# PraKesEy/EEGNetReplication

Hardware: AMD Instinct MI355X
Metric: train trials/sec (fwd+bwd) EEGNet-8,2 22ch x 256 (higher is better)
Workload: dtype fp32; 1 GPU; EEGNet-8,2 train step (fwd+CE+bwd+clamps+Adam), 22ch x 256, batch 4096/GPU, p=0.5, fp32 HIP kernels; model=EEGNet-8,2, global_batch=4096, seq_len=256, channels=22, parallelism=dp1

## Files before the change

eegnetreplication_amd/csrc/eegnet_common.h:

```cpp
#pragma once

#include <hip/hip_runtime.h>
#include <stdint.h>
#include <math.h>

namespace eeg {

constexpr int NTH = 1024;
constexpr int NWAVE = NTH / 64;
constexpr int K2 = 16;
constexpr int NCLS = 4;
constexpr int LP2 = 8;
constexpr int MAXPF = 16;
constexpr int F2MAX = 16;
constexpr int MAXT1Q = 4;

typedef float floatx4 __attribute__((ext_vector_type(4)));

__device__ __forceinline__ floatx4 lds_ld4(const float* p) {
    return *reinterpret_cast<const floatx4*>(__builtin_assume_aligned(p, 16));
}
__device__ __forceinline__ void lds_st4(float* p, floatx4 v) {
    *reinterpret_cast<floatx4*>(__builtin_assume_aligned(p, 16)) = v;
}
typedef float floatx2 __attribute__((ext_vector_type(2)));
__device__ __forceinline__ floatx2 lds_ld2(const float* p) {
    return *reinterpret_cast<const floatx2*>(__builtin_assume_aligned(p, 8));
}
__device__ __forceinline__ void lds_st_oct(float* p, int oc, floatx4 lo, floatx4 hi) {
    const bool sw = (oc >> 2) & 1;
    lds_st4(p + (sw ? 4 : 0), sw ? hi : lo);
    lds_st4(p + (sw ? 0 : 4), sw ? lo : hi);
}

struct Geo {
    int B, C, T, F1, D, F2, K1, P, R;
    int T1, T2, NF;
    int LP, RS;
    int TQ, NT16;
    int RS2;
    int RSW;
    int nwC, nwD;
    int CK, NCT, NKG;
    int nH, nTl, nedge;
    float p, scale, eps, mom;
    int drop;
    int noclamp;
    unsigned long long key;
    unsigned key0, key1;
    unsigned pthr;
    const int32_t* keystep;
    unsigned long long kseed, koff;
    int o_w1, o_g1, o_b1, o_ws, o_g2, o_b2, o_w2, o_W3, o_g3, o_b3, o_Wfc, o_bfc, nparam;
    int nA, nB, nC, nD, nE;
    int QR;
    int grid;
    int gridS;
    int gridA, gridE;
    int ldsA, ldsB, ldsC, ldsD, ldsE, ldsI;
    int ldsX;
    unsigned long long* trace;
    int wide, NOC, CPC, F2P, RB, gridB2;
    int gridW2;
    int splitC, splitD, splitE;
    int ldsWA, ldsWB, ldsWB2, ldsWC, ldsWD, ldsWE, ldsWI;
    int Bn;
    int defer;
    int XP;
};

#define EEG_SHAPE_W5(X)                                                                             \
    X(C, 64) X(T, 512) X(F1, 16) X(D, 4) X(F2, 64) X(K1, 32) X(P, 15) X(R, 16) X(T1, 128) X(T2, 16)  \
    X(NF, 1024) X(LP, 16) X(RS, 548) X(TQ, 128) X(NT16, 32) X(RS2, 144) X(RSW, 156) X(CK, 64)       \
    X(NCT, 4) X(NKG, 32) X(nH, 136) X(nTl, 120) X(nedge, 287) X(o_w1, 0) X(o_g1, 512) X(o_b1, 528)   \
    X(o_ws, 544) X(o_g2, 4640) X(o_b2, 4704) X(o_w2, 4768) X(o_W3, 5792) X(o_g3, 9888) X(o_b3, 9952) \
    X(o_Wfc, 10016) X(o_bfc, 14112) X(nparam, 14116) X(nA, 448) X(nB, 128) X(nC, 4229) X(nD, 5248)    \
    X(nE, 6272) X(QR, 64) X(wide, 1) X(NOC, 4) X(CPC, 16) X(F2P, 64) X(RB, 144) X(splitC, 1)         \
    X(splitD, 1) X(splitE, 1) X(ldsWA, 36656) X(ldsWB, 0) X(ldsWB2, 19712) X(ldsWC, 10528)           \
    X(ldsWD, 37952) X(ldsWE, 29504) X(ldsWI, 37760)
__host__ __device__ __forceinline__ void shape_w5(Geo& g) {
#define EEG_SET_(f, v) g.f = v;
    EEG_SHAPE_W5(EEG_SET_)
#undef EEG_SET_
}
template <bool SPEC>
__device__ __forceinline__ Geo geo_w(const Geo& gin) {
    Geo g = gin;
    if constexpr (SPEC) shape_w5(g);
    return g;
}

constexpr int TR_SLOTS = 16, TR_MAXWG = 2048;
enum TraceEv { TR_ENTRY = 0, TR_PRO, TR_LOOP, TR_PUB, TR_GRP, TR_TOP, TR_FIN, TR_PH0 = 8 };
#ifdef EEGNET_TRACE
#define TRACE_ON(g_) ((g_).trace != nullptr)
#else
#define TRACE_ON(g_) false
#endif
#define TRACE(g_, pass_, ev_)                                                                    \
    do {                                                                                         \
        if (TRACE_ON(g_) && threadIdx.x == 0)                                                      \
            (g_).trace[((size_t)(pass_) * TR_MAXWG + blockIdx.x) * TR_SLOTS + (ev_)] = wall_clock64(); \
    } while (0)
__device__ __forceinline__ void trial_range(const Geo& g, int& b0, int& b1) {
    const long long w = blockIdx.x, G = gridDim.x;
    b0 = (int)(w * g.B / G);
    b1 = (int)((w + 1) * g.B / G);
}

constexpr int TR_FINE = 6;
#define TRACE_FS(g_, pass_, k_)                                                                  \
    do {                                                                                         \
        if (TRACE_ON(g_) && threadIdx.x == 0)                                                      \
            (g_).trace[((size_t)TR_FINE * TR_MAXWG + (pass_)) * TR_SLOTS + (k_)] = wall_clock64(); \
    } while (0)
#define TRACE_PS(g_, k_)                                                                         \
    do {                                                                                         \
        if (TRACE_ON(g_) && threadIdx.x == 0)                                                      \
            (g_).trace[((size_t)(TR_FINE + 1) * TR_MAXWG + blockIdx.x) * TR_SLOTS + (k_)] = wall_clock64(); \
    } while (0)
#define TRACE_PH(g_, pass_, ph_, t0_)                                                            \
    do {                                                                                         \
        if (TRACE_ON(g_) && threadIdx.x == 0) {                                                  \
            const unsigned long long t1_ = clock64();                                            \
            tr_lds_[ph_] += t1_ - (t0_);                                                         \
            (t0_) = t1_;                                                                         \
        }                                                                                        \
    } while (0)
#define TRACE_LOOP(g_, pass_)                                                                    \
    do {                                                                                         \
        TRACE(g_, pass_, TR_LOOP);                                                               \
        if (TRACE_ON(g_) && threadIdx.x == 0)                                                    \
            for (int ph_ = 0; ph_ < 8; ++ph_)                                                    \
                (g_).trace[((size_t)(pass_) * TR_MAXWG + blockIdx.x) * TR_SLOTS + TR_PH0 + ph_] = tr_lds_[ph_]; \
    } while (0)
#ifdef EEGNET_TRACE
#define TRACE_DECL()                                                                             \
    __shared__ unsigned long long tr_lds_[8];                                                    \
    if (threadIdx.x == 0)                                                                        \
        for (int ph_ = 0; ph_ < 8; ++ph_) tr_lds_[ph_] = 0;                                      \
    unsigned long long tph_ = clock64();                                                         \
    (void)tph_
#else
#define TRACE_DECL() unsigned long long tph_ = 0; unsigned long long* tr_lds_ = nullptr; (void)tph_; (void)tr_lds_
#endif

enum CoefField {
    CF_A1 = 0, CF_C1, CF_INV1, CF_MU1, CF_AL2, CF_BE2, CF_INV2, CF_MU3, CF_INV3,
    CF_A3, CF_B3, CF_C3, CF_AO, CF_BO, CF_CO, CF_W, CF_LOSS, CF_ADAM, CF_COUNT
};
constexpr int CSTR = 64;

enum PassCMode { PC_LOGITS = 1, PC_BWD = 2, PC_CE = 4 };

constexpr int KSMAX = 16;
#ifndef EEGNET_NGRPMAX
#define EEGNET_NGRPMAX 16
#endif
constexpr int NGRPMAX = EEGNET_NGRPMAX;
constexpr int NCNT = 40;
#ifndef EEGNET_TKS
#define EEGNET_TKS 64
#endif
constexpr int TKS = EEGNET_TKS;
__host__ __device__ __forceinline__ unsigned* tkw(unsigned* cnt, int i) { return cnt + (size_t)i * TKS; }
constexpr int SPLIT_COLS = 2048;
constexpr int TK_PASSES = 5;
struct FinArgs {
    double* part2;
    unsigned* cnt;
    double* stats;
    float* coef;
    float* bn;
    float* grads;
    float* loss;
    int64_t* nbt;
    int update_running, ce;
    int tpass;
    float* params;
    float* adam_m;
    float* adam_v;
    int32_t* step;
    float lr, b1, b2, eps;
};

enum { TK_A = 0, TK_B, TK_C, TK_D, TK_E, TK_COUNT };

struct WsOff {
    unsigned long long cnt, partA, partB, partC, partD, partE, sums, stats, coef, d2, E1, E2, dp2, dl, s, v, q3, r3;
};
struct FoldCall {
    const eegnet_fold* folds;
    long long row0, slot;
    unsigned long long koff;
    float lr, b1, b2, eps;
    WsOff off;
};

#ifndef EEGNET_NT_MID
#define EEGNET_NT_MID 1
#endif
#ifndef EEGNET_NT_SV
#define EEGNET_NT_SV 1
#endif
template <int NT, typename V>
__device__ __forceinline__ void st_pol(V v, V* p) {
    if constexpr (NT != 0) __builtin_nontemporal_store(v, p);
    else *p = v;
}

#ifndef EEGNET_PRIO
#define EEGNET_PRIO 1
#endif
__device__ __forceinline__ void pace_prio(int done, int total) {
    if constexpr (EEGNET_PRIO != 0) {
        switch ((done * 4) / total) {
        case 0: __builtin_amdgcn_s_setprio(3); break;
        case 1: __builtin_amdgcn_s_setprio(2); break;
        case 2: __builtin_amdgcn_s_setprio(1); break;
        default: __builtin_amdgcn_s_setprio(0); break;
        }
    }
}
__device__ __forceinline__ void tail_prio() {
    if constexpr (EEGNET_PRIO != 0) __builtin_amdgcn_s_setprio(3);
}

__device__ __forceinline__ eegnet_fold fold_rec(const FoldCall& fc) {
#if defined(__HIP_DEVICE_COMPILE__)
    return ((const __attribute__((address_space(4))) eegnet_fold*)fc.folds)[blockIdx.y];
#else
    return fc.folds[blockIdx.y];
#endif
}

__device__ __forceinline__ long long fold_row(const int64_t* __restrict__ perm, long long row0, int bb) {
    return perm ? perm[row0 + bb] : row0 + bb;
}

__device__ __forceinline__ FinArgs fold_fin(const FoldCall& fc, const eegnet_fold& f, int tk, int update_running,
                                            int ce, bool nbt, bool adam, int nparam) {
    char* ws = (char*)f.ws;
    FinArgs a;
    a.part2 = (double*)(ws + fc.off.sums);
    a.cnt = tkw((unsigned*)(ws + fc.off.cnt), tk * NCNT);
    a.stats = (double*)(ws + fc.off.stats);
    a.coef = (float*)(ws + fc.off.coef);
    a.bn = f.bn_buffers;
    a.grads = f.grads;
    a.loss = f.losses ? f.losses + fc.slot : nullptr;
    a.nbt = nbt ? f.num_batches_tracked : nullptr;
    a.update_running = update_running;
    a.ce = ce;
    a.tpass = tk;
    a.params = adam ? f.params : nullptr;
    a.adam_m = adam ? f.adam_state : nullptr;
    a.adam_v = adam ? f.adam_state + nparam : nullptr;
    a.step = adam ? f.step : nullptr;
    a.lr = fc.lr; a.b1 = fc.b1; a.b2 = fc.b2; a.eps = fc.eps;
    return a;
}

__host__ __device__ constexpr int rup4(int a) { return (a + 3) & ~3; }
__host__ __device__ constexpr int imax(int a, int b) { return a > b ? a : b; }
__host__ __device__ constexpr int s_pitch(int T) { return (T + 3) & ~3; }

__host__ __device__ constexpr int row_stride(int K1, int T) {
    const int P = (K1 - 1) / 2, R = K1 - 1 - P, LP = (R + 3) & ~3, OFF = LP - P, OFFD = LP - R;
    const int NW = (OFF + K1 + 6) / 4, TQ = (T + 3) / 4, NT16 = (T + 15) / 16;
    const int NW8 = (imax(OFF, OFFD) + K1 + 10) / 4, NO = (T + 7) / 8;
    const int NWT = (15 + K1 - 1) / 16 + 1;
    const int rs = rup4(imax(imax(imax(imax(4 * (TQ - 1) + 4 * NW, 8 * (NO - 1) + 4 * NW8), LP + 16 * NT16), LP + T + R),
                             OFF + 16 * (NT16 + NWT - 1)));
    return ((rs / 4) & 1) ? rs : rs + 4;
}
__host__ __device__ constexpr int row_stride2(int T) { return rup4(LP2 + T / 4 + 8); }
__host__ __device__ constexpr int row_stride_b2(int T1) {
    const int r = rup4(T1 + 24);
    return ((r / 4) & 1) ? r : r + 4;
}

template <int K1>
struct KG {
    static constexpr int P = (K1 - 1) / 2;
    static constexpr int R = K1 - 1 - P;
    static constexpr int LP = (R + 3) & ~3;
    static constexpr int OFF = LP - P;
    static constexpr int OFFD = LP - R;
    static constexpr int NW = (OFF + K1 + 3 + 3) / 4;
    static constexpr int NW8 = ((OFF > OFFD ? OFF : OFFD) + K1 + 7 + 3) / 4;
    template <int NT>
    static constexpr int nei() { return ((R * (R + 1) / 2 + P * (P + 1) / 2 + R + P) + NT - 1) / NT; }
};

__device__ __forceinline__ float fast_exp(float z) { return __builtin_amdgcn_exp2f(z * 1.4426950408889634f); }
__device__ __forceinline__ float elu_f(float z) { return z > 0.f ? z : fast_exp(z) - 1.f; }
__device__ __forceinline__ float elu_d(float z) { return z > 0.f ? 1.f : fast_exp(z); }

__device__ __forceinline__ unsigned long long mix_key_dev(unsigned long long seed, unsigned long long off) {
    unsigned long long z = seed * 0xD1B54A32D192ED03ull + off * 0x9E3779B97F4A7C15ull + 0x632BE59BD9B4E019ull;
    z = (z ^ (z >> 30)) * 0xBF58476D1CE4E5B9ull;
    z = (z ^ (z >> 27)) * 0x94D049BB133111EBull;
    return z ^ (z >> 31);
}
__device__ __forceinline__ unsigned drop_key(const Geo& g, int layer) {
    if (!g.keystep) return layer ? g.key1 : g.key0;
    const unsigned long long k = mix_key_dev(g.kseed, g.koff + (unsigned long long)(*g.keystep));
    return layer ? (unsigned)(k >> 32) ^ 0x5BD1E995u : (unsigned)k;
}
__device__ __forceinline__ unsigned fold_drop_key(const FoldCall& fc, const eegnet_fold& f, int layer) {
    const unsigned long long k = mix_key_dev(f.seed, fc.koff + (unsigned long long)(*f.step));
    return layer ? (unsigned)(k >> 32) ^ 0x5BD1E995u : (unsigned)k;
}
__device__ __forceinline__ float keep_mul(const Geo& g, const uint8_t* __restrict__ mask, unsigned key,
                                          unsigned idx) {
    if (!g.drop) return 1.f;
    if (mask) return mask[idx] ? g.scale : 0.f;
    unsigned h = idx * 0x9E3779B1u + key;
    h ^= h >> 16;
    h *= 0x85EBCA6Bu;
    h ^= h >> 13;
    h *= 0xC2B2AE35u;
    h ^= h >> 16;
    return (h >> 8) >= g.pthr ? g.scale : 0.f;
}

__device__ __forceinline__ void drain_prologue_loads() { __builtin_amdgcn_s_waitcnt(0); }

template <int U, typename T>
struct Stage {
    T v[U];
    const T* src;
    __device__ __forceinline__ void load(const T* s, int n) {
        src = s;
        const int nth = blockDim.x, last = n > 0 ? n - 1 : 0;
#pragma unroll
        for (int j = 0; j < U; ++j) v[j] = s[min((int)threadIdx.x + j * nth, last)];
    }
    template <typename D>
    __device__ __forceinline__ void store(D* dst, int n) const {
        const int nth = blockDim.x;
#pragma unroll
        for (int j = 0; j < U; ++j) {
            const int i = threadIdx.x + j * nth;
            if (i < n) dst[i] = (D)v[j];
        }
        for (int i = threadIdx.x + U * nth; i < n; i += nth) dst[i] = (D)src[i];
    }
};

template <typename T>
__device__ __forceinline__ T ldc(const T* p) {
#if defined(__HIP_DEVICE_COMPILE__)
    return *(const __attribute__((address_space(4))) T*)p;
#else
    return *p;
#endif
}

__device__ __forceinline__ int opaque0() {
    int z = 0;
    asm volatile("" : "+s"(z));
    return z;
}
__device__ __forceinline__ int opaque0_after(float dep) {
    int z = 0;
    asm volatile("" : "+s"(z) : "v"(dep));
    return z;
}

__device__ __forceinline__ void swap32(float& a, float& b) {
    asm("s_nop 1\n\tv_permlane32_swap_b32 %0, %1" : "+v"(a), "+v"(b));
}
__device__ __forceinline__ void swap16(float& a, float& b) {
    asm("s_nop 1\n\tv_permlane16_swap_b32 %0, %1" : "+v"(a), "+v"(b));
}
template <int CTRL>
__device__ __forceinline__ float dpp(float v) {
    return __builtin_bit_cast(float, __builtin_amdgcn_update_dpp(0, __builtin_bit_cast(int, v), CTRL, 0xF, 0xF, false));
}
__device__ __forceinline__ float row_sum16(float v) {
    v += dpp<0xB1>(v);
    v += dpp<0x4E>(v);
    v += dpp<0x124>(v);
    v += dpp<0x128>(v);
    return v;
}

template <int N>
__device__ __forceinline__ void half_reduce(float (&v)[N]) {
    static_assert(N % 2 == 0, "half_reduce: N must be even");
#pragma unroll
    for (int j = 0; j < N / 2; ++j) {
        swap16(v[j], v[j + N / 2]);
        v[j] += v[j + N / 2];
    }
#pragma unroll
    for (int j = 0; j < N / 2; ++j) v[j] = row_sum16(v[j]);
}

__device__ __forceinline__ float wave_sum(float v) {
    float a = v, b = v;
    swap32(a, b);
    v = a + b;
    a = v; b = v;
    swap16(a, b);
    return row_sum16(a + b);
}

template <int N>
__device__ __forceinline__ void wave_reduce(float (&v)[N]) {
    static_assert(N % 4 == 0, "wave_reduce: N must be a multiple of 4");
#pragma unroll
    for (int i = 0; i < N / 2; ++i) {
        swap32(v[i], v[i + N / 2]);
        v[i] += v[i + N / 2];
    }
#pragma unroll
    for (int j = 0; j < N / 4; ++j) {
        swap16(v[j], v[j + N / 4]);
        v[j] += v[j + N / 4];
    }
#pragma unroll
    for (int j = 0; j < N / 4; ++j) v[j] = row_sum16(v[j]);
}

template <int NWMAX>
__device__ __forceinline__ float wave_rows_sum(const float* red, int nw, int stride, int c) {
    float v[NWMAX];
#pragma unroll
    for (int w = 0; w < NWMAX; ++w) v[w] = red[min(w, nw - 1) * stride + c];
    float a = 0.f;
#pragma unroll
    for (int w = 0; w < NWMAX; ++w) a += w < nw ? v[w] : 0.f;
    return a;
}

__device__ __forceinline__ void wave_lds_fence() {
    __builtin_amdgcn_fence(__ATOMIC_RELEASE, "wavefront");
    __builtin_amdgcn_s_waitcnt(0xC07F);
    __builtin_amdgcn_fence(__ATOMIC_ACQUIRE, "wavefront");
}

template <int NW>
__device__ __forceinline__ void lds_window(const float* __restrict__ p, float (&w)[4 * NW]) {
#pragma unroll
    for (int i = 0; i < NW; ++i) {
        const floatx4 f = lds_ld4(p + 4 * i);
        w[4 * i + 0] = f[0]; w[4 * i + 1] = f[1]; w[4 * i + 2] = f[2]; w[4 * i + 3] = f[3];
    }
}

template <int K, int OFF, int NWF>
__device__ __forceinline__ void fir4(const float (&w)[NWF], const float (&tap)[K], float (&out)[4]) {
#pragma unroll
    for (int i = 0; i < 4; ++i) {
        float a = 0.f;
#pragma unroll
        for (int k = 0; k < K; ++k) a = fmaf(tap[k], w[OFF + i + k], a);
        out[i] = a;
    }
}

template <int K, int OFF, int NWF>
__device__ __forceinline__ void fir8(const float (&w)[NWF], const float (&tap)[K], float (&out)[8]) {
#pragma unroll
    for (int i = 0; i < 8; ++i) out[i] = 0.f;
#pragma unroll
    for (int k = 0; k < K; ++k)
#pragma unroll
        for (int i = 0; i < 8; ++i) out[i] = fmaf(tap[k], w[OFF + i + k], out[i]);
}

template <int PF, int NT = NTH>
__device__ __forceinline__ void x_prefetch(const float* __restrict__ xb, int C, int T, float (&pf)[PF], int tid) {
    const int n = C * T;
    if ((T & 3) == 0) {
        const float4* src = reinterpret_cast<const float4*>(xb);
#pragma unroll
        for (int j = 0; j < PF / 4; ++j) {
            const int i = tid + NT * j;
            float4 v = make_float4(0.f, 0.f, 0.f, 0.f);
            if (4 * i < n) v = src[i];
            pf[4 * j] = v.x; pf[4 * j + 1] = v.y; pf[4 * j + 2] = v.z; pf[4 * j + 3] = v.w;
        }
    } else {
#pragma unroll
        for (int j = 0; j < PF; ++j) {
            const int i = tid + NT * j;
            pf[j] = i < n ? xb[i] : 0.f;
        }
    }
}

template <int PF, int NT = NTH>
__device__ __forceinline__ void x_store(const float (&pf)[PF], int C, int T, int RS, int LP, float* Xs, int tid) {
    const int n = C * T;
    if ((T & 3) == 0) {
        const int TQ = T >> 2;
#pragma unroll
        for (int j = 0; j < PF / 4; ++j) {
            const int i = tid + NT * j;
            if (4 * i < n) {
                const int c = i / TQ, q = i - c * TQ;
                lds_st4(Xs + c * RS + LP + 4 * q, (floatx4){pf[4 * j], pf[4 * j + 1], pf[4 * j + 2], pf[4 * j + 3]});
            }
        }
    } else {
#pragma unroll
        for (int j = 0; j < PF; ++j) {
            const int i = tid + NT * j;
            if (i < n) {
                const int c = i / T, t = i - c * T;
                Xs[c * RS + LP + t] = pf[j];
            }
        }
    }
}

#ifndef EEGNET_LDSX_A
#define EEGNET_LDSX_A 0
#endif
#ifndef EEGNET_SPATIAL_PLAIN
#define EEGNET_SPATIAL_PLAIN 0
#endif
template <int KS>
__device__ __forceinline__ int spatial_ch(int s, int lk) {
    if constexpr (KS % 2 == 0 && !EEGNET_SPATIAL_PLAIN) {
        return (8 * (s >> 1) + 2 * (s & 1)) + ((lk >> 1) + 4 * (lk & 1));
    } else {
        return 4 * s + lk;
    }
}

template <int KS>
__device__ __forceinline__ void load_ws_frag(const float* __restrict__ ws, int C, int F2, float (&aw)[KS],
                                             int lane) {
    const int o = lane & 15, lk = lane >> 4;
#pragma unroll
    for (int s = 0; s < KS; ++s) {
        const int c = spatial_ch<KS>(s, lk);
        aw[s] = (o < F2 && c < C) ? ws[o * C + c] : 0.f;
    }
}

template <int KS, int NW = NWAVE>
__device__ __forceinline__ void spatial_mfma(const float* Xs, const float (&aw)[KS], float* Ss, int C, int F2,
                                             int NT16, int RS, int LP, int wave, int lane) {
    const int li = lane & 15, lk = lane >> 4;
    int ks = (C + 3) >> 2;
    if constexpr (KS % 2 == 0 && !EEGNET_SPATIAL_PLAIN) ks = (ks + 1) & ~1;
    const int cl = spatial_ch<KS>(0, lk);
    const float* xcol = Xs + LP + li + cl * RS;
    for (int n = wave; n < NT16; n += NW) {
        floatx4 acc = {0.f, 0.f, 0.f, 0.f};
#pragma unroll
        for (int s = 0; s < KS; ++s) {
            if (s < ks) {
                const int c = spatial_ch<KS>(s, lk), cs = c - cl;
#if EEGNET_LDSX_A == 1
                const float b = 0.01f * (c + n);
#else
                const float b = (c < C) ? xcol[cs * RS + 16 * n] : 0.f;
#endif
                acc = __builtin_amdgcn_mfma_f32_16x16x4f32(aw[s], b, acc, 0, 0, 0);
            }
        }
#pragma unroll
        for (int r = 0; r < 4; ++r) {
            const int o = 4 * lk + r;
            if (o < F2) Ss[o * RS + LP + 16 * n + li] = acc[r];
        }
    }
}

#define EEG_DIMS(g) EEG_DIMS_NT(g, NTH)
#define EEG_DIMS_NT(g, NT_)                                                                 \
    const int C = CC ? CC : (g).C;                                                          \
    const int T = TT ? TT : (g).T;                                                          \
    const int F2 = FF ? FF : (g).F2;                                                        \
    const int TQ = (T + 3) >> 2, T1 = T >> 2, T2 = T1 >> 3, NF = F2 * T2;                   \
    const int RS = TT ? row_stride(K1, TT) : (g).RS;                                        \
    const int RS2 = TT ? row_stride2(TT) : (g).RS2;                                         \
    const int NT16 = (T + 15) >> 4, NCT = (C + 15) >> 4;                                    \
    constexpr int LP = KG<K1>::LP;                                                          \
    constexpr int PF = (CC && TT) ? ((CC * TT + (NT_) - 1) / (NT_) + 3) / 4 * 4 : MAXPF * NTH / (NT_); \
    constexpr int KS = CC ? (CC + 3) / 4 : 16;                                              \
    (void)TQ; (void)T1; (void)T2; (void)NF; (void)RS2; (void)NT16; (void)NCT; (void)LP

}
```

eegnetreplication_amd/csrc/eegnet_host.hip:

```cpp
using namespace eeg;

static thread_local std::string g_err;

static int fail(int code, const char* fmt, ...) {
    char buf[512];
    va_list ap;
    va_start(ap, fmt);
    vsnprintf(buf, sizeof(buf), fmt, ap);
    va_end(ap);
    g_err = buf;
    return code;
}

constexpr int LDS_MAX = 160 * 1024 - 256;

static inline int rup(int a, int m) { return (a + m - 1) / m * m; }
static inline size_t rupz(size_t a, size_t m) { return (a + m - 1) / m * m; }

constexpr size_t CNT_BYTES = (size_t)TK_COUNT * NCNT * TKS * 4;

struct WsLayout {
    size_t cnt, partA, partB, partC, partD, partE, sums, stats, coef, d2, E1, E2, dp2, dl, s, v, q3, r3;
    size_t total;
};

static int device_cus() {
    static int cus = 0;
    if (cus == 0) {
        int dev = 0;
        if (hipGetDevice(&dev) != hipSuccess ||
            hipDeviceGetAttribute(&cus, hipDeviceAttributeMultiprocessorCount, dev) != hipSuccess || cus <= 0)
            cus = 256;
    }
    return cus;
}

static unsigned long long* g_trace_buf = nullptr;

static int make_geo_wide(Geo* g, bool launch);

static void b2_lds(Geo* g, int nw) {
    auto tailw = [](int ncols, int fin) { return 2 * (tail_s_doubles(ncols) + fin); };
    const int nf4 = (g->NF + 3) / 4 * 4;
    const int b2 = 2 * g->F2P * g->RB + g->F2P * K2 + g->F2P * (g->F2P + 1);
    const int TQ1 = (g->T1 + 3) / 4;
    g->ldsWB2 = std::max(b2 + nw * 2 * 16, tailw(g->nB, 0));
    g->ldsWC = std::max(nf4 + nw * 4 + nw * 2 * 16 + g->F2P * g->RB, tailw(g->nC, 0));
    g->ldsWD = std::max(b2 + g->F2P * g->RB + nf4 + 2 * g->F2 * TQ1, tailw(g->nD, 0));
}

#ifndef EEGNET_B2
#define EEGNET_B2 0
#endif
static bool use_b2_narrow(const Geo&) { return EEGNET_B2 == 1; }

#ifndef EEGNET_D1
#define EEGNET_D1 0
#endif

#ifndef EEGNET_GRIDS_MULT
#define EEGNET_GRIDS_MULT 1
#endif
#ifndef EEGNET_GRIDC_MULT
#define EEGNET_GRIDC_MULT 1
#endif
static_assert(EEGNET_GRIDS_MULT >= 1 && EEGNET_GRIDS_MULT <= 8 && EEGNET_GRIDC_MULT >= 1 && EEGNET_GRIDC_MULT <= 8,
              "grid multipliers are 1..8");
static constexpr int grid_mult() { return EEGNET_GRIDS_MULT; }
static constexpr int grid_mult_cd() { return EEGNET_GRIDC_MULT; }

static bool x_pitch_shape(const eegnet_dims& d) {
    return d.K1 == 32 && d.C == 22 && d.T == 257 && d.F1 == 8 && d.D == 2;
}

static int make_geo(const eegnet_dims* d, Geo* g, bool launch = true) {
    if (!d) return fail(EEGNET_EINVAL, "dims is NULL");
    memset(g, 0, sizeof(*g));
    g->trace = g_trace_buf;
    g->B = d->B; g->C = d->C; g->T = d->T; g->F1 = d->F1; g->D = d->D; g->K1 = d->K1;
    g->Bn = d->B;
    g->F2 = d->F1 * d->D;
    if (g->B < 1) return fail(EEGNET_EINVAL, "B must be >= 1 (got %d)", g->B);
    if (g->K1 != 32 && g->K1 != 64) return fail(EEGNET_EINVAL, "K1 must be 32 or 64 (got %d)", g->K1);
    if (g->C < 1 || g->C > 64) return fail(EEGNET_EINVAL, "C must be in [1,64] (got %d)", g->C);
    if (g->F1 < 1 || g->D < 1 || g->F2 > 64 || (g->F2 & 3))
        return fail(EEGNET_EINVAL, "F1*D must be a multiple of 4 in [4,64] (got F1=%d D=%d)", g->F1, g->D);
    if (g->T < 32 || g->T < g->K1 || g->T > 1024)
        return fail(EEGNET_EINVAL, "T must be in [max(32,K1), 1024] (got %d)", g->T);
    g->XP = d->x_pitch ? d->x_pitch : g->T;
    if (g->XP != g->T && !(x_pitch_shape(*d) && (g->XP & 3) == 0 && g->XP > g->T))
        return fail(EEGNET_EINVAL, "x_pitch %d: only the 22 x 257 EEGNet-8,2 (K1 = 32) training kernels take "
                    "a row pitch, a multiple of 4 above T (eegnet_x_pitch)", g->XP);
    g->P = (g->K1 - 1) / 2; g->R = g->K1 - 1 - g->P;
    g->T1 = g->T / 4; g->T2 = g->T1 / 8; g->NF = g->F2 * g->T2;
    g->LP = (g->R + 3) & ~3;
    g->TQ = (g->T + 3) / 4; g->NT16 = (g->T + 15) / 16; g->NKG = g->NT16;
    g->RS = row_stride(g->K1, g->T);
    g->RS2 = rup(LP2 + g->T1 + 8, 4);
    g->CK = rup(g->C, 4); g->NCT = (g->C + 15) / 16;
    g->nH = g->R * (g->R + 1) / 2;
    g->nTl = g->P * (g->P + 1) / 2;
    g->nedge = g->nH + g->nTl + g->R + g->P;
    g->p = d->p_drop; g->eps = d->bn_eps; g->mom = d->bn_momentum;
    if (!(g->p >= 0.f && g->p <= 1.f)) return fail(EEGNET_EINVAL, "p_drop must be in [0,1]");
    g->scale = g->p < 1.f ? 1.f / (1.f - g->p) : 0.f;
    int o = 0;
    g->o_w1 = o; o += g->F1 * g->K1;
    g->o_g1 = o; o += g->F1;
    g->o_b1 = o; o += g->F1;
    g->o_ws = o; o += g->F2 * g->C;
    g->o_g2 = o; o += g->F2;
    g->o_b2 = o; o += g->F2;
    g->o_w2 = o; o += g->F2 * 16;
    g->o_W3 = o; o += g->F2 * g->F2;
    g->o_g3 = o; o += g->F2;
    g->o_b3 = o; o += g->F2;
    g->o_Wfc = o; o += NCLS * g->NF;
    g->o_bfc = o; o += NCLS;
    g->nparam = o;
    if (g->NF < 1) return fail(EEGNET_EINVAL, "T//32 must be >= 1");
    g->nA = g->K1 + 1 + g->nedge + 2 * g->F2;
    g->nB = 2 * g->F2;
    g->nC = NCLS * g->NF + NCLS + 2 * g->F2 + 1;
    g->nD = g->F2 * g->F2 + 18 * g->F2;
    g->QR = (g->F2 <= F2MAX && g->D == 2) ? g->F1 : g->F2;
    g->nE = g->QR * g->K1 + g->F2 * g->C + 2 * g->F2;
    g->grid = std::min(g->B, device_cus() * grid_mult_cd());
    g->gridS = std::min(g->B, device_cus() * WGPC * grid_mult());
    g->gridA = g->gridE = g->gridS;
    const int rows1 = g->C * g->RS;
    const int nf4 = rup(g->NF, 4);
    const bool spec = g->C == 22 && (g->T == 256 || g->T == 257) && g->F1 == 8 && g->D == 2 && g->K1 == 32;
    g->ldsA = (spec ? 2 : 1) * rows1 + g->F2 * g->RS + NWB * (g->K1 + 1) + (spec ? 2 * rup(g->K1 + 1 + g->nedge, 4) : 0);
    g->ldsB = 3 * g->F2 * g->RS2 + F2MAX * (K2 + F2MAX);
    g->RSW = row_stride_b2(g->T1);
    const int pwC = nf4, pwD = 3 * g->F2 * g->RSW + nf4;
    g->nwC = std::max(1, std::min(spec ? NWAVE : NTHS / 64, (LDS_MAX / 4 - 4 * F2MAX) / pwC));
    g->nwD = std::max(1, std::min(NTHS / 64, (LDS_MAX / 4) / pwD));
    g->ldsC = std::max(g->nwC * pwC + 4 * F2MAX, g->nwC * g->nC);
    g->ldsD = EEGNET_D1 ? std::max(g->nwD * pwD, g->nwD * g->nD)
                        : std::max(dr_lds_floats(spec ? 1 : MAXT1Q), dr_tail_floats(spec));
    g->ldsE = std::max((2 * g->F2 + g->C) * g->RS + rup(g->F2 * g->T1, 4) + 8 * g->F2,
                       NWB * 256 * (1 + (15 + g->K1 - 1) / 16 + 1));
    g->ldsI = rows1 + g->F2 * g->RS + 2 * g->F2 * g->RS2 + nf4;
    g->ldsX = rows1 + 2 * g->F2 * g->RS + 2 * g->F2 * g->RS2 + nf4 + 4;
    auto tail = [](int ncols, int fin) { return 2 * (tail_s_doubles(ncols) + std::max(tail_scratch_doubles(ncols), fin)); };
    g->ldsA = std::max(g->ldsA, tail(g->nA, fin1_scratch_doubles(g->K1, g->F1, g->F2, g->C)));
    g->ldsB = std::max(g->ldsB, tail(g->nB, 0));
    g->ldsC = std::max(g->ldsC, tail(g->nC, 0));
    g->ldsD = std::max(g->ldsD, tail(g->nD, 0));
    g->ldsE = std::max(g->ldsE, tail(g->nE, fin5_scratch_doubles(g->K1, g->F1, g->o_g2)));
    g->wide = g->F2 > F2MAX ? 1 : 0;
    if (g->wide) return make_geo_wide(g, launch);
    g->F2P = 16;
    g->RB = rb_stride(g->T1);
    b2_lds(g, 4);
    g->gridB2 = std::min(g->B, 4 * device_cus());
    if (launch) {
        if (g->C * g->T > NTH * MAXPF)
            return fail(EEGNET_EINVAL, "C*T = %d exceeds the %d-float prefetch of one trial", g->C * g->T,
                        NTH * MAXPF);
        if (g->T1 > 64 * MAXT1Q) return fail(EEGNET_EINVAL, "T/4 > %d", 64 * MAXT1Q);
        if (g->F2 * g->T1 > 4 * NTH) return fail(EEGNET_EINVAL, "F2*(T/4) > %d", 4 * NTH);
        if ((double)g->B * g->F2 * g->T1 >= 4294967296.0)
            return fail(EEGNET_EINVAL, "B*F2*(T/4) must stay below 2^32 (dropout / mask indices)");
        if (g->NF > 64 * MAXNFQ) return fail(EEGNET_EINVAL, "F2*(T/32) = %d > %d", g->NF, 64 * MAXNFQ);
        if (g->nparam > APT * NTB) return fail(EEGNET_EINVAL, "%d parameters > %d", g->nparam, APT * NTB);
        const int lmax = std::max(std::max(std::max(g->ldsA, g->ldsB), std::max(g->ldsC, g->ldsD)),
                                  std::max(g->ldsE, g->ldsI));
        if (lmax * 4 > LDS_MAX) return fail(EEGNET_EINVAL, "dims need %d B of LDS (> %d)", lmax * 4, LDS_MAX);
    }
    return 0;
}

static int make_geo_wide(Geo* g, bool launch) {
    const int cus = device_cus();
    g->NOC = (g->F2 + 15) / 16;
    g->CPC = (g->C + g->NOC - 1) / g->NOC;
    g->F2P = g->F2 <= 32 ? 32 : 64;
    g->RB = rb_stride(g->T1);
    int G = std::min(g->B * g->NOC, cus);
    G = std::max(g->NOC, G / g->NOC * g->NOC);
    if (G >= 8 * g->NOC) G = G / (8 * g->NOC) * (8 * g->NOC);
    g->gridS = G;
    g->gridA = g->gridE = G;
    g->grid = std::min(g->B, cus);
    g->splitC = g->nC > SPLIT_COLS; g->splitD = g->nD > SPLIT_COLS; g->splitE = g->nE > SPLIT_COLS;
    const int nf4 = rup(g->NF, 4);
    auto tailw = [](int ncols, int fin) { return 2 * (tail_s_doubles(ncols) + fin); };
    const int awl = KSW * 64;
    const int cgw = NWW * 256 * ((15 + g->K1 - 1) / 16 + 1);
    const bool w5 = g->C == 64 && g->T == 512 && g->F1 == 16 && g->D == 4 && g->K1 == 32;
    const int baseA = (w5 ? 2 : 1) * (g->CPC + 16) * g->RS + NWW * (g->K1 + 1) + 2 * NWW + awl;
    g->ldsWA = std::max(baseA + ((g->CPC + 16) * g->RS >= cgw ? 0 : cgw),
                        tailw(g->nA, std::max(NTH, fin1_scratch_doubles(g->K1, g->F1, g->F2, g->C))));
    g->ldsWB = 0;
    const int b2 = 2 * g->F2P * g->RB + g->F2P * K2 + g->F2P * (g->F2P + 1);
    b2_lds(g, NWB2);
    g->gridB2 = g->grid;
    g->gridW2 = w5 ? std::min(g->B, 2 * cus) : g->grid;
    if (w5) g->ldsWB2 = std::max(g->ldsWB2 - g->F2P * (g->F2P + 1), tailw(g->nB, 0));
    g->ldsWE = std::max(std::max(3 * 16 * g->RS + rup(16 * g->T1, 4) + 8 * 16 + awl, NWW * 256 + 32 + NWW * 256 * ((15 + g->K1 - 1) / 16 + 1)),
                        tailw(g->nE, fin5_scratch_doubles(g->K1, g->F1, g->o_g2)));
    g->ldsWI = 16 * g->RS + b2 + nf4 + 4 * g->F2P + g->NOC * awl;
    (void)nf4;
    if (!launch) return 0;
    if (g->C > 4 * KSW) return fail(EEGNET_EINVAL, "C = %d > %d", g->C, 4 * KSW);
    if (g->T1 > 16 * NTTW * (NWB2 / 4)) return fail(EEGNET_EINVAL, "T/4 = %d > %d", g->T1, 16 * NTTW * (NWB2 / 4));
    if (g->NF > MAXNFW * NTB2) return fail(EEGNET_EINVAL, "F2*(T/32) = %d > %d", g->NF, MAXNFW * NTB2);
    if ((double)g->B * g->F2 * g->T1 >= 4294967296.0)
        return fail(EEGNET_EINVAL, "B*F2*(T/4) must stay below 2^32 (dropout / mask indices)");
    const int lmax = std::max(std::max(std::max(g->ldsWA, g->ldsWB), std::max(g->ldsWB2, g->ldsWC)),
                              std::max(std::max(g->ldsWD, g->ldsWE), g->ldsWI));
    if (lmax * 4 > LDS_MAX) return fail(EEGNET_EINVAL, "dims need %d B of LDS (> %d)", lmax * 4, LDS_MAX);
    return 0;
}

static WsLayout make_layout(const Geo& g) {
    WsLayout L;
    size_t o = 0;
    auto take = [&](size_t bytes) { size_t r = o; o = rupz(o + bytes, 256); return r; };
    L.cnt = take(CNT_BYTES);
    L.partA = take((size_t)std::max(g.gridS, g.gridA) * g.nA * 4);
    L.partB = take((size_t)std::max(std::max(g.gridS, g.grid), g.gridW2) * g.nB * 4);
    L.partC = take((size_t)std::max(std::max(g.grid, g.gridB2), g.gridW2) * g.nC * 4);
    L.partD = take((size_t)std::max(std::max(g.grid, g.gridB2), g.gridS) * g.nD * 4);
    L.partE = take((size_t)std::max(g.gridS, g.gridE) * g.nE * 4);
    const int nmax = std::max(std::max(std::max(g.nA, g.nB), std::max(g.nC, g.nD)), g.nE);
    L.sums = take((size_t)nmax * 8 * NGRPMAX);
    L.stats = take((size_t)(g.F1 * g.K1 + g.K1) * 8);
    L.coef = take((size_t)CF_COUNT * CSTR * 4);
    const size_t per = (size_t)g.B * g.F2 * g.T1 * 4;
    L.d2 = take(per); L.E1 = take(per); L.E2 = take(per); L.dp2 = take(per);
    L.dl = take((size_t)g.B * NCLS * 4);
    L.s = take((size_t)g.B * g.F2 * s_pitch(g.T) * 4);
    L.v = take((size_t)g.B * g.F2 * ((g.T + 7) / 8 * 8) * 4);
    L.q3 = take(per);
    L.r3 = take(per);
    L.total = o;
    return L;
}

static uint64_t mix_key(uint64_t seed, uint64_t offset) {
    uint64_t z = seed * 0xD1B54A32D192ED03ull + offset * 0x9E3779B97F4A7C15ull + 0x632BE59BD9B4E019ull;
    z = (z ^ (z >> 30)) * 0xBF58476D1CE4E5B9ull;
    z = (z ^ (z >> 27)) * 0x94D049BB133111EBull;
    return z ^ (z >> 31);
}

static void set_key(Geo* g, uint64_t seed, uint64_t offset) {
    g->key = mix_key(seed, offset);
    g->key0 = (unsigned)g->key;
    g->key1 = (unsigned)(g->key >> 32) ^ 0x5BD1E995u;
    g->pthr = (unsigned)std::min(16777216.0, std::max(0.0, (double)g->p * 16777216.0));
}

enum KernelId { KID_A = 0, KID_B, KID_C, KID_D, KID_E, KID_ADAM, KID_INFER, KID_MEMSET, KID_INFER_BF16,
                KID_WA, KID_WB, KID_WB2, KID_WC, KID_WD, KID_WE, KID_WINFER, KID_CTAIL, KID_XSTATS, KID_INFER_DX,
                KID_COUNT };
static const char* kKernelNames[KID_COUNT] = {"k_pass_a", "k_pass_b", "k_pass_c", "k_pass_d", "k_pass_e",
                                              "k_adam", "k_infer", "memset_tickets", "k_infer_bf16",
                                              "k_wpass_a", "k_wpass_b", "k_wpass_b2", "k_wpass_c", "k_wpass_d",
                                              "k_wpass_e", "k_winfer", "k_coltail", "k_xstats", "k_infer_dx"};
#ifndef EEGNET_PROF_EVENT_FLAGS
#define EEGNET_PROF_EVENT_FLAGS hipEventDisableSystemFence
#endif
struct ProfRec { int kid; hipEvent_t a, b; };
struct ProfState { unsigned mask = 0; std::vector<ProfRec> recs; std::vector<hipEvent_t> pool; };
static thread_local ProfState g_prof;

static hipEvent_t prof_event() {
    if (!g_prof.pool.empty()) { hipEvent_t e = g_prof.pool.back(); g_prof.pool.pop_back(); return e; }
    hipEvent_t e;
    hipEventCreateWithFlags(&e, EEGNET_PROF_EVENT_FLAGS);
    return e;
}
struct ProfScope {
    int kid; hipStream_t s; hipEvent_t a = nullptr;
    ProfScope(int k, hipStream_t st) : kid(k), s(st) {
        if ((g_prof.mask >> k) & 1u) { a = prof_event(); hipEventRecord(a, s); }
    }
    ~ProfScope() {
        if (a) { hipEvent_t b = prof_event(); hipEventRecord(b, s); g_prof.recs.push_back({kid, a, b}); }
    }
};
#define PROF(kid) ProfScope prof_scope_##kid(kid, s)

#define LAUNCH_CHECK(what)                                                            \
    do {                                                                              \
        hipError_t e_ = hipGetLastError();                                            \
        if (e_ != hipSuccess) return fail(EEGNET_ELAUNCH, "%s: %s", what, hipGetErrorString(e_)); \
    } while (0)

static bool g_attr_done = false;

template <int K1, int CC, int TT, int FF>
static void set_attrs_shape() {
    const int lds = LDS_MAX;
    for (const void* f : {(const void*)k_pass_a<K1, CC, TT, FF>, (const void*)k_pass_b<K1, CC, TT, FF>,
                          (const void*)k_pass_c<K1, CC, TT, FF>,
                          (const void*)k_pass_e<K1, CC, TT, FF>, (const void*)k_pass_a<K1, CC, TT, FF, true>,
                          (const void*)k_pass_b<K1, CC, TT, FF, true>, (const void*)k_pass_c<K1, CC, TT, FF, true>,
                          (const void*)k_pass_e<K1, CC, TT, FF, true>,
#if EEGNET_D1
                          (const void*)k_pass_d<K1, CC, TT, FF>, (const void*)k_pass_d<K1, CC, TT, FF, false, false>,
                          (const void*)k_pass_d<K1, CC, TT, FF, true, false>,
#endif
                          (const void*)k_pass_dr<K1, CC, TT, FF>, (const void*)k_pass_dr<K1, CC, TT, FF, false, false>,
                          (const void*)k_pass_dr<K1, CC, TT, FF, true, false>})
        hipFuncSetAttribute(f, hipFuncAttributeMaxDynamicSharedMemorySize, lds);
    hipFuncSetAttribute((const void*)k_infer<K1, CC, TT, FF>, hipFuncAttributeMaxDynamicSharedMemorySize, lds);
    hipFuncSetAttribute((const void*)k_infer_dx<K1, CC, TT, FF>, hipFuncAttributeMaxDynamicSharedMemorySize, lds);
    hipFuncSetAttribute((const void*)k_frozen<K1, CC, TT, FF, true>, hipFuncAttributeMaxDynamicSharedMemorySize, lds);
    hipFuncSetAttribute((const void*)k_frozen<K1, CC, TT, FF, false>, hipFuncAttributeMaxDynamicSharedMemorySize, lds);
    hipFuncSetAttribute((const void*)k_eval_folds<K1, CC, TT, FF>, hipFuncAttributeMaxDynamicSharedMemorySize, lds);
}

template <int K1>
static void set_attrs_wide() {
    for (const void* f : {(const void*)k_wpass_a<K1>, (const void*)k_wpass_b<K1>, (const void*)k_wpass_e<K1>,
                          (const void*)k_winfer<K1>})
        hipFuncSetAttribute(f, hipFuncAttributeMaxDynamicSharedMemorySize, LDS_MAX);
}

static void ensure_attrs() {
    if (g_attr_done) return;
    set_attrs_wide<32>();
    set_attrs_wide<64>();
    for (const void* f : {(const void*)k_wpass_a<32, true>, (const void*)k_wpass_b<32, true>, (const void*)k_wpass_e<32, true>,
                          (const void*)k_winfer<32, true>, (const void*)k_wpass_b2<NTB2, true>,
                          (const void*)k_wpass_c<NTB2, false, true>, (const void*)k_wpass_d<NTB2, false, true>,
                          (const void*)k_coltail<3, true>, (const void*)k_coltail<4, true>, (const void*)k_coltail<5, true>})
        hipFuncSetAttribute(f, hipFuncAttributeMaxDynamicSharedMemorySize, LDS_MAX);
    for (const void* f : {(const void*)k_wpass_b2<NTB2>, (const void*)k_wpass_c<NTB2>, (const void*)k_wpass_d<NTB2>,
                          (const void*)k_wpass_c<256>, (const void*)k_wpass_d<256>,
                          (const void*)k_wpass_c<256, true>, (const void*)k_wpass_d<256, true>,
                          (const void*)k_coltail<3>, (const void*)k_coltail<4>, (const void*)k_coltail<5>,
                          (const void*)k_fin})
        hipFuncSetAttribute(f, hipFuncAttributeMaxDynamicSharedMemorySize, LDS_MAX);
    for (const void* f : {(const void*)k_infer_bf16<0>, (const void*)k_infer_bf16<1>, (const void*)k_infer_bf16<2>,
                          (const void*)k_infer_bf16<4>, (const void*)k_infer_bf16<8>, (const void*)k_infer_bf16<16>,
                          (const void*)k_infer_bf16<8, true>, (const void*)k_infer_bf16_cfg5})
        hipFuncSetAttribute(f, hipFuncAttributeMaxDynamicSharedMemorySize, LDS_MAX);
    set_attrs_shape<32, 0, 0, 0>();
    set_attrs_shape<64, 0, 0, 0>();
    hipFuncSetAttribute((const void*)k_xstats<32>, hipFuncAttributeMaxDynamicSharedMemorySize, LDS_MAX);
    hipFuncSetAttribute((const void*)k_xstats<64>, hipFuncAttributeMaxDynamicSharedMemorySize, LDS_MAX);
    set_attrs_shape<32, 22, 256, 16>();
    set_attrs_shape<32, 22, 257, 16>();
    g_attr_done = true;
}

#define EEG_DISPATCH(K1_, g_, LAUNCH)                                                            \
    do {                                                                                         \
        if ((K1_) == 32 && (g_).C == 22 && (g_).T == 256 && (g_).F1 == 8 && (g_).D == 2) { LAUNCH(32, 22, 256, 16); } \
        else if ((K1_) == 32 && (g_).C == 22 && (g_).T == 257 && (g_).F1 == 8 && (g_).D == 2) { LAUNCH(32, 22, 257, 16); } \
        else { LAUNCH(K1_, 0, 0, 0); }                                                           \
    } while (0)

static FinArgs fin_args(const WsLayout& L, char* ws, int tk, float* bn, float* grads, float* loss,
                        int update_running, int ce, int64_t* nbt = nullptr) {
    FinArgs f;
    memset(&f, 0, sizeof(f));
    f.part2 = (double*)(ws + L.sums);
    f.cnt = tkw((unsigned*)(ws + L.cnt), tk * NCNT);
    f.stats = (double*)(ws + L.stats);
    f.coef = (float*)(ws + L.coef);
    f.bn = bn; f.grads = grads; f.loss = loss;
    f.update_running = update_running; f.ce = ce;
    f.nbt = nbt;
    f.tpass = tk;
    return f;
}


static bool same_shape_w5(const Geo& g) {
#define EEG_EQ_(f, v) && g.f == v
    return true EEG_SHAPE_W5(EEG_EQ_);
#undef EEG_EQ_
}
#define WLAUNCH(sp, KG, KS, grid_, blk_, lds_, ...)                                               \
    do {                                                                                          \
        if (sp) hipLaunchKernelGGL(KS, grid_, blk_, lds_, __VA_ARGS__);                           \
        else hipLaunchKernelGGL(KG, grid_, blk_, lds_, __VA_ARGS__);                              \
    } while (0)

static int grid_wpass_b(const Geo& g, bool sp) { return sp ? std::min(2 * g.gridS, g.B * g.NOC) : g.gridS; }
static int grid_pass_c(const Geo& g) { return g.wide ? g.gridW2 : use_b2_narrow(g) ? g.gridB2 : g.grid; }
static int grid_pass_d(const Geo& g) {
    return g.wide ? g.grid : use_b2_narrow(g) ? g.gridB2 : EEGNET_D1 ? g.grid : g.gridS;
}
static int streams_pass_c(const Geo& g) {
    return grid_pass_c(g) * ((g.wide || use_b2_narrow(g)) ? 1 : g.nwC);
}
static int streams_pass_d(const Geo& g) {
    return grid_pass_d(g) * ((g.wide || use_b2_narrow(g) || !EEGNET_D1) ? 1 : g.nwD);
}

template <int K1>
static int run_forward_wide(const Geo& g, const WsLayout& L, char* ws, const float* params, float* bn,
                            const float* x, const uint8_t* m2, int update_running, int64_t* nbt, hipStream_t s) {
    const FinArgs fa = fin_args(L, ws, TK_A, bn, nullptr, nullptr, update_running, 0);
    const FinArgs fb = fin_args(L, ws, TK_B, bn, nullptr, nullptr, update_running, 0, nbt);
    const bool sp = K1 == 32 && same_shape_w5(g);
    { PROF(KID_WA); WLAUNCH(sp, (k_wpass_a<K1>), (k_wpass_a<K1, K1 == 32>), dim3(g.gridS), dim3(NTW), g.ldsWA * 4, s, g,
                            params, x, (float*)(ws + L.s), (float*)(ws + L.v), (float*)(ws + L.partA), fa); }
    LAUNCH_CHECK("k_wpass_a");
    { PROF(KID_WB); WLAUNCH(sp, (k_wpass_b<K1>), (k_wpass_b<K1, K1 == 32>), dim3(sp ? std::min(2 * g.gridS, g.B * g.NOC) : g.gridS), dim3(NTW), g.ldsWB * 4, s, g,
                            params, (const float*)(ws + L.coef), (const float*)(ws + L.v), m2, (float*)(ws + L.d2),
                            (float*)(ws + L.E1), (float*)(ws + L.E2)); } LAUNCH_CHECK("k_wpass_b");
    { PROF(KID_WB2); WLAUNCH(sp, k_wpass_b2<NTB2>, (k_wpass_b2<NTB2, true>), dim3(g.gridW2), dim3(NTB2), g.ldsWB2 * 4, s,
                             g, params, (const float*)(ws + L.d2), (float*)(ws + L.q3), (float*)(ws + L.r3),
                             (float*)(ws + L.partB), fb); } LAUNCH_CHECK("k_wpass_b2");
    return 0;
}

template <int K1>
static int run_backward_wide(const Geo& g, const WsLayout& L, char* ws, float* params, const float* x,
                             const uint8_t* m2, const uint8_t* m3, const float* dlogits, const int64_t* labels,
                             float* logits, float* grads, float* loss, int c_mode, const FinArgs* adam,
                             hipStream_t s) {
    const float* coef = (const float*)(ws + L.coef);
    const float* dl = dlogits ? dlogits : (const float*)(ws + L.dl);
    const FinArgs fc = fin_args(L, ws, TK_C, nullptr, grads, loss, 0, (c_mode & PC_CE) ? 1 : 0);
    const FinArgs fd = fin_args(L, ws, TK_D, nullptr, grads, nullptr, 0, 0);
    FinArgs fe = fin_args(L, ws, TK_E, nullptr, grads, nullptr, 0, 0);
    if (adam) {
        fe.params = params; fe.adam_m = adam->adam_m; fe.adam_v = adam->adam_v; fe.step = adam->step;
        fe.lr = adam->lr; fe.b1 = adam->b1; fe.b2 = adam->b2; fe.eps = adam->eps;
    }
    const bool sp = K1 == 32 && same_shape_w5(g);
    auto coltail = [&](int fin, const float* part, int nrows, int ncols, const FinArgs& fa, int scr) {
        const int nb = (ncols + 63) / 64;
        const size_t lds = 8 * (size_t)std::max(2 + (NTCT / 64) * 64, tail_s_doubles(ncols) + scr);
        PROF(KID_CTAIL);
        if (fin == 3) WLAUNCH(sp, k_coltail<3>, (k_coltail<3, true>), dim3(nb), dim3(NTCT), lds, s, g, (const float*)params, part, nrows, ncols, fa);
        else if (fin == 4) WLAUNCH(sp, k_coltail<4>, (k_coltail<4, true>), dim3(nb), dim3(NTCT), lds, s, g, (const float*)params, part, nrows, ncols, fa);
        else WLAUNCH(sp, k_coltail<5>, (k_coltail<5, true>), dim3(nb), dim3(NTCT), lds, s, g, (const float*)params, part, nrows, ncols, fa);
    };
    { PROF(KID_WC); WLAUNCH(sp, k_wpass_c<NTB2>, (k_wpass_c<NTB2, false, true>), dim3(g.gridW2), dim3(NTB2), g.ldsWC * 4, s,
                            g, params, coef, (const float*)(ws + L.r3), m3, dlogits, labels, logits, (float*)(ws + L.dl),
                            (float*)(ws + L.partC), c_mode, fc, FoldCall{}); } LAUNCH_CHECK("k_wpass_c(bwd)");
    if (g.splitC) { coltail(3, (const float*)(ws + L.partC), g.gridW2, g.nC, fc, 0); LAUNCH_CHECK("k_coltail(C)"); }
    { PROF(KID_WD); WLAUNCH(sp, k_wpass_d<NTB2>, (k_wpass_d<NTB2, false, true>), dim3(g.grid), dim3(NTB2), g.ldsWD * 4, s,
                            g, params, coef, (const float*)(ws + L.d2), (const float*)(ws + L.E1), (const float*)(ws + L.E2),
                            (const float*)(ws + L.q3), (const float*)(ws + L.r3), m2, m3, dl,
                            (float*)(ws + L.dp2), (float*)(ws + L.partD), fd, FoldCall{}); }
    LAUNCH_CHECK("k_wpass_d");
    if (g.splitD) { coltail(4, (const float*)(ws + L.partD), g.grid, g.nD, fd, 0); LAUNCH_CHECK("k_coltail(D)"); }
    { PROF(KID_WE); WLAUNCH(sp, (k_wpass_e<K1>), (k_wpass_e<K1, K1 == 32>), dim3(g.gridS), dim3(NTW), g.ldsWE * 4, s, g,
                            (const float*)params, coef, x, (const float*)(ws + L.s), (const float*)(ws + L.v),
                            (const float*)(ws + L.dp2), (float*)(ws + L.partE), fe); } LAUNCH_CHECK("k_wpass_e");
    if (g.splitE) {
        coltail(5, (const float*)(ws + L.partE), g.gridS / g.NOC, g.nE, fe, fin5_scratch_doubles(g.K1, g.F1, g.o_g2));
        LAUNCH_CHECK("k_coltail(E)");
    }
    return 0;
}

template <int K1>
static int run_forward(const Geo& g, const WsLayout& L, char* ws, const float* params, float* bn,
                       const float* x, const uint8_t* m2, int update_running, int64_t* nbt, hipStream_t s,
                       const FoldCall& fc = FoldCall{}, int nf = 1, int only = -1) {
    if (g.wide) return run_forward_wide<K1>(g, L, ws, params, bn, x, m2, update_running, nbt, s);
    const FinArgs fa = fin_args(L, ws, TK_A, bn, nullptr, nullptr, update_running, 0);
    const FinArgs fb = fin_args(L, ws, TK_B, bn, nullptr, nullptr, update_running, 0, nbt);
#define LAUNCH_A(K, CC, TT, FF) if (fc.folds) hipLaunchKernelGGL((k_pass_a<K, CC, TT, FF, true>), dim3(g.gridA, nf), dim3(NTB), g.ldsA * 4, s, \
                                                   g, params, x, (float*)(ws + L.s), (float*)(ws + L.v), (float*)(ws + L.partA), fa, fc); \
    else hipLaunchKernelGGL((k_pass_a<K, CC, TT, FF>), dim3(g.gridA, nf), dim3(NTB), g.ldsA * 4, s, \
                                                   g, params, x, (float*)(ws + L.s), (float*)(ws + L.v), (float*)(ws + L.partA), fa, fc)
    if (only < 0 || only == 0) { { PROF(KID_A); EEG_DISPATCH(K1, g, LAUNCH_A);
    } LAUNCH_CHECK("k_pass_a"); }
#define LAUNCH_B(K, CC, TT, FF) if (fc.folds) hipLaunchKernelGGL((k_pass_b<K, CC, TT, FF, true>), dim3(g.gridS, nf), dim3(NTB), g.ldsB * 4, s, \
                       g, params, (const float*)(ws + L.coef), (const float*)(ws + L.v), m2, (float*)(ws + L.d2), \
                       (float*)(ws + L.E1), (float*)(ws + L.E2), (float*)(ws + L.q3), (float*)(ws + L.r3), \
                       (float*)(ws + L.partB), fb, fc); \
    else hipLaunchKernelGGL((k_pass_b<K, CC, TT, FF>), dim3(g.gridS, nf), dim3(NTB), g.ldsB * 4, s, \
                       g, params, (const float*)(ws + L.coef), (const float*)(ws + L.v), m2, (float*)(ws + L.d2), \
                       (float*)(ws + L.E1), (float*)(ws + L.E2), (float*)(ws + L.q3), (float*)(ws + L.r3), \
                       (float*)(ws + L.partB), fb, fc)
    if (only < 0 || only == 1) { { PROF(KID_B); EEG_DISPATCH(K1, g, LAUNCH_B);
    } LAUNCH_CHECK("k_pass_b"); }
    return 0;
}

template <int K1>
static int run_backward(const Geo& g, const WsLayout& L, char* ws, float* params,
                        const float* x, const uint8_t* m2, const uint8_t* m3, const float* dlogits,
                        const int64_t* labels, float* logits, float* grads, float* loss, int c_mode,
                        const FinArgs* adam, hipStream_t s, const FoldCall& fc = FoldCall{}, int nf = 1,
                        int only = -1) {
    if (g.wide)
        return run_backward_wide<K1>(g, L, ws, params, x, m2, m3, dlogits, labels, logits, grads, loss, c_mode,
                                     adam, s);
    const float* coef = (const float*)(ws + L.coef);
    const float* dl = dlogits ? dlogits : (const float*)(ws + L.dl);
    const FinArgs fcC = fin_args(L, ws, TK_C, nullptr, grads, loss, 0, (c_mode & PC_CE) ? 1 : 0);
    const FinArgs fd = fin_args(L, ws, TK_D, nullptr, grads, nullptr, 0, 0);
    FinArgs fe = fin_args(L, ws, TK_E, nullptr, grads, nullptr, 0, 0);
    if (adam) {
        fe.params = params; fe.adam_m = adam->adam_m; fe.adam_v = adam->adam_v; fe.step = adam->step;
        fe.lr = adam->lr; fe.b1 = adam->b1; fe.b2 = adam->b2; fe.eps = adam->eps;
    }
#define LAUNCH_CB(K, CC, TT, FF) if (fc.folds) hipLaunchKernelGGL((k_pass_c<K, CC, TT, FF, true>), dim3(grid_pass_c(g), nf), dim3(64 * g.nwC), g.ldsC * 4, s, \
                       g, params, coef, (const float*)(ws + L.r3), m3, dlogits, labels, logits, \
                       (float*)(ws + L.dl), (float*)(ws + L.partC), c_mode, fcC, fc); \
    else hipLaunchKernelGGL((k_pass_c<K, CC, TT, FF>), dim3(grid_pass_c(g), nf), dim3(64 * g.nwC), g.ldsC * 4, s, \
                       g, params, coef, (const float*)(ws + L.r3), m3, dlogits, labels, logits, \
                       (float*)(ws + L.dl), (float*)(ws + L.partC), c_mode, fcC, fc)
    if (use_b2_narrow(g)) {
        if (only >= 0) return fail(EEGNET_EINVAL, "staged steps do not support EEGNET_B2=1");
        { PROF(KID_C);
          if (fc.folds) hipLaunchKernelGGL((k_wpass_c<256, true>), dim3(grid_pass_c(g), nf), dim3(256), g.ldsWC * 4, s, g,
                                           params, coef, (const float*)(ws + L.r3), m3, dlogits, labels, logits,
                                           (float*)(ws + L.dl), (float*)(ws + L.partC), c_mode, fcC, fc);
          else hipLaunchKernelGGL((k_wpass_c<256>), dim3(grid_pass_c(g)), dim3(256), g.ldsWC * 4, s, g, params, coef,
                                  (const float*)(ws + L.r3), m3, dlogits, labels, logits, (float*)(ws + L.dl),
                                  (float*)(ws + L.partC), c_mode, fcC, fc);
        } LAUNCH_CHECK("k_wpass_c<256>");
        { PROF(KID_D);
          if (fc.folds) hipLaunchKernelGGL((k_wpass_d<256, true>), dim3(grid_pass_d(g), nf), dim3(256), g.ldsWD * 4, s, g,
                                           params, coef, (const float*)(ws + L.d2), (const float*)(ws + L.E1),
                                           (const float*)(ws + L.E2), (const float*)(ws + L.q3),
                                           (const float*)(ws + L.r3), m2, m3, dl, (float*)(ws + L.dp2),
                                           (float*)(ws + L.partD), fd, fc);
          else hipLaunchKernelGGL((k_wpass_d<256>), dim3(grid_pass_d(g)), dim3(256), g.ldsWD * 4, s, g, params, coef,
                                  (const float*)(ws + L.d2), (const float*)(ws + L.E1), (const float*)(ws + L.E2),
                                  (const float*)(ws + L.q3), (const float*)(ws + L.r3), m2, m3, dl,
                                  (float*)(ws + L.dp2), (float*)(ws + L.partD), fd, fc);
        } LAUNCH_CHECK("k_wpass_d<256>");
    } else {
    if (only < 0 || only == 2) { { PROF(KID_C); EEG_DISPATCH(K1, g, LAUNCH_CB);
    } LAUNCH_CHECK("k_pass_c(bwd)"); }
#define LAUNCH_DR(K, CC, TT, FF) if (fc.folds) hipLaunchKernelGGL((k_pass_dr<K, CC, TT, FF, true, false>), dim3(grid_pass_d(g), nf), dim3(NTB), g.ldsD * 4, s, \
                       g, params, coef, (const float*)(ws + L.d2), (const float*)(ws + L.E1), \
                       (const float*)(ws + L.E2), (const float*)(ws + L.q3), (const float*)(ws + L.r3), \
                       m2, m3, dl, (float*)(ws + L.dp2), \
                       (float*)(ws + L.partD), fd, fc); \
    else if (m2 || m3) hipLaunchKernelGGL((k_pass_dr<K, CC, TT, FF>), dim3(grid_pass_d(g), nf), dim3(NTB), g.ldsD * 4, s, \
                       g, params, coef, (const float*)(ws + L.d2), (const float*)(ws + L.E1), \
                       (const float*)(ws + L.E2), (const float*)(ws + L.q3), (const float*)(ws + L.r3), \
                       m2, m3, dl, (float*)(ws + L.dp2), \
                       (float*)(ws + L.partD), fd, fc); \
    else hipLaunchKernelGGL((k_pass_dr<K, CC, TT, FF, false, false>), dim3(grid_pass_d(g), nf), dim3(NTB), g.ldsD * 4, s, \
                       g, params, coef, (const float*)(ws + L.d2), (const float*)(ws + L.E1), \
                       (const float*)(ws + L.E2), (const float*)(ws + L.q3), (const float*)(ws + L.r3), \
                       m2, m3, dl, (float*)(ws + L.dp2), \
                       (float*)(ws + L.partD), fd, fc)
#define LAUNCH_D(K, CC, TT, FF) if (fc.folds) hipLaunchKernelGGL((k_pass_d<K, CC, TT, FF, true, false>), dim3(grid_pass_d(g), nf), dim3(64 * g.nwD), g.ldsD * 4, s, \
                       g, params, coef, (const float*)(ws + L.d2), (const float*)(ws + L.E1), \
                       (const float*)(ws + L.E2), (const float*)(ws + L.q3), (const float*)(ws + L.r3), \
                       m2, m3, dl, (float*)(ws + L.dp2), \
                       (float*)(ws + L.partD), fd, fc); \
    else if (m2 || m3) hipLaunchKernelGGL((k_pass_d<K, CC, TT, FF>), dim3(grid_pass_d(g), nf), dim3(64 * g.nwD), g.ldsD * 4, s, \
                       g, params, coef, (const float*)(ws + L.d2), (const float*)(ws + L.E1), \
                       (const float*)(ws + L.E2), (const float*)(ws + L.q3), (const float*)(ws + L.r3), \
                       m2, m3, dl, (float*)(ws + L.dp2), \
                       (float*)(ws + L.partD), fd, fc); \
    else hipLaunchKernelGGL((k_pass_d<K, CC, TT, FF, false, false>), dim3(grid_pass_d(g), nf), dim3(64 * g.nwD), g.ldsD * 4, s, \
                       g, params, coef, (const float*)(ws + L.d2), (const float*)(ws + L.E1), \
                       (const float*)(ws + L.E2), (const float*)(ws + L.q3), (const float*)(ws + L.r3), \
                       m2, m3, dl, (float*)(ws + L.dp2), \
                       (float*)(ws + L.partD), fd, fc)
#if EEGNET_D1
#define LAUNCH_PASS_D LAUNCH_D
#else
#define LAUNCH_PASS_D LAUNCH_DR
#endif
    if (only < 0 || only == 3) { { PROF(KID_D); EEG_DISPATCH(K1, g, LAUNCH_PASS_D);
    } LAUNCH_CHECK("k_pass_d"); }
    }
#define LAUNCH_E(K, CC, TT, FF) if (fc.folds) hipLaunchKernelGGL((k_pass_e<K, CC, TT, FF, true>), dim3(g.gridE, nf), dim3(NTB), g.ldsE * 4, s, \
                       g, (const float*)params, coef, x, (const float*)(ws + L.s), (const float*)(ws + L.v), \
                       (const float*)(ws + L.dp2), (float*)(ws + L.partE), fe, fc); \
    else hipLaunchKernelGGL((k_pass_e<K, CC, TT, FF>), dim3(g.gridE, nf), dim3(NTB), g.ldsE * 4, s, \
                       g, (const float*)params, coef, x, (const float*)(ws + L.s), (const float*)(ws + L.v), \
                       (const float*)(ws + L.dp2), (float*)(ws + L.partE), fe, fc)
    if (only < 0 || only == 4) { { PROF(KID_E); EEG_DISPATCH(K1, g, LAUNCH_E);
    } LAUNCH_CHECK("k_pass_e"); }
    return 0;
}

#ifndef EEGNET_BF16_V1
#define EEGNET_BF16_V1 0
#endif
static float* g_bf16_dbg = nullptr;

static int make_geo_bf16(const eegnet_dims* d, GeoI* g) {
    Geo q;
    if (int r = make_geo(d, &q, false)) return r;
    memset(g, 0, sizeof(*g));
    g->B = q.B; g->C = q.C; g->T = q.T; g->F1 = q.F1; g->D = q.D; g->F2 = q.F2; g->K1 = q.K1; g->P = q.P;
    g->eps = q.eps;
    g->o_w1 = q.o_w1; g->o_g1 = q.o_g1; g->o_b1 = q.o_b1; g->o_ws = q.o_ws; g->o_g2 = q.o_g2;
    g->o_b2 = q.o_b2; g->o_w2 = q.o_w2; g->o_W3 = q.o_W3; g->o_g3 = q.o_g3; g->o_b3 = q.o_b3;
    g->o_Wfc = q.o_Wfc; g->o_bfc = q.o_bfc;
    g->CP = rup(g->C, 32); g->KC = g->CP / 32;
    g->F2P = g->F2 <= 16 ? 16 : g->F2 <= 32 ? 32 : 64;
    g->NOT = g->F2P / 16;
    g->F2K = std::max(32, g->F2P); g->KCW = g->F2K / 32;
    g->TX = rup(g->T, 128);
    g->NT = (g->T + 15) / 16; g->NBLK = (g->NT + 15) / 16;
    g->LPs = g->P + 1;
    g->KSF = (g->K1 + 16 + 31) / 32;
    g->SXs = 256 * g->NBLK + 32 * g->KSF - 8;
    g->T1 = g->T / 4; g->T2 = g->T1 / 8; g->NF = g->F2 * g->T2;
    const int nq = (g->T1 + 3) / 4;
    g->RA = 4 * nq + 16;
    g->NT1 = (8 * g->T2 + 15) / 16;
    g->TZ = rup(std::max(4 * nq, 16 * g->NT1), 128);
    if (g->T % 8 == 0) {
        const int units = g->CP * g->TX / 8;
        int u = (units + NTI - 1) / NTI, p = 1;
        while (p < u) p *= 2;
        g->PFU = p;
    } else {
        g->PFU = 0;
    }
    if (g->PFU > 16) return fail(EEGNET_EINVAL, "bf16 eval: C*T too large for one trial in registers");
    const int r1 = std::max(g->CP * g->TX * 2, rup(g->F2P * g->RA * 4, 16) + g->F2K * g->TZ * 2);
    g->offZ = rup(g->F2P * g->RA * 4, 16);
    g->offS = rup(r1, 16);
    g->offW1 = rup(g->offS + g->F2P * g->SXs * 2, 16);
    g->offW2 = rup(g->offW1 + g->F1 * g->K1 * 4, 16);
    g->offCo = rup(g->offW2 + g->F2P * K2 * 4, 16);
    g->offL = rup(g->offCo + 4 * g->F2P * 4, 16);
    g->lds = g->offL + NWI * NCLS * 4;
    const int offF = rup(g->lds, 16);
    if (offF + NCLS * g->NF * 4 <= LDS_MAX) {
        g->offF = offF;
        g->lds = offF + NCLS * g->NF * 4;
    }
    g->dbg = g_bf16_dbg;
    if (g->lds > LDS_MAX)
        return fail(EEGNET_EINVAL, "bf16 eval: dims need %d B of LDS (> %d): C=%d T=%d F2=%d", g->lds, LDS_MAX,
                    g->C, g->T, g->F2);
    return 0;
}

static bool same_geo_bf16(GeoI a, GeoI b) {
    a.B = b.B = 0;
    a.eps = b.eps = 0.f;
    a.dbg = b.dbg = nullptr;
    return memcmp(&a, &b, sizeof(GeoI)) == 0;
}

static int check_wide_train(const Geo& g, const char* what) {
    if (g.wide && g.K1 == 64)
        return fail(EEGNET_EINVAL, "%s: training with F1*D = %d > 16 and K1 = 64 is not supported "
                    "(K1 = 32, or F1*D <= 16; the eval forward takes these dims)", what, g.F2);
    return 0;
}

static int check_ptrs(const void* a, const char* na, const void* b = (const void*)1, const char* nb = "") {
    if (!a) return fail(EEGNET_EINVAL, "%s is NULL", na);
    if (!b) return fail(EEGNET_EINVAL, "%s is NULL", nb);
    return 0;
}

extern "C" {

int eegnet_param_count(const eegnet_dims* dims, int64_t* out) {
    Geo g;
    if (int r = make_geo(dims, &g, false)) return r;
    if (!out) return fail(EEGNET_EINVAL, "out is NULL");
    *out = g.nparam;
    return 0;
}

int eegnet_x_pitch(const eegnet_dims* dims) {
    if (!dims) return fail(EEGNET_EINVAL, "dims is NULL");
    return x_pitch_shape(*dims) && (dims->T & 3) ? (dims->T + 3) & ~3 : dims->T;
}

int eegnet_wide_spec(const eegnet_dims* dims) {
    Geo g;
    memset(&g, 0, sizeof(g));
    if (int r = make_geo(dims, &g, false)) return r;
    if (!g.wide || g.K1 != 32) return 0;
    if (same_shape_w5(g)) return 1;
    std::string msg = "geometry differs from EEG_SHAPE_W5:";
    char b[96];
#define EEG_DIFF_(f, v) if (g.f != v) { snprintf(b, sizeof(b), " %s = %d (compiled %d)", #f, (int)g.f, v); msg += b; }
    EEG_SHAPE_W5(EEG_DIFF_)
#undef EEG_DIFF_
    g_err = msg;
    return 0;
}

int eegnet_workspace_bytes(const eegnet_dims* dims, size_t* out) {
    Geo g;
    if (int r = make_geo(dims, &g)) return r;
    if (!out) return fail(EEGNET_EINVAL, "out is NULL");
    *out = make_layout(g).total;
    return 0;
}

int eegnet_forward_train(const eegnet_dims* dims, const float* params, float* bn_buffers,
                         const float* x, const uint8_t* mask2, const uint8_t* mask3,
                         uint64_t seed, uint64_t offset, float* logits, void* ws, void* stream,
                         int64_t* num_batches_tracked) {
    Geo g;
    if (int r = make_geo(dims, &g)) return r;
    if (int r = check_wide_train(g, "eegnet_forward_train")) return r;
    if (int r = check_ptrs(params, "params", bn_buffers, "bn_buffers")) return r;
    if (int r = check_ptrs(x, "x", logits, "logits")) return r;
    if (int r = check_ptrs(ws, "ws")) return r;
    g.drop = g.p > 0.f ? 1 : 0;
    set_key(&g, seed, offset);
    ensure_attrs();
    const WsLayout L = make_layout(g);
    hipStream_t s = (hipStream_t)stream;
    char* w = (char*)ws;
    int r = g.K1 == 32 ? run_forward<32>(g, L, w, params, bn_buffers, x, mask2, 1, num_batches_tracked, s)
                       : run_forward<64>(g, L, w, params, bn_buffers, x, mask2, 1, num_batches_tracked, s);
    if (r) return r;
    FinArgs none;
    memset(&none, 0, sizeof(none));
    if (g.wide) {
        const bool sp = g.K1 == 32 && same_shape_w5(g);
        { PROF(KID_WC); WLAUNCH(sp, k_wpass_c<NTB2>, (k_wpass_c<NTB2, false, true>), dim3(g.gridW2), dim3(NTB2),
                                g.ldsWC * 4, s, g, params, (const float*)(w + L.coef), (const float*)(w + L.r3), mask3,
                                (const float*)nullptr, (const int64_t*)nullptr, logits, (float*)nullptr,
                                (float*)nullptr, (int)PC_LOGITS, none, FoldCall{}); }
        LAUNCH_CHECK("k_wpass_c(fwd)");
        return 0;
    }
#define LAUNCH_CF(K, CC, TT, FF) hipLaunchKernelGGL((k_pass_c<K, CC, TT, FF>), dim3(g.grid), dim3(64 * g.nwC), g.ldsC * 4, s, \
                       g, params, (const float*)(w + L.coef), (const float*)(w + L.r3), mask3, (const float*)nullptr, \
                       (const int64_t*)nullptr, logits, (float*)nullptr, (float*)nullptr, (int)PC_LOGITS, none, \
                       FoldCall{})
    { PROF(KID_C);
      if (g.K1 == 32) EEG_DISPATCH(32, g, LAUNCH_CF); else EEG_DISPATCH(64, g, LAUNCH_CF);
    } LAUNCH_CHECK("k_pass_c(fwd)");
    return 0;
}

int eegnet_backward(const eegnet_dims* dims, const float* params, const float* x,
                    const float* dlogits, const int64_t* labels, const uint8_t* mask2,
                    const uint8_t* mask3, uint64_t seed, uint64_t offset, float* grads, float* loss,
                    void* ws, void* stream, int flags) {
    Geo g;
    if (int r = make_geo(dims, &g)) return r;
    if (int r = check_wide_train(g, "eegnet_backward")) return r;
    g.noclamp = (flags & EEGNET_NO_CLAMP) ? 1 : 0;
    if (int r = check_ptrs(params, "params", x, "x")) return r;
    if (int r = check_ptrs(grads, "grads", ws, "ws")) return r;
    if (!dlogits && !labels) return fail(EEGNET_EINVAL, "need dlogits or labels");
    g.drop = g.p > 0.f ? 1 : 0;
    set_key(&g, seed, offset);
    ensure_attrs();
    const WsLayout L = make_layout(g);
    const int mode = PC_BWD | (dlogits ? 0 : PC_CE);
    hipStream_t s = (hipStream_t)stream;
    float* p = const_cast<float*>(params);
    return g.K1 == 32
        ? run_backward<32>(g, L, (char*)ws, p, x, mask2, mask3, dlogits, labels, nullptr, grads, loss, mode, nullptr, s)
        : run_backward<64>(g, L, (char*)ws, p, x, mask2, mask3, dlogits, labels, nullptr, grads, loss, mode, nullptr, s);
}

int eegnet_forward_eval(const eegnet_dims* dims, const float* params, const float* bn_buffers,
                        const float* x, float* logits, void* stream) {
    Geo g;
    if (int r = make_geo(dims, &g)) return r;
    if (g.XP != g.T) return fail(EEGNET_EINVAL, "the eval forward takes x as [B][C][T] (x_pitch 0 or T)");
    if (int r = check_ptrs(params, "params", bn_buffers, "bn_buffers")) return r;
    if (int r = check_ptrs(x, "x", logits, "logits")) return r;
    ensure_attrs();
    hipStream_t s = (hipStream_t)stream;
    if (g.wide) {
        PROF(KID_WINFER);
        if (g.K1 == 32) WLAUNCH(same_shape_w5(g), k_winfer<32>, (k_winfer<32, true>), dim3(g.grid), dim3(NTW), g.ldsWI * 4, s,
                                g, params, bn_buffers, x, logits);
        else hipLaunchKernelGGL(k_winfer<64>, dim3(g.grid), dim3(NTW), g.ldsWI * 4, s, g, params, bn_buffers, x, logits);
        LAUNCH_CHECK("k_winfer");
        return 0;
    }
    PROF(KID_INFER);
#define LAUNCH_I(K, CC, TT, FF) hipLaunchKernelGGL((k_infer<K, CC, TT, FF>), dim3(g.grid), dim3(NTH), g.ldsI * 4, s, \
                                                   g, params, bn_buffers, x, logits)
    if (g.K1 == 32) EEG_DISPATCH(32, g, LAUNCH_I); else EEG_DISPATCH(64, g, LAUNCH_I);
    LAUNCH_CHECK("k_infer");
    return 0;
}

int eegnet_input_grad_eval(const eegnet_dims* dims, const float* params, const float* bn_buffers,
                           const float* x, int seed_kind, const float* dlogits, const int64_t* targets,
                           float* dx, float* logits, void* stream) {
    Geo g;
    if (int r = make_geo(dims, &g, false)) return r;
    if (g.wide) return fail(EEGNET_EINVAL, "input gradients: F1*D = %d > 16 is not supported", g.F2);
    if (int r = make_geo(dims, &g)) return r;
    if (g.XP != g.T) return fail(EEGNET_EINVAL, "input gradients take x as [B][C][T] (x_pitch 0 or T)");
    if (seed_kind < EEGNET_SEED_DLOGITS || seed_kind > EEGNET_SEED_CE)
        return fail(EEGNET_EINVAL, "seed_kind must be 0 (dlogits), 1 (logit) or 2 (cross-entropy) (got %d)", seed_kind);
    if (int r = check_ptrs(params, "params", bn_buffers, "bn_buffers")) return r;
    if (int r = check_ptrs(x, "x", dx, "dx")) return r;
    if (seed_kind == EEGNET_SEED_DLOGITS && !dlogits) return fail(EEGNET_EINVAL, "EEGNET_SEED_DLOGITS needs dlogits");
    if (seed_kind == EEGNET_SEED_CE && !targets) return fail(EEGNET_EINVAL, "EEGNET_SEED_CE needs targets");
    if (g.ldsX * 4 > LDS_MAX)
        return fail(EEGNET_EINVAL, "input gradients: dims need %d B of LDS (> %d)", g.ldsX * 4, LDS_MAX);
    if ((g.T & 3) == 0 && ((uintptr_t)x & 15)) return fail(EEGNET_EINVAL, "input gradients: x must be 16-byte aligned");
    const int vec = (g.T & 3) == 0 && ((uintptr_t)dx & 15) == 0;
    ensure_attrs();
    hipStream_t s = (hipStream_t)stream;
    PROF(KID_INFER_DX);
#define LAUNCH_X(K, CC, TT, FF) hipLaunchKernelGGL((k_infer_dx<K, CC, TT, FF>), dim3(g.grid), dim3(NTH), g.ldsX * 4, s, \
                                                   g, params, bn_buffers, x, seed_kind, dlogits, targets, dx, logits, vec)
    if (g.K1 == 32) EEG_DISPATCH(32, g, LAUNCH_X); else EEG_DISPATCH(64, g, LAUNCH_X);
    LAUNCH_CHECK("k_infer_dx");
    return 0;
}

int eegnet_forward_eval_bf16(const eegnet_dims* dims, const float* params, const float* bn_buffers,
                             const uint16_t* x, float* logits, void* stream) {
    GeoI g;
    if (int r = make_geo_bf16(dims, &g)) return r;
    if (dims->x_pitch && dims->x_pitch != dims->T)
        return fail(EEGNET_EINVAL, "the eval forward takes x as [B][C][T] (x_pitch 0 or T)");
    if (int r = check_ptrs(params, "params", bn_buffers, "bn_buffers")) return r;
    if (int r = check_ptrs(x, "x", logits, "logits")) return r;
    if (g.PFU > 0 && ((uintptr_t)x & 15))
        return fail(EEGNET_EINVAL, "bf16 eval: x must be 16-byte aligned");
    ensure_attrs();
    hipStream_t s = (hipStream_t)stream;
    const dim3 grid(std::min(g.B, device_cus())), blk(NTI);
    PROF(KID_INFER_BF16);
    if (same_geo_bf16(g, kGeoCfg5)) {
        if (EEGNET_BF16_V1 == 1) hipLaunchKernelGGL((k_infer_bf16<8, true>), grid, blk, g.lds, s, g, params, bn_buffers, x, logits);
        else hipLaunchKernelGGL(k_infer_bf16_cfg5, dim3(std::min(g.B, 2 * device_cus())), dim3(c5::NT), c5::LDS, s,
                                g, params, bn_buffers, x, logits);
        LAUNCH_CHECK("k_infer_bf16(cfg5)");
        return 0;
    }
    switch (g.PFU) {
        case 0: hipLaunchKernelGGL(k_infer_bf16<0>, grid, blk, g.lds, s, g, params, bn_buffers, x, logits); break;
        case 1: hipLaunchKernelGGL(k_infer_bf16<1>, grid, blk, g.lds, s, g, params, bn_buffers, x, logits); break;
        case 2: hipLaunchKernelGGL(k_infer_bf16<2>, grid, blk, g.lds, s, g, params, bn_buffers, x, logits); break;
        case 4: hipLaunchKernelGGL(k_infer_bf16<4>, grid, blk, g.lds, s, g, params, bn_buffers, x, logits); break;
        case 8: hipLaunchKernelGGL(k_infer_bf16<8>, grid, blk, g.lds, s, g, params, bn_buffers, x, logits); break;
        default: hipLaunchKernelGGL(k_infer_bf16<16>, grid, blk, g.lds, s, g, params, bn_buffers, x, logits); break;
    }
    LAUNCH_CHECK("k_infer_bf16");
    return 0;
}

int eegnet_adam_step(int64_t n, float* params, const float* grads, float* exp_avg,
                     float* exp_avg_sq, int32_t* step, float lr, float beta1, float beta2,
                     float eps, void* stream) {
    if (n <= 0) return fail(EEGNET_EINVAL, "n must be > 0");
    if (!params || !grads || !exp_avg || !exp_avg_sq || !step) return fail(EEGNET_EINVAL, "null pointer");
    hipStream_t s = (hipStream_t)stream;
    { PROF(KID_ADAM); hipLaunchKernelGGL(k_adam, dim3((unsigned)((n + 255) / 256)), dim3(256), 0, s, n, params, grads,
                       exp_avg, exp_avg_sq, step, lr, beta1, beta2, eps);
    } LAUNCH_CHECK("k_adam");
    hipLaunchKernelGGL(k_step_inc, dim3(1), dim3(64), 0, s, step);
    LAUNCH_CHECK("k_step_inc");
    return 0;
}

int eegnet_train_step(const eegnet_dims* dims, float* params, float* bn_buffers, const float* x,
                      const int64_t* labels, uint64_t seed, uint64_t offset, float* grads,
                      float* adam_state, int32_t* step, float lr, float beta1, float beta2,
                      float eps, float* loss, float* logits, void* ws, void* stream, int flags,
                      int64_t* num_batches_tracked) {
    Geo g;
    if (int r = make_geo(dims, &g)) return r;
    if (int r = check_wide_train(g, "eegnet_train_step")) return r;
    if (int r = check_ptrs(params, "params", bn_buffers, "bn_buffers")) return r;
    if (int r = check_ptrs(x, "x", labels, "labels")) return r;
    if (int r = check_ptrs(grads, "grads", ws, "ws")) return r;
    if (adam_state && !step) return fail(EEGNET_EINVAL, "step is NULL");
// ... 416 lines not shown
```

eegnetreplication_amd/csrc/eegnet_passes.hip:

```cpp

namespace eeg {


__device__ __forceinline__ void block2_rows(int F2, int T1, int RS2, const float* D2s, float* Qs,
                                            const float (&w2)[K2], const float (&w3)[F2MAX], bool row_on,
                                            int o, int lane, float (&r)[MAXT1Q]) {
    if (row_on) {
        const float* dr = D2s + o * RS2 + 1;
#pragma unroll
        for (int m = 0; m < MAXT1Q; ++m) {
            const int t = lane + 64 * m;
            if (t < T1) {
                float a = 0.f;
#pragma unroll
                for (int k = 0; k < K2; ++k) a = fmaf(w2[k], dr[t + k], a);
                Qs[o * RS2 + t] = a;
            }
        }
    }
    __syncthreads();
#pragma unroll
    for (int m = 0; m < MAXT1Q; ++m) {
        const int t = lane + 64 * m;
        float a = 0.f;
// ... 33 lines not shown
        const float carry = m > 0 ? readlane_f(x[m > 0 ? m - 1 : 0], 63) : 0.f;
        const float v = __builtin_bit_cast(float, __builtin_amdgcn_update_dpp(0, __builtin_bit_cast(int, x[m]), 0x138, 0xF, 0xF, true));
        x[m] = (m > 0 && lane == 0) ? carry : v;
    }
}
template <int MQ>
__device__ __forceinline__ void shl1(float (&x)[MQ], int lane) {
#pragma unroll
    for (int m = 0; m < MQ; ++m) {
        const float carry = m < MQ - 1 ? readlane_f(x[m < MQ - 1 ? m + 1 : m], 0) : 0.f;
        const float v = __builtin_bit_cast(float, __builtin_amdgcn_update_dpp(0, __builtin_bit_cast(int, x[m]), 0x130, 0xF, 0xF, true));
        x[m] = (m < MQ - 1 && lane == 63) ? carry : v;
    }
}

template <int MQ>
__device__ __forceinline__ void conv16_same_t(const float (&x)[MQ], const float* __restrict__ w, float (&y)[MQ],
                                              int lane) {
    float s[MQ];
#pragma unroll
    for (int m = 0; m < MQ; ++m) { y[m] = w[7] * x[m]; s[m] = x[m]; }
#pragma unroll
    for (int k = 6; k >= 0; --k) {
        shl1<MQ>(s, lane);
#pragma unroll
        for (int m = 0; m < MQ; ++m) y[m] = fmaf(w[k], s[m], y[m]);
    }
#pragma unroll
    for (int m = 0; m < MQ; ++m) s[m] = x[m];
#pragma unroll
    for (int k = 8; k < K2; ++k) {
        shr1<MQ>(s, lane);
#pragma unroll
        for (int m = 0; m < MQ; ++m) y[m] = fmaf(w[k], s[m], y[m]);
    }
}

template <int MQ>
__device__ __forceinline__ void conv16_same_t2(const float (&x)[MQ], const float* __restrict__ w, float (&y)[MQ],
                                               int lane) {
    float s[MQ], u[MQ], y1[MQ];
#pragma unroll
    for (int m = 0; m < MQ; ++m) { y[m] = w[7] * x[m]; s[m] = x[m]; u[m] = x[m]; y1[m] = 0.f; }
#pragma unroll
    for (int k = 6; k >= 0; --k) {
        shl1<MQ>(s, lane);
        shr1<MQ>(u, lane);
#pragma unroll
        for (int m = 0; m < MQ; ++m) { y[m] = fmaf(w[k], s[m], y[m]); y1[m] = fmaf(w[14 - k], u[m], y1[m]); }
    }
    shr1<MQ>(u, lane);
#pragma unroll
    for (int m = 0; m < MQ; ++m) y[m] += fmaf(w[15], u[m], y1[m]);
}

template <int MQ>
__device__ __forceinline__ void load_rows(const float* __restrict__ src, int b, int F2, int T1, int lane,
                                          float (&d)[F2MAX][MQ]) {
    const float* base = src + (size_t)b * F2 * T1;
#pragma unroll
    for (int o = 0; o < F2MAX; ++o)
#pragma unroll
        for (int m = 0; m < MQ; ++m) {
            const int t = lane + 64 * m;
            d[o][m] = (o < F2 && t < T1) ? base[o * T1 + t] : 0.f;
        }
}

template <int MQ>
__device__ __forceinline__ void bn3_rows(const float* coef, int F2, const float (&r)[F2MAX][MQ],
                                         float (&xh)[F2MAX][MQ]) {
#pragma unroll
    for (int j = 0; j < F2MAX; ++j) {
        const float mu3 = j < F2 ? coef[CF_MU3 * CSTR + j] : 0.f, inv3 = j < F2 ? coef[CF_INV3 * CSTR + j] : 0.f;
#pragma unroll
        for (int m = 0; m < MQ; ++m) xh[j][m] = (r[j][m] - mu3) * inv3;
    }
}

template <int K1, int CC, int TT, int FF, bool FOLD>
__device__ __forceinline__ void pass_c_body(const Geo& g, const float* __restrict__ prm,
                                            const float* coef,
                                            const float* __restrict__ r3g,
                                            const uint8_t* __restrict__ mask3,
                                            const float* __restrict__ dlin,
                                            const int64_t* __restrict__ labels,
                                            float* __restrict__ logits, float* __restrict__ dlout,
                                            float* __restrict__ part, int mode, FinArgs fa, const FoldCall& fc,
                                            float* sm) {
    EEG_DIMS(g);
    TRACE(g, 2, TR_ENTRY);
    unsigned dk1;
    const int64_t* perm = nullptr;
    long long row0 = 0;
    if (FOLD) {
        const eegnet_fold f = fold_rec(fc);
        char* ws = (char*)f.ws;
        prm = f.params;
        coef = (const float*)(ws + fc.off.coef);
        r3g = (const float*)(ws + fc.off.r3);
        mask3 = nullptr; dlin = nullptr; logits = nullptr;
        labels = f.labels;
        perm = f.perm; row0 = fc.row0;
        dlout = (float*)(ws + fc.off.dl);
        part = (float*)(ws + fc.off.partC);
        fa = fold_fin(fc, f, TK_C, 0, 1, false, false, g.nparam);
        dk1 = fold_drop_key(fc, f, 1);
    } else {
        dk1 = drop_key(g, 1);
    }
    constexpr int MQ = TT ? (TT / 4 + 63) / 64 : MAXT1Q;
    constexpr int NFQ = (TT && FF) ? (FF * (TT / 32) + 63) / 64 : MAXNFQ;
    const int NFP = rup4(NF);
    const int nw = blockDim.x >> 6;
    const int tid = threadIdx.x, lane = tid & 63;
    const int wave = __builtin_amdgcn_readfirstlane(tid >> 6);
    float* Hs = sm + wave * NFP;
    float* const Ct = sm + nw * NFP;
    if (tid < F2MAX) {
        const int j = tid < F2 ? tid : 0;
        const bool on = tid < F2;
        Ct[4 * tid + 0] = on ? coef[CF_MU3 * CSTR + j] : 0.f;
        Ct[4 * tid + 1] = on ? coef[CF_INV3 * CSTR + j] : 0.f;
        Ct[4 * tid + 2] = on ? prm[g.o_g3 + j] : 0.f;
        Ct[4 * tid + 3] = on ? prm[g.o_b3 + j] : 0.f;
    }

    float wf[NCLS][NFQ], wacc[NCLS][NFQ];
#pragma unroll
    for (int n = 0; n < NCLS; ++n)
#pragma unroll
        for (int u = 0; u < NFQ; ++u) {
            const int i = lane + 64 * u;
            wf[n][u] = i < NF ? prm[g.o_Wfc + n * NF + i] : 0.f;
            wacc[n][u] = 0.f;
        }
    float sdz[2 * F2MAX];
#pragma unroll
    for (int j = 0; j < 2 * F2MAX; ++j) sdz[j] = 0.f;
    float bacc[NCLS] = {0.f, 0.f, 0.f, 0.f}, lossacc = 0.f;
    const float invB = 1.0f / (float)g.Bn;
    const int bfirst = blockIdx.x * nw + wave, bstop = g.B, bstep = gridDim.x * nw;

    __syncthreads();
    TRACE(g, 2, TR_PRO);
    TRACE_DECL();
    drain_prologue_loads();
    for (int b = bfirst; b < bstop; b += bstep) {
        float xh[F2MAX][MQ];
        {
            float r[F2MAX][MQ];
            load_rows<MQ>(r3g, b, F2, T1, lane, r);
            TRACE_PH(g, 2, 0, tph_);
#pragma unroll
            for (int j = 0; j < F2MAX; ++j) {
                const floatx4 c = lds_ld4(Ct + 4 * j);
                const float mu = sgpr_f(c[0]), inv = sgpr_f(c[1]);
#pragma unroll
                for (int m = 0; m < MQ; ++m) xh[j][m] = (r[j][m] - mu) * inv;
            }
            TRACE_PH(g, 2, 1, tph_);
        }
#pragma unroll
        for (int j = 0; j < F2MAX; ++j) {
            if (j >= F2) continue;
            const floatx4 c = lds_ld4(Ct + 4 * j);
            const float g3 = sgpr_f(c[2]), b3 = sgpr_f(c[3]);
#pragma unroll
            for (int m = 0; m < MQ; ++m) {
                const int t = lane + 64 * m;
                float e = t < 8 * T2 ? elu_f(fmaf(g3, xh[j][m], b3)) : 0.f;
                e = sum8_hi(e);
                if ((lane & 7) == 7 && t < 8 * T2) Hs[j * T2 + (t >> 3)] = e * 0.125f;
            }
        }
        wave_lds_fence();
        TRACE_PH(g, 2, 2, tph_);
        float hv[NFQ], kp[NFQ];
#pragma unroll
        for (int u = 0; u < NFQ; ++u) {
            const int i = lane + 64 * u;
            kp[u] = i < NF ? keep_mul(g, mask3, dk1, (unsigned)(b * NF + i)) : 0.f;
            hv[u] = i < NF ? Hs[i] * kp[u] : 0.f;
        }
        float lg[NCLS];
#pragma unroll
        for (int n = 0; n < NCLS; ++n) {
            float a = 0.f;
#pragma unroll
            for (int u = 0; u < NFQ; ++u) a = fmaf(wf[n][u], hv[u], a);
            lg[n] = a;
        }
        wave_reduce<NCLS>(lg);
        float L[NCLS];
#pragma unroll
        for (int n = 0; n < NCLS; ++n) L[n] = readlane_f(lg[0], 16 * n) + prm[g.o_bfc + n];
        if ((mode & PC_LOGITS) && lane < NCLS)
            logits[(size_t)b * NCLS + lane] = lane == 0 ? L[0] : lane == 1 ? L[1] : lane == 2 ? L[2] : L[3];
        if (mode & PC_BWD) {
            float dl[NCLS];
            if (mode & PC_CE) {
                const float mx = fmaxf(fmaxf(L[0], L[1]), fmaxf(L[2], L[3]));
                float se = 0.f;
#pragma unroll
                for (int n = 0; n < NCLS; ++n) se += expf(L[n] - mx);
                const float lse = mx + logf(se);
                const int y = (int)labels[fold_row(perm, row0, b)];
                const float Ly = y == 0 ? L[0] : y == 1 ? L[1] : y == 2 ? L[2] : L[3];
                lossacc += lse - Ly;
#pragma unroll
                for (int n = 0; n < NCLS; ++n) dl[n] = (expf(L[n] - lse) - (n == y ? 1.f : 0.f)) * invB;
                if (lane < NCLS)
                    dlout[(size_t)b * NCLS + lane] = lane == 0 ? dl[0] : lane == 1 ? dl[1] : lane == 2 ? dl[2] : dl[3];
            } else {
#pragma unroll
                for (int n = 0; n < NCLS; ++n) dl[n] = dlin[(size_t)b * NCLS + n];
            }
#pragma unroll
            for (int n = 0; n < NCLS; ++n) {
                bacc[n] += dl[n];
#pragma unroll
                for (int u = 0; u < NFQ; ++u) wacc[n][u] = fmaf(dl[n], hv[u], wacc[n][u]);
            }
#pragma unroll
            for (int u = 0; u < NFQ; ++u) {
                const int i = lane + 64 * u;
                float d = 0.f;
#pragma unroll
                for (int n = 0; n < NCLS; ++n) d = fmaf(dl[n], wf[n][u], d);
                if (i < NF) Hs[i] = d * kp[u];
            }
            wave_lds_fence();
            TRACE_PH(g, 2, 3, tph_);
#pragma unroll
            for (int j = 0; j < F2MAX; ++j) {
                if (j >= F2) continue;
                const floatx4 c = lds_ld4(Ct + 4 * j);
                const float g3 = sgpr_f(c[2]), b3 = sgpr_f(c[3]);
#pragma unroll
                for (int m = 0; m < MQ; ++m) {
                    const int t = lane + 64 * m;
                    if (t < 8 * T2) {
                        const float dz = Hs[j * T2 + (t >> 3)] * 0.125f * elu_d(fmaf(g3, xh[j][m], b3));
                        sdz[j] += dz;
                        sdz[F2MAX + j] = fmaf(dz, xh[j][m], sdz[F2MAX + j]);
                    }
                }
            }
        }
        wave_lds_fence();
        TRACE_PH(g, 2, 4, tph_);
    }
    TRACE_LOOP(g, 2);
    if (!(mode & PC_BWD)) return;
    __syncthreads();
    TRACE_PS(g, 8);
    float* red = sm;
    float* rw = red + wave * g.nC;
#pragma unroll
    for (int n = 0; n < NCLS; ++n)
#pragma unroll
        for (int u = 0; u < NFQ; ++u) {
            const int i = lane + 64 * u;
            if (i < NF) rw[n * NF + i] = wacc[n][u];
        }
    wave_reduce<2 * F2MAX>(sdz);
    TRACE_PS(g, 9);
    if ((lane & 15) == 0) {
        const int r0 = (lane >> 4) * (F2MAX / 2);
#pragma unroll
        for (int j = 0; j < F2MAX / 2; ++j) {
            const int idx = j + r0;
            if (idx < F2MAX) { if (idx < F2) rw[NCLS * NF + NCLS + idx] = sdz[j]; }
            else if (idx - F2MAX < F2) rw[NCLS * NF + NCLS + F2 + idx - F2MAX] = sdz[j];
        }
    }
    if (lane == 0) {
#pragma unroll
        for (int n = 0; n < NCLS; ++n) rw[NCLS * NF + n] = bacc[n];
        rw[NCLS * NF + NCLS + 2 * F2] = lossacc;
    }
    __syncthreads();
    TRACE_PS(g, 10);
    float* row = part + (size_t)blockIdx.x * g.nC;
    for (int c = tid; c < g.nC; c += blockDim.x) pub(row + c, wave_rows_sum<NTH / 64>(red, nw, g.nC, c));
    TRACE_PS(g, 11);
    double* dsm = (double*)sm;
    if (grid_reduce(g, part, g.nC, fa, dsm)) { fin3(g, prm, dsm + 2, fa); TRACE(g, 2, TR_FIN); }
}

template <int K1, int CC, int TT, int FF, bool FOLD = false>
__global__ __launch_bounds__(TT ? NTH : NTHS) void k_pass_c(Geo g, const float* __restrict__ prm,
                                                const float* coef,
                                                const float* __restrict__ r3g,
                                                const uint8_t* __restrict__ mask3,
                                                const float* __restrict__ dlin,
                                                const int64_t* __restrict__ labels,
                                                float* __restrict__ logits, float* __restrict__ dlout,
                                                float* __restrict__ part, int mode, FinArgs fa, FoldCall fc) {
    extern __shared__ __attribute__((aligned(16))) float sm[];
    pass_c_body<K1, CC, TT, FF, FOLD>(g, prm, coef, r3g, mask3, dlin, labels, logits, dlout, part, mode, fa, fc, sm);
}

#if EEGNET_D1
template <int K1, int CC, int TT, int FF, bool FOLD = false, bool MASK = true>
__global__ __launch_bounds__(NTHS) void k_pass_d(Geo g, const float* __restrict__ prm,
                                                 const float* coef,
                                                 const float* __restrict__ d2g,
                                                 const float* __restrict__ E1g,
                                                 const float* __restrict__ E2g,
                                                 const float* __restrict__ q3g,
                                                 const float* __restrict__ r3g,
                                                 const uint8_t* __restrict__ mask2,
                                                 const uint8_t* __restrict__ mask3,
                                                 const float* __restrict__ dl,
                                                 float* __restrict__ dp2g, float* __restrict__ part,
                                                 FinArgs fa, FoldCall fc) {
    EEG_DIMS(g);
    TRACE(g, 3, TR_ENTRY);
    unsigned dk0, dk1;
    if (FOLD) {
        const eegnet_fold f = fold_rec(fc);
        char* ws = (char*)f.ws;
        prm = f.params;
        coef = (const float*)(ws + fc.off.coef);
        d2g = (const float*)(ws + fc.off.d2);
        E1g = (const float*)(ws + fc.off.E1); E2g = (const float*)(ws + fc.off.E2);
        q3g = (const float*)(ws + fc.off.q3); r3g = (const float*)(ws + fc.off.r3);
        mask2 = nullptr; mask3 = nullptr;
        dl = (const float*)(ws + fc.off.dl);
        dp2g = (float*)(ws + fc.off.dp2);
        part = (float*)(ws + fc.off.partD);
        fa = fold_fin(fc, f, TK_D, 0, 0, false, false, g.nparam);
        dk0 = fold_drop_key(fc, f, 0);
        dk1 = fold_drop_key(fc, f, 1);
    } else {
        dk0 = drop_key(g, 0);
        dk1 = drop_key(g, 1);
    }
    if constexpr (!MASK) { mask2 = nullptr; mask3 = nullptr; }
    constexpr int MQ = TT ? (TT / 4 + 63) / 64 : MAXT1Q;
    constexpr int NFQ = (TT && FF) ? (FF * (TT / 32) + 63) / 64 : MAXNFQ;
    const int RSW = TT ? row_stride_b2(TT / 4) : g.RSW;
    const int NFP = rup4(NF);
    const int nw = blockDim.x >> 6;
    extern __shared__ __attribute__((aligned(16))) float sm[];
    const int tid = threadIdx.x, lane = tid & 63;
    const int li = lane & 15, lk = lane >> 4;
    const int wave = __builtin_amdgcn_readfirstlane(tid >> 6);
    float* P0 = sm + wave * (3 * F2 * RSW + NFP);
    float* P1 = P0 + F2 * RSW;
    float* P2 = P1 + F2 * RSW;
    float* Hs = P2 + F2 * RSW;

    for (int i = lane; i < 3 * F2 * RSW; i += 64) P0[i] = 0.f;
    float wf[NCLS][NFQ];
#pragma unroll
    for (int n = 0; n < NCLS; ++n)
#pragma unroll
        for (int u = 0; u < NFQ; ++u) {
            const int i = lane + 64 * u;
            wf[n][u] = i < NF ? prm[g.o_Wfc + n * NF + i] : 0.f;
        }
    floatx4 acc3 = {0.f, 0.f, 0.f, 0.f};
    const int o2 = lane >> 2, kq = lane & 3;
    float acc2[4] = {0.f, 0.f, 0.f, 0.f};
    float sz[2 * F2MAX];
#pragma unroll
    for (int j = 0; j < 2 * F2MAX; ++j) sz[j] = 0.f;
    const int nkg = (T1 + 15) >> 4, ntq = (T1 + 3) >> 2;
    wave_lds_fence();

    TRACE(g, 3, TR_PRO);
    TRACE_DECL();
    drain_prologue_loads();
    float dlv[NCLS];
    float d[F2MAX][MQ], q[F2MAX][MQ], r[F2MAX][MQ];
    auto load_trial = [&](int bb) {
#pragma unroll
        for (int n = 0; n < NCLS; ++n) dlv[n] = dl[(size_t)bb * NCLS + n];
        load_rows<MQ>(d2g, bb, F2, T1, lane, d);
        load_rows<MQ>(q3g, bb, F2, T1, lane, q);
        load_rows<MQ>(r3g, bb, F2, T1, lane, r);
    };
    const int bstep = gridDim.x * nw;
    if (blockIdx.x * nw + wave < g.B) load_trial(blockIdx.x * nw + wave);
    for (int b = blockIdx.x * nw + wave; b < g.B; b += bstep) {
#pragma unroll
        for (int o = 0; o < F2MAX; ++o)
#pragma unroll
            for (int m = 0; m < MQ; ++m) {
                const int t = lane + 64 * m;
                if (o < F2 && t < T1) P0[o * RSW + LPD + t] = d[o][m];
            }
#pragma unroll
        for (int u = 0; u < NFQ; ++u) {
            const int i = lane + 64 * u;
            float dd = 0.f;
#pragma unroll
            for (int n = 0; n < NCLS; ++n) dd = fmaf(dlv[n], wf[n][u], dd);
            if (i < NF) Hs[i] = dd * keep_mul(g, mask3, dk1, (unsigned)(b * NF + i));
        }
        TRACE_PH(g, 3, 0, tph_);
#pragma unroll
        for (int o = 0; o < F2MAX; ++o)
#pragma unroll
            for (int m = 0; m < MQ; ++m) {
                const int t = lane + 64 * m;
                if (o < F2 && t < T1) P1[o * RSW + LPQ + t] = q[o][m];
            }
        wave_lds_fence();
        TRACE_PH(g, 3, 1, tph_);
        float dr[F2MAX][MQ];
        {
            float xh[F2MAX][MQ];
            bn3_rows<MQ>(coef, F2, r, xh);
#pragma unroll
            for (int j = 0; j < F2MAX; ++j) {
                if (j < F2) {
                    const int oz = opaque0();
                    const float g3 = prm[g.o_g3 + j + oz], b3 = prm[g.o_b3 + j + oz];
                    const float A3 = coef[CF_A3 * CSTR + j + oz], B3 = coef[CF_B3 * CSTR + j + oz];
                    const float C3 = coef[CF_C3 * CSTR + j + oz];
#pragma unroll
                    for (int m = 0; m < MQ; ++m) {
                        const int t = lane + 64 * m;
                        const float dz = t < 8 * T2 ? Hs[j * T2 + (t >> 3)] * 0.125f * elu_d(fmaf(g3, xh[j][m], b3)) : 0.f;
                        dr[j][m] = t < T1 ? fmaf(A3, dz, fmaf(C3, xh[j][m], B3)) : 0.f;
                        if (t < T1) P2[j * RSW + LPQ + t] = dr[j][m];
                    }
                } else {
#pragma unroll
                    for (int m = 0; m < MQ; ++m) dr[j][m] = 0.f;
                }
            }
        }
        wave_lds_fence();
        TRACE_PH(g, 3, 2, tph_);
        float e1v[F2MAX][MQ], e2v[F2MAX][MQ];
        load_rows<MQ>(E1g, b, F2, T1, lane, e1v);
        load_rows<MQ>(E2g, b, F2, T1, lane, e2v);
        if (b + bstep < g.B) load_trial(b + bstep);
        {
            const bool on = li < F2;
            const float* ar = P2 + (on ? li : 0) * RSW + LPQ + 2 * lk;
            const float* br = P1 + (on ? li : 0) * RSW + LPQ + 2 * lk;
            for (int kg = 0; kg < nkg; ++kg) {
                floatx2 a0 = lds_ld2(ar + 16 * kg), a1 = lds_ld2(ar + 16 * kg + 8);
                floatx2 b0 = lds_ld2(br + 16 * kg), b1 = lds_ld2(br + 16 * kg + 8);
                if (!on) { a0 = (floatx2){0.f, 0.f}; a1 = a0; b0 = a0; b1 = a0; }
                acc3 = __builtin_amdgcn_mfma_f32_16x16x4f32(a0[0], b0[0], acc3, 0, 0, 0);
                acc3 = __builtin_amdgcn_mfma_f32_16x16x4f32(a0[1], b0[1], acc3, 0, 0, 0);
                acc3 = __builtin_amdgcn_mfma_f32_16x16x4f32(a1[0], b1[0], acc3, 0, 0, 0);
                acc3 = __builtin_amdgcn_mfma_f32_16x16x4f32(a1[1], b1[1], acc3, 0, 0, 0);
            }
        }
        wave_lds_fence();
        TRACE_PH(g, 3, 3, tph_);
        float dq[F2MAX][MQ];
#pragma unroll
        for (int i = 0; i < F2MAX; ++i) {
            if (i < F2) {
                const int oz = i >= 2 ? opaque0_after(dq[i >= 2 ? i - 2 : 0][0]) : opaque0();
                const float* w3c = prm + (g.o_W3 + i + oz);
#pragma unroll
                for (int m = 0; m < MQ; ++m) {
                    const int t = lane + 64 * m;
                    float a = 0.f;
#pragma unroll
                    for (int j = 0; j < F2MAX; ++j)
                        if (j < F2) a = fmaf(w3c[j * F2], dr[j][m], a);
                    dq[i][m] = a;
                    if (t < T1) P1[i * RSW + LPQ + t] = a;
                }
            } else {
#pragma unroll
                for (int m = 0; m < MQ; ++m) dq[i][m] = 0.f;
            }
        }
        wave_lds_fence();
        TRACE_PH(g, 3, 4, tph_);
        if (o2 < F2) {
            const float* dqr = P1 + o2 * RSW + LPQ;
            const float* d2r = P0 + o2 * RSW + 4 * kq;
            for (int tq = 0; tq < ntq; ++tq) {
                const floatx4 a4 = lds_ld4(dqr + 4 * tq);
                const floatx4 w0 = lds_ld4(d2r + 4 * tq), w1 = lds_ld4(d2r + 4 * tq + 4);
                const float w[8] = {w0[0], w0[1], w0[2], w0[3], w1[0], w1[1], w1[2], w1[3]};
#pragma unroll
                for (int kk = 0; kk < 4; ++kk)
#pragma unroll
                    for (int i = 0; i < 4; ++i) acc2[kk] = fmaf(a4[i], w[i + kk], acc2[kk]);
            }
        }
        TRACE_PH(g, 3, 5, tph_);
        const size_t rb = (size_t)b * F2 * T1;
#pragma unroll
        for (int o = 0; o < F2MAX; ++o) {
            if (o >= F2) continue;
            float a[MQ];
            const int oz = o >= 2 ? opaque0_after(sz[o >= 2 ? o - 2 : 0]) : opaque0();
            conv16_same_t<MQ>(dq[o], prm + (g.o_w2 + o * K2 + oz), a, lane);
#pragma unroll
            for (int m = 0; m < MQ; ++m) {
                const int t = lane + 64 * m;
                if (t < T1) {
                    const int gi = o * T1 + t;
                    const float dp = a[m] * keep_mul(g, mask2, dk0, (unsigned)(rb + gi));
                    st_pol<EEGNET_NT_MID>(dp, dp2g + rb + gi);
                    sz[o] = fmaf(dp * 0.25f, e1v[o][m], sz[o]);
                    sz[F2MAX + o] = fmaf(dp * 0.25f, e2v[o][m], sz[F2MAX + o]);
                }
            }
        }
        wave_lds_fence();
        TRACE_PH(g, 3, 6, tph_);
    }
    TRACE_LOOP(g, 3);
    __syncthreads();
    float* red = sm;
    float* rw = red + wave * g.nD;
#pragma unroll
    for (int r = 0; r < 4; ++r) {
        const int j = 4 * lk + r;
        if (j < F2 && li < F2) rw[j * F2 + li] = acc3[r];
    }
    if (o2 < F2) {
#pragma unroll
        for (int kk = 0; kk < 4; ++kk) rw[F2 * F2 + o2 * K2 + 4 * kq + kk] = acc2[kk];
    }
    wave_reduce<2 * F2MAX>(sz);
    if ((lane & 15) == 0) {
        const int r0 = (lane >> 4) * (F2MAX / 2);
#pragma unroll
        for (int j = 0; j < F2MAX / 2; ++j) {
            const int idx = j + r0;
            if (idx < F2MAX) { if (idx < F2) rw[F2 * F2 + 16 * F2 + idx] = sz[j]; }
            else if (idx - F2MAX < F2) rw[F2 * F2 + 17 * F2 + idx - F2MAX] = sz[j];
        }
    }
    __syncthreads();
    float* row = part + (size_t)blockIdx.x * g.nD;
    for (int c = tid; c < g.nD; c += blockDim.x) pub(row + c, wave_rows_sum<NTHS / 64>(red, nw, g.nD, c));
    double* dsm = (double*)sm;
    if (grid_reduce(g, part, g.nD, fa, dsm)) { fin4(g, prm, dsm + 2, fa); TRACE(g, 3, TR_FIN); }
}
#endif

__host__ __device__ constexpr int dr_stride(int MQ) { return 64 * MQ + 2; }
__host__ __device__ constexpr int dr_lds_floats(int MQ) { return 4 * F2MAX * dr_stride(MQ) + F2MAX * (F2MAX + K2); }
__host__ __device__ constexpr int dr_tail_floats(bool hankel) { return NWB * 256 + 18 * F2MAX + (hankel ? NWB * RPW * 2 * 256 : 0); }

template <int K1, int CC, int TT, int FF, bool FOLD = false, bool MASK = true>
__global__ __launch_bounds__(NTB, TT ? WPEB : 2) void k_pass_dr(Geo g, const float* __restrict__ prm,
                                                  const float* coef,
                                                  const float* __restrict__ d2g,
                                                  const float* __restrict__ E1g,
                                                  const float* __restrict__ E2g,
                                                  const float* __restrict__ q3g,
                                                  const float* __restrict__ r3g,
                                                  const uint8_t* __restrict__ mask2,
                                                  const uint8_t* __restrict__ mask3,
                                                  const float* __restrict__ dl,
                                                  float* __restrict__ dp2g, float* __restrict__ part,
                                                  FinArgs fa, FoldCall fc) {
    EEG_DIMS_NT(g, NTB);
    TRACE(g, 3, TR_ENTRY);
    unsigned dk0, dk1;
    if (FOLD) {
        const eegnet_fold f = fold_rec(fc);
        char* ws = (char*)f.ws;
        prm = f.params;
        coef = (const float*)(ws + fc.off.coef);
        d2g = (const float*)(ws + fc.off.d2);
        E1g = (const float*)(ws + fc.off.E1); E2g = (const float*)(ws + fc.off.E2);
        q3g = (const float*)(ws + fc.off.q3); r3g = (const float*)(ws + fc.off.r3);
        mask2 = nullptr; mask3 = nullptr;
        dl = (const float*)(ws + fc.off.dl);
        dp2g = (float*)(ws + fc.off.dp2);
        part = (float*)(ws + fc.off.partD);
        fa = fold_fin(fc, f, TK_D, 0, 0, false, false, g.nparam);
        dk0 = fold_drop_key(fc, f, 0);
        dk1 = fold_drop_key(fc, f, 1);
    } else {
        dk0 = drop_key(g, 0);
        dk1 = drop_key(g, 1);
    }
    if constexpr (!MASK) { mask2 = nullptr; mask3 = nullptr; }
    constexpr int MQ = TT ? (TT / 4 + 63) / 64 : MAXT1Q;
    constexpr int RSD = dr_stride(MQ);
    constexpr int NKS = TT ? (TT / 4 + 3) / 4 : 16 * MAXT1Q;
    extern __shared__ __attribute__((aligned(16))) float sm[];
    float* const DR0 = sm;
    float* const Q0 = DR0 + 2 * F2MAX * RSD;
    float* const W3t = Q0 + 2 * F2MAX * RSD;
    float* const W2t = W3t + F2MAX * F2MAX;
    const int tid = threadIdx.x, lane = tid & 63;
    const int li = lane & 15, lk = lane >> 4;
    const int wave = __builtin_amdgcn_readfirstlane(tid >> 6);
    int b0, b1;
    trial_range(g, b0, b1);
    const int nks = TT ? NKS : (T1 + 3) >> 2;
    constexpr bool FULL = TT && FF == F2MAX && TT / 4 == 64 * MQ;

    float sr[2][RPW][MQ], sq[2][RPW][MQ], sd[2][RPW][MQ], se1[2][RPW][MQ], se2[2][RPW][MQ];
    floatx4 sdl[2];
    auto row_base = [&](int bb, int r) {
        const int o = RPW * wave + r;
        return (size_t)bb * F2 * T1 + (size_t)((FULL || o < F2) ? o * T1 : 0);
    };
    auto lane_off = [&](int r, int m, bool& ok) {
        const int o = RPW * wave + r, t = lane + 64 * m;
        ok = FULL || (o < F2 && t < T1);
        return ok ? t : 0;
    };
    auto load_rq = [&](int bb, float (&xr)[RPW][MQ], float (&xq)[RPW][MQ], floatx4& xdl) {
#pragma unroll
        for (int r = 0; r < RPW; ++r)
#pragma unroll
            for (int m = 0; m < MQ; ++m) {
                bool ok;
                const int i = lane_off(r, m, ok);
                const size_t rb_ = row_base(bb, r);
                const float vr = (r3g + rb_)[i], vq = (q3g + rb_)[i];
                xr[r][m] = ok ? vr : 0.f;
                xq[r][m] = ok ? vq : 0.f;
            }
        xdl = ldc(reinterpret_cast<const floatx4*>(dl) + bb);
    };
    auto load_de = [&](int bb, float (&xd)[RPW][MQ], float (&x1)[RPW][MQ], float (&x2)[RPW][MQ]) {
#pragma unroll
        for (int r = 0; r < RPW; ++r)
#pragma unroll
            for (int m = 0; m < MQ; ++m) {
                bool ok;
                const int i = lane_off(r, m, ok);
                const size_t rb_ = row_base(bb, r);
                const float vd = (d2g + rb_)[i], v1 = (E1g + rb_)[i], v2 = (E2g + rb_)[i];
                xd[r][m] = ok ? vd : 0.f;
                x1[r][m] = ok ? v1 : 0.f;
                x2[r][m] = ok ? v2 : 0.f;
            }
    };

    for (int i = tid; i < F2MAX * (F2MAX + K2); i += NTB) {
        float v = 0.f;
        if (i < F2MAX * F2MAX) {
            const int ii = i / F2MAX, j = i - ii * F2MAX;
            if (ii < F2 && j < F2) v = prm[g.o_W3 + j * F2 + ii];
        } else {
            const int k = i - F2MAX * F2MAX, o = k / K2;
            if (o < F2) v = prm[g.o_w2 + k];
        }
        W3t[i] = v;
    }
    if (F2 < F2MAX)
        for (int i = tid; i < 4 * (F2MAX - F2) * RSD; i += NTB) {
            const int buf = i / ((F2MAX - F2) * RSD), k = i - buf * ((F2MAX - F2) * RSD);
            DR0[buf * F2MAX * RSD + F2 * RSD + k] = 0.f;
        }
    float g3[RPW], b3[RPW], mu3[RPW], inv3[RPW], A3[RPW], B3[RPW], C3[RPW];
    float wfl[RPW][MQ][NCLS];
#pragma unroll
    for (int r = 0; r < RPW; ++r) {
        const int o = RPW * wave + r, oo = (FULL || o < F2) ? o : 0;
        const bool on = FULL || o < F2;
        g3[r] = on ? ldc(prm + g.o_g3 + oo) : 0.f;
        b3[r] = on ? ldc(prm + g.o_b3 + oo) : 0.f;
        mu3[r] = on ? ldc(coef + CF_MU3 * CSTR + oo) : 0.f;
        inv3[r] = on ? ldc(coef + CF_INV3 * CSTR + oo) : 0.f;
        A3[r] = on ? ldc(coef + CF_A3 * CSTR + oo) : 0.f;
        B3[r] = on ? ldc(coef + CF_B3 * CSTR + oo) : 0.f;
        C3[r] = on ? ldc(coef + CF_C3 * CSTR + oo) : 0.f;
#pragma unroll
        for (int m = 0; m < MQ; ++m) {
            const int t = lane + 64 * m;
            const bool ft = on && t < 8 * T2;
#pragma unroll
            for (int n = 0; n < NCLS; ++n) wfl[r][m][n] = ft ? prm[g.o_Wfc + n * NF + oo * T2 + (t >> 3)] : 0.f;
        }
    }
    floatx4 acc3 = {0.f, 0.f, 0.f, 0.f};
    floatx4 hq[RPW][2];
    float acc2[RPW][K2];
    float sz1[RPW], sz2[RPW];
#pragma unroll
    for (int r = 0; r < RPW; ++r) {
        sz1[r] = 0.f; sz2[r] = 0.f;
        hq[r][0] = acc3; hq[r][1] = acc3;
#pragma unroll
        for (int k = 0; k < K2; ++k) acc2[r][k] = 0.f;
    }
    const int blast = b1 > b0 ? b1 - 1 : b0;
#pragma unroll
    for (int k = 0; k < 2; ++k) {
        load_rq(min(b0 + k, blast), sr[k], sq[k], sdl[k]);
        load_de(min(b0 + k, blast), sd[k], se1[k], se2[k]);
    }
    barrier_lds();

    TRACE(g, 3, TR_PRO);
    TRACE_DECL();
    auto trial = [&](const int bt, const bool live, const int buf, float (&xr)[RPW][MQ], float (&xq)[RPW][MQ],
                     float (&xd)[RPW][MQ], float (&x1)[RPW][MQ], float (&x2)[RPW][MQ], floatx4& xdl) {
        const int b = min(bt, blast), bn = min(bt + 2, blast);
        float* DR = DR0 + buf * F2MAX * RSD;
        float* Qb = Q0 + buf * F2MAX * RSD;
        TRACE_PH(g, 3, 0, tph_);
        const floatx4 dlv = xdl;
#pragma unroll
        for (int r = 0; r < RPW; ++r) {
            const int o = RPW * wave + r;
            if (FULL || o < F2) {
#pragma unroll
                for (int m = 0; m < MQ; ++m) {
                    const int t = lane + 64 * m;
                    const float xh = (xr[r][m] - mu3[r]) * inv3[r];
                    float dd = 0.f;
#pragma unroll
                    for (int n = 0; n < NCLS; ++n) dd = fmaf(dlv[n], wfl[r][m][n], dd);
                    const bool ft = t < 8 * T2;
                    const float kp = keep_mul(g, mask3, dk1, (unsigned)(b * NF + (ft ? o * T2 + (t >> 3) : 0)));
                    const float dz = ft ? dd * kp * 0.125f * elu_d(fmaf(g3[r], xh, b3[r])) : 0.f;
                    DR[o * RSD + t] = (FULL || t < T1) ? fmaf(A3[r], dz, fmaf(C3[r], xh, B3[r])) : 0.f;
                    Qb[o * RSD + t] = xq[r][m];
                }
            }
        }
        load_rq(bn, xr, xq, xdl);
        TRACE_PH(g, 3, 1, tph_);
        barrier_lds();
        TRACE_PH(g, 3, 2, tph_);
        for (int ks = wave; ks < nks; ks += NWB) {
            const float a = DR[li * RSD + 4 * ks + lk], bq = Qb[li * RSD + 4 * ks + lk];
            acc3 = __builtin_amdgcn_mfma_f32_16x16x4f32(live ? a : 0.f, bq, acc3, 0, 0, 0);
        }
        float dq[RPW][MQ];
        {
            float dv[F2MAX][MQ];
#pragma unroll
            for (int j = 0; j < F2MAX; ++j)
#pragma unroll
                for (int m = 0; m < MQ; ++m) dv[j][m] = j < F2 ? DR[j * RSD + lane + 64 * m] : 0.f;
#pragma unroll
            for (int r = 0; r < RPW; ++r) {
                const int o = RPW * wave + r, oo = (FULL || o < F2) ? o : 0;
                float w3r[F2MAX];
#pragma unroll
                for (int q4 = 0; q4 < F2MAX / 4; ++q4) {
                    const floatx4 w = lds_ld4(W3t + oo * F2MAX + 4 * q4);
                    w3r[4 * q4] = sgpr_f(w[0]); w3r[4 * q4 + 1] = sgpr_f(w[1]);
                    w3r[4 * q4 + 2] = sgpr_f(w[2]); w3r[4 * q4 + 3] = sgpr_f(w[3]);
                }
#pragma unroll
                for (int m = 0; m < MQ; ++m) {
                    float a = 0.f;
#pragma unroll
                    for (int j = 0; j < F2MAX; ++j)
                        if (j < F2) a = fmaf(w3r[j], dv[j][m], a);
                    dq[r][m] = a;
                }
            }
        }
        TRACE_PH(g, 3, 3, tph_);
        const size_t rb = (size_t)b * F2 * T1;
#pragma unroll
        for (int r = 0; r < RPW; ++r) {
            const int o = RPW * wave + r;
            if (!FULL && o >= F2) continue;
            if constexpr (FULL) {
                const float dqg = live ? dq[r][0] : 0.f;
                const int i0 = lane - 7, i1 = lane + 9;
                const float d0 = __builtin_bit_cast(float, __builtin_amdgcn_ds_bpermute(max(i0, 0) * 4, __builtin_bit_cast(int, xd[r][0])));
                const float d1 = __builtin_bit_cast(float, __builtin_amdgcn_ds_bpermute(min(i1, 63) * 4, __builtin_bit_cast(int, xd[r][0])));
                hq[r][0] = __builtin_amdgcn_mfma_f32_16x16x4f32(dqg, i0 >= 0 ? d0 : 0.f, hq[r][0], 0, 0, 0);
                hq[r][1] = __builtin_amdgcn_mfma_f32_16x16x4f32(dqg, i1 < 64 ? d1 : 0.f, hq[r][1], 0, 0, 0);
            } else {
                float s[MQ], dqg[MQ];
#pragma unroll
                for (int m = 0; m < MQ; ++m) {
                    dqg[m] = live ? dq[r][m] : 0.f;
                    s[m] = xd[r][m];
                    acc2[r][7] = fmaf(dqg[m], s[m], acc2[r][7]);
                }
#pragma unroll
                for (int k = 8; k < K2; ++k) {
                    shl1<MQ>(s, lane);
#pragma unroll
                    for (int m = 0; m < MQ; ++m) acc2[r][k] = fmaf(dqg[m], s[m], acc2[r][k]);
                }
#pragma unroll
                for (int m = 0; m < MQ; ++m) s[m] = xd[r][m];
#pragma unroll
                for (int k = 6; k >= 0; --k) {
                    shr1<MQ>(s, lane);
#pragma unroll
                    for (int m = 0; m < MQ; ++m) acc2[r][k] = fmaf(dqg[m], s[m], acc2[r][k]);
                }
            }
            float w2r[K2];
#pragma unroll
            for (int q4 = 0; q4 < K2 / 4; ++q4) {
                const floatx4 w = lds_ld4(W2t + o * K2 + 4 * q4);
                w2r[4 * q4] = sgpr_f(w[0]); w2r[4 * q4 + 1] = sgpr_f(w[1]);
                w2r[4 * q4 + 2] = sgpr_f(w[2]); w2r[4 * q4 + 3] = sgpr_f(w[3]);
            }
            float y[MQ];
            conv16_same_t2<MQ>(dq[r], w2r, y, lane);
#pragma unroll
            for (int m = 0; m < MQ; ++m) {
                const int t = lane + 64 * m;
                if (FULL || t < T1) {
                    const int gi = o * T1 + t;
                    const float dp = y[m] * keep_mul(g, mask2, dk0, (unsigned)(rb + gi));
                    st_pol<EEGNET_NT_MID>(dp, dp2g + rb + gi);
                    const float dpg = live ? dp * 0.25f : 0.f;
                    sz1[r] = fmaf(dpg, x1[r][m], sz1[r]);
                    sz2[r] = fmaf(dpg, x2[r][m], sz2[r]);
                }
            }
        }
        load_de(bn, xd, x1, x2);
        TRACE_PH(g, 3, 4, tph_);
    };
    for (int b = b0; b < b1; b += 2) {
        pace_prio(b - b0, b1 - b0);
        trial(b, true, 0, sr[0], sq[0], sd[0], se1[0], se2[0], sdl[0]);
        trial(b + 1, b + 1 < b1, 1, sr[1], sq[1], sd[1], se1[1], se2[1], sdl[1]);
    }
    TRACE_LOOP(g, 3);
    tail_prio();
    __syncthreads();
    float* red = sm;
    float* own = red + NWB * 256;
#pragma unroll
    for (int r = 0; r < 4; ++r) red[wave * 256 + (4 * lk + r) * 16 + li] = acc3[r];
    if constexpr (FULL) {
        float* hs = own + 18 * F2MAX + wave * (RPW * 2 * 256);
#pragma unroll
        for (int r = 0; r < RPW; ++r)
#pragma unroll
            for (int h = 0; h < 2; ++h)
#pragma unroll
                for (int i = 0; i < 4; ++i) hs[((r * 2 + h) * 16 + 4 * lk + i) * 16 + li] = hq[r][h][i];
        wave_lds_fence();
        if (lane < RPW * K2) {
            const int r = lane / K2, k = lane % K2;
            float a = 0.f;
#pragma unroll
            for (int u = 0; u < 16; ++u) {
                const int w = u + k;
                a += hs[((r * 2 + (w >> 4)) * 16 + u) * 16 + (w & 15)];
            }
            own[(RPW * wave + r) * K2 + k] = a;
        }
        float v[4] = {sz1[0], sz1[1], sz2[0], sz2[1]};
        wave_reduce<4>(v);
        if ((lane & 15) == 0) {
            const int q = lane >> 4;
            own[F2 * K2 + (q >> 1) * F2 + RPW * wave + (q & 1)] = v[0];
        }
    } else {
        constexpr int NV = RPW * K2 + 2 * RPW;
        float v[NV];
#pragma unroll
        for (int r = 0; r < RPW; ++r) {
#pragma unroll
            for (int k = 0; k < K2; ++k) v[r * K2 + k] = acc2[r][k];
            v[RPW * K2 + r] = sz1[r];
            v[RPW * K2 + RPW + r] = sz2[r];
        }
        wave_reduce<NV>(v);
        if ((lane & 15) == 0) {
            const int q = lane >> 4;
#pragma unroll
            for (int j = 0; j < NV / 4; ++j) {
                const int item = j + (NV / 4) * q;
                if (item < RPW * K2) {
                    const int o = RPW * wave + item / K2;
                    if (o < F2) own[o * K2 + item % K2] = v[j];
                } else {
                    const int e = item - RPW * K2, o = RPW * wave + (e % RPW);
                    if (o < F2) own[F2 * K2 + (e / RPW) * F2 + o] = v[j];
                }
            }
        }
    }
    __syncthreads();
    float* row = part + (size_t)blockIdx.x * g.nD;
    for (int c = tid; c < g.nD; c += NTB) {
        float val;
        if (c < F2 * F2) {
            const int j = c / F2, i = c - j * F2;
            val = wave_rows_sum<NWB>(red, NWB, 256, j * 16 + i);
        } else {
            val = own[c - F2 * F2];
        }
        pub(row + c, val);
    }
    double* dsm = (double*)sm;
    if (grid_reduce(g, part, g.nD, fa, dsm)) { fin4(g, prm, dsm + 2, fa); TRACE(g, 3, TR_FIN); }
}

template <int K1, int KS_>
struct InferOps {
    float aw[KS_];
    float tap[K1];
    float w2[K2], w3[F2MAX];
    float al, be, s3, b3;
};

template <bool SC>
__device__ __forceinline__ float ld_w(const float* p) {
    if constexpr (SC) return ldc(p);
    else return *p;
}

template <int K1, int CC, int TT, int FF, bool SC, int KS_>
__device__ __forceinline__ void infer_ops_load(const Geo& g, const float* __restrict__ prm,
                                               const float* __restrict__ bn, int wave, int lane,
                                               InferOps<K1, KS_>& w) {
    EEG_DIMS(g);
    static_assert(KS_ == KS, "InferOps: k-steps of the spatial fragment");
    const float* rm1 = bn;                 const float* rv1 = bn + g.F1;
    const float* rm2 = bn + 2 * g.F1;      const float* rv2 = rm2 + F2;
    const float* rm3 = rm2 + 2 * F2;     const float* rv3 = rm3 + F2;
    load_ws_frag<KS>(prm + g.o_ws, C, F2, w.aw, lane);
    const int o = wave;
    const int oo = o < F2 ? o : 0, gg = oo / g.D;
#pragma unroll
    for (int k = 0; k < K1; ++k) w.tap[k] = ld_w<SC>(prm + (g.o_w1 + gg * K1 + k));
#pragma unroll
    for (int k = 0; k < K2; ++k) w.w2[k] = ld_w<SC>(prm + (g.o_w2 + oo * K2 + k));
#pragma unroll
    for (int i = 0; i < F2MAX; ++i) w.w3[i] = i < F2 ? ld_w<SC>(prm + (g.o_W3 + oo * F2 + i)) : 0.f;
    {
        const float a1 = ld_w<SC>(prm + (g.o_g1 + gg)) / sqrtf(ld_w<SC>(rv1 + gg) + g.eps);
        const float c1 = ld_w<SC>(prm + (g.o_b1 + gg)) - a1 * ld_w<SC>(rm1 + gg);
        float W = 0.f;
        for (int c = 0; c < C; ++c) W += ld_w<SC>(prm + (g.o_ws + oo * C + c));
        const float s2 = ld_w<SC>(prm + (g.o_g2 + oo)) / sqrtf(ld_w<SC>(rv2 + oo) + g.eps);
        w.al = a1 * s2;
        w.be = (c1 * W - ld_w<SC>(rm2 + oo)) * s2 + ld_w<SC>(prm + (g.o_b2 + oo));
        w.s3 = ld_w<SC>(prm + (g.o_g3 + oo)) / sqrtf(ld_w<SC>(rv3 + oo) + g.eps);
        w.b3 = ld_w<SC>(prm + (g.o_b3 + oo)) - ld_w<SC>(rm3 + oo) * w.s3;
    }
}

template <int K1, int CC, int TT, int FF, int KS_, int PF_, typename Out>
__device__ __forceinline__ void infer_trial(const Geo& g, const float* __restrict__ prm,
                                            const InferOps<K1, KS_>& w, float* sm,
                                            const float* __restrict__ xn, float (&pf)[PF_], int tid, int wave,
                                            int lane, Out&& out) {
    using G_ = KG<K1>;
    EEG_DIMS(g);
    static_assert(KS_ == KS && PF_ == PF, "infer_trial: fragment / prefetch sizes of this shape");
    float* const Xb0 = sm;
    float* Ss = sm + C * RS;
    float* D2s = Ss + F2 * RS;
    float* Qs = D2s + F2 * RS2;
    float* Hs = Qs + F2 * RS2;
    const int o = wave;
    const bool row_on = o < F2;
    if (xn) x_prefetch<PF>(xn, C, T, pf, tid);
    spatial_mfma<KS>(Xb0, w.aw, Ss, C, F2, NT16, RS, LP, wave, lane);
    __syncthreads();
    if (row_on) {
        const float* row = Ss + o * RS;
        float* drow = D2s + o * RS2 + LP2;
        for (int q = lane; q < T1; q += 64) {
            float win[4 * G_::NW];
            lds_window<G_::NW>(row + 4 * q, win);
            float v[4];
            fir4<K1, G_::OFF>(win, w.tap, v);
            float pe = 0.f;
#pragma unroll
            for (int i = 0; i < 4; ++i) pe += elu_f(fmaf(w.al, v[i], w.be));
            drow[q] = pe * 0.25f;
        }
    }
    if (xn) x_store<PF>(pf, C, T, RS, LP, Xb0, tid);
    __syncthreads();
    float r[MAXT1Q];
    block2_rows(F2, T1, RS2, D2s, Qs, w.w2, w.w3, row_on, o, lane, r);
#pragma unroll
    for (int m = 0; m < MAXT1Q; ++m) {
        const int t = lane + 64 * m;
        float e = (row_on && t < 8 * T2) ? elu_f(fmaf(w.s3, r[m], w.b3)) : 0.f;
        e += dpp<0xB1>(e);
        e += dpp<0x4E>(e);
        e += dpp<0x141>(e);
        if (row_on && (t & 7) == 0 && t < 8 * T2) Hs[o * T2 + (t >> 3)] = e * 0.125f;
    }
    __syncthreads();
    if (wave < NCLS) {
        const int n = wave;
        float a = 0.f;
        for (int i = lane; i < NF; i += 64) a = fmaf(prm[g.o_Wfc + n * NF + i], Hs[i], a);
        a = wave_sum(a);
        if (lane == 0) out(n, a + prm[g.o_bfc + n]);
    }
    __syncthreads();
}

template <int K1, int CC, int TT, int FF>
__global__ __launch_bounds__(NTH) void k_infer(Geo g, const float* __restrict__ prm,
                                               const float* __restrict__ bn,
                                               const float* __restrict__ x, float* __restrict__ logits) {
    EEG_DIMS(g);
    TRACE(g, 5, TR_ENTRY);
    extern __shared__ __attribute__((aligned(16))) float sm[];
    float* const Xb0 = sm;
    const int tid = threadIdx.x, lane = tid & 63;
    const int wave = __builtin_amdgcn_readfirstlane(tid >> 6);

    for (int i = tid; i < (C + F2) * RS + 2 * F2 * RS2; i += NTH) sm[i] = 0.f;
    InferOps<K1, KS> w;
    infer_ops_load<K1, CC, TT, FF, false>(g, prm, bn, wave, lane, w);
    float pf[PF];
    if ((int)blockIdx.x < g.B) x_prefetch<PF>(x + (size_t)blockIdx.x * C * T, C, T, pf, tid);
    __syncthreads();
    x_store<PF>(pf, C, T, RS, LP, Xb0, tid);
    __syncthreads();

    TRACE(g, 5, TR_PRO);
    drain_prologue_loads();
    for (int b = blockIdx.x; b < g.B; b += gridDim.x) {
        const int bnx = b + gridDim.x;
        const float* xn = bnx < g.B ? x + (size_t)bnx * C * T : nullptr;
        infer_trial<K1, CC, TT, FF>(g, prm, w, sm, xn, pf, tid, wave, lane,
                                    [&](int n, float l) { logits[(size_t)b * NCLS + n] = l; });
    }
}

}
```

eegnetreplication_amd/csrc/eegnet_stream.hip:

```cpp

namespace eeg {

constexpr int NTB = 512;
constexpr int NWB = NTB / 64;
constexpr int RPW = F2MAX / NWB;
constexpr int WGPC = 2;
constexpr int WPEB = NWB * WGPC / 4;

__device__ __forceinline__ int fir_row(int lane) { return (lane >> 3) & 1; }
__device__ __forceinline__ int fir_oct(int lane) { return (lane & 7) | ((lane >> 4) << 3); }
#define EEG_XP(TT, g) (((TT) && ((TT) & 3) == 0) ? (TT) : (g).XP)
#define EEG_NO(TT) ((TT) ? ((TT) + 7) / 8 : ((T + 7) >> 3))
#define EEG_MO(TT) ((TT) ? (((TT) + 7) / 8 + 31) / 32 : 4)

typedef __attribute__((address_space(1))) void gvoid_t;
typedef __attribute__((address_space(3))) void lvoid_t;
__device__ __forceinline__ void x_dma(const float* __restrict__ xb, int C, int T, int RS, int LP, float* Xs,
                                      int wave, int lane) {
    if ((T & 255) == 0) {
        const int np = T >> 8;
        for (int i = wave; i < C * np; i += NWB) {
            const int c = i / np, p = i - c * np;
            __builtin_amdgcn_global_load_lds((gvoid_t*)(xb + (size_t)c * T + 256 * p + 4 * lane),
                                             (lvoid_t*)(Xs + c * RS + LP + 256 * p), 16, 0, 0);
// ... 329 lines not shown
#pragma unroll
            for (int i = 0; i < 4; ++i) a[i] = (4 * q + i < T) ? w[G_::OFF + i] : 0.f;
            s0 += (a[0] + a[1]) + (a[2] + a[3]);
#pragma unroll
            for (int d = 0; d < K1; ++d) {
                float acc = G0[d];
#pragma unroll
                for (int i = 0; i < 4; ++i) acc = fmaf(a[i], w[G_::OFF + i + d], acc);
                G0[d] = acc;
            }
        }
#pragma unroll
        for (int i = 0; i < NEIX; ++i) {
            if (ea[i] >= 0) {
                const float* xa = Xb + LP + ea[i];
                float acc0 = 0.f, acc1 = 0.f;
                if (eb[i] >= 0) {
                    const float* xb2 = Xb + LP + eb[i];
                    int c = 0;
                    for (; c + 1 < C; c += 2) {
                        acc0 = fmaf(xa[c * RS], xb2[c * RS], acc0);
                        acc1 = fmaf(xa[(c + 1) * RS], xb2[(c + 1) * RS], acc1);
                    }
                    if (c < C) acc0 = fmaf(xa[c * RS], xb2[c * RS], acc0);
                } else {
                    int c = 0;
                    for (; c + 1 < C; c += 2) { acc0 += xa[c * RS]; acc1 += xa[(c + 1) * RS]; }
                    if (c < C) acc0 += xa[c * RS];
                }
                eacc[i] += acc0 + acc1;
            }
        }
        }
        TRACE_PH(g, 0, 0, tph_);
        barrier_lds();
        if constexpr (!XDMA)
            if (bn < b1) x_prefetch<PF, NTB>(x + fold_row(perm, row0, bn) * (C * XP), C, T, pf, tid);
        TRACE_PH(g, 0, 1, tph_);
        if (EEGNET_LDSX_A != 5) s_rows_store<NTB>(Ss, sg + (size_t)b * F2 * s_pitch(T), F2, T, RS, LP, tid);
        const int hr = fir_row(lane), o = RPW * wave + hr;
        float* const vrow = vg + ((size_t)b * F2 + (o < F2 ? o : 0)) * (8 * NO);
        constexpr bool DEFER = XDMA;
        constexpr int MOA = DEFER ? EEG_MO(TT) : 1;
        float vs[MOA][8];
        {
            float tl[K1];
            half_taps<K1, NTS>(tap, hr, tl);
            if (o < F2) {
                const float* row = Ss + o * RS;
                if constexpr (DEFER) {
                    constexpr bool TAIL1 = TT && (TT % 8 == 1) && (EEG_NO(TT) % 32 == 1);
#pragma unroll
                    for (int m = 0; m < MOA; ++m) {
                        const int oc = fir_oct(lane) + 32 * m;
                        if (oc < NO) {
                            float w[4 * G_::NW8];
                            if (EEGNET_LDSX_A == 6) {
#pragma unroll
                                for (int i = 0; i < 4 * G_::NW8; ++i) w[i] = 0.001f * (oc + i);
                            } else
                                lds_window<G_::NW8>(row + 8 * oc, w);
                            if (TAIL1 && m == MOA - 1) {
                                float a = 0.f;
#pragma unroll
                                for (int k = 0; k < K1; ++k) a = fmaf(tl[k], w[G_::OFF + k], a);
                                vs[m][0] = a;
#pragma unroll
                                for (int i = 1; i < 8; ++i) vs[m][i] = 0.f;
                                svl += a;
                                sv2l = fmaf(a, a, sv2l);
                            } else {
                                fir8<K1, G_::OFF>(w, tl, vs[m]);
#pragma unroll
                                for (int i = 0; i < 8; ++i)
                                    if (8 * oc + i < T) { svl += vs[m][i]; sv2l = fmaf(vs[m][i], vs[m][i], sv2l); }
                            }
                        }
                    }
                } else {
                    for (int oc = fir_oct(lane); oc < NO; oc += 32) {
                        float w[4 * G_::NW8];
                        lds_window<G_::NW8>(row + 8 * oc, w);
                        float v[8];
                        fir8<K1, G_::OFF>(w, tl, v);
#pragma unroll
                        for (int i = 0; i < 8; ++i)
                            if (8 * oc + i < T) { svl += v[i]; sv2l = fmaf(v[i], v[i], sv2l); }
                        st_pol<EEGNET_NT_SV>((floatx4){v[0], v[1], v[2], v[3]}, reinterpret_cast<floatx4*>(vrow + 8 * oc));
                        st_pol<EEGNET_NT_SV>((floatx4){v[4], v[5], v[6], v[7]}, reinterpret_cast<floatx4*>(vrow + 8 * oc + 4));
                    }
                }
            }
        }
        TRACE_PH(g, 0, 2, tph_);
        if constexpr (!XDMA)
            if (bn < b1) x_store<PF, NTB>(pf, C, T, RS, LP, Xb, tid);
        TRACE_PH(g, 0, 3, tph_);
        constexpr int NSST = (TT && FF) ? imax(0, (FF * (s_pitch(TT) / 4)) / NTB) : 0;
        static_assert(NSST <= 16, "vmcnt window");
        if constexpr (XDMA) barrier_vm<NSST>();
        else __syncthreads();
        if constexpr (DEFER) {
            if (o < F2) {
#pragma unroll
                for (int m = 0; m < MOA; ++m) {
                    const int oc = fir_oct(lane) + 32 * m;
                    if (oc < NO) {
                        st_pol<EEGNET_NT_SV>((floatx4){vs[m][0], vs[m][1], vs[m][2], vs[m][3]}, reinterpret_cast<floatx4*>(vrow + 8 * oc));
                        st_pol<EEGNET_NT_SV>((floatx4){vs[m][4], vs[m][5], vs[m][6], vs[m][7]}, reinterpret_cast<floatx4*>(vrow + 8 * oc + 4));
                    }
                }
            }
        }
        TRACE_PH(g, 0, 4, tph_);
    }
    TRACE_LOOP(g, 0);
    tail_prio();

    float* row = part + (size_t)blockIdx.x * g.nA;
    {
        constexpr int NR = K1 + 8, NQ = NR / 4;
        float rv[NR];
#pragma unroll
        for (int d = 0; d < K1; ++d) rv[d] = G0[d];
        rv[K1] = s0;
#pragma unroll
        for (int r = 0; r < RPW; ++r) {
            rv[K1 + 1 + r] = fir_row(lane) == r ? svl : 0.f;
            rv[K1 + 1 + RPW + r] = fir_row(lane) == r ? sv2l : 0.f;
        }
#pragma unroll
        for (int i = K1 + 1 + 2 * RPW; i < NR; ++i) rv[i] = 0.f;
        wave_reduce<NR>(rv);
        if ((lane & 15) == 0) {
            const int r0 = (lane >> 4) * NQ;
#pragma unroll
            for (int j = 0; j < NQ; ++j) {
                const int idx = j + r0;
                if (idx <= K1) {
                    red[wave * (K1 + 1) + idx] = rv[j];
                } else if (idx < K1 + 1 + 2 * RPW) {
                    const int k = idx - K1 - 1, r = k % RPW, o = RPW * wave + r;
                    if (o < F2) pub(row + (K1 + 1 + g.nedge + (k < RPW ? 0 : F2) + o), rv[j]);
                }
            }
        }
    }
    __syncthreads();
    if (FOLD && xst) {
#pragma unroll
        for (int k = 0; k < NXI; ++k) {
            const int c = tid + NTB * k;
            if (c < NV) pub(row + c, xacc[k]);
        }
    } else {
    if (tid <= K1) {
        float t = 0.f;
        for (int w = 0; w < NWB; ++w) t += red[w * (K1 + 1) + tid];
        pub(row + (tid), t);
    }
    if constexpr (LAGM) {
        constexpr int R_ = G_::R, P_ = G_::P, nH_ = R_ * (R_ + 1) / 2, nTl_ = P_ * (P_ + 1) / 2;
        if (wave == EW_H || wave == EW_T) {
            const int n = lane & 15, E = wave == EW_H ? R_ : P_;
            const int base = K1 + 1 + (wave == EW_H ? 0 : nH_);
#pragma unroll
            for (int r = 0; r < 4; ++r) {
                const int m = 4 * (lane >> 4) + r;
                if (m <= n && n < E) pub(row + (base + m * E - m * (m - 1) / 2 + (n - m)), egram[r]);
            }
        } else if (wave == EW_S && lane < R_ + P_) {
            pub(row + (K1 + 1 + nH_ + nTl_ + lane), esum);
        }
    } else {
#pragma unroll
    for (int i = 0; i < NEIX; ++i)
        if (ea[i] != -2 && tid + NTB * i < g.nedge) pub(row + (K1 + 1 + tid + NTB * i), eacc[i]);
    }
    }
    {
        double* dsm = (double*)sm;
        Fin1Stage f1;
        if (!g.defer) fin1_load(g, prm, fa, f1);
        if (grid_reduce(g, part, g.nA, fa, dsm)) {
            fin1_body<K1, true>(g, prm, dsm + 2, dsm + tail_s_doubles(g.nA), fa, f1);
            TRACE(g, 0, TR_FIN);
        }
    }
}

template <int K1, int CC, int TT, int FF, bool FOLD = false>
__global__ __launch_bounds__(NTB, WPEB) void k_pass_a(Geo g, const float* __restrict__ prm,
                                                      const float* __restrict__ x, float* __restrict__ sg,
                                                      float* __restrict__ vg, float* __restrict__ part,
                                                      FinArgs fa, FoldCall fc) {
    extern __shared__ __attribute__((aligned(16))) float sm[];
    pass_a_body<K1, CC, TT, FF, FOLD>(g, prm, x, sg, vg, part, fa, fc, sm);
}

template <int K1>
__global__ __launch_bounds__(NTB) void k_xstats(Geo g, long long n, const float* __restrict__ x,
                                                float* __restrict__ out) {
    using G_ = KG<K1>;
    constexpr int NEI = G_::template nei<NTB>();
    const int C = g.C, T = g.T, RS = g.RS, XP = g.XP, TQ = (T + 3) >> 2;
    constexpr int LP = G_::LP;
    const int NV = K1 + 1 + g.nedge;
    extern __shared__ __attribute__((aligned(16))) float sm[];
    float* const Xb = sm;
    float* const red = sm + C * RS;
    const int tid = threadIdx.x, lane = tid & 63;
    const int wave = __builtin_amdgcn_readfirstlane(tid >> 6);
    for (int i = tid; i < C * RS; i += NTB) Xb[i] = 0.f;
    int ea[NEI], eb[NEI];
#pragma unroll
    for (int i = 0; i < NEI; ++i) {
        int e = tid + NTB * i;
        ea[i] = -2; eb[i] = -1;
        if (e < g.nH) {
            int a = 0;
            while (e >= g.R - a) { e -= g.R - a; ++a; }
            ea[i] = a; eb[i] = a + e;
        } else if ((e -= g.nH) < g.nTl) {
            int u = 0;
            while (e >= g.P - u) { e -= g.P - u; ++u; }
            ea[i] = T - g.P + u; eb[i] = T - g.P + u + e;
        } else if ((e -= g.nTl) < g.R) {
            ea[i] = e;
        } else if ((e -= g.R) < g.P) {
            ea[i] = T - g.P + e;
        }
    }
    for (long long b = blockIdx.x; b < n; b += gridDim.x) {
        __syncthreads();
        const float* xb = x + (size_t)b * C * XP;
        for (int i = tid; i < C * T; i += NTB) {
            const int c = i / T, t = i - c * T;
            Xb[c * RS + LP + t] = xb[(size_t)c * XP + t];
        }
        __syncthreads();
        float G0[K1];
#pragma unroll
        for (int d = 0; d < K1; ++d) G0[d] = 0.f;
        float s0 = 0.f;
        for (int j = tid; j < C * TQ; j += NTB) {
            const int c = j / TQ, q = j - c * TQ;
            float w[4 * G_::NW];
            lds_window<G_::NW>(Xb + c * RS + 4 * q, w);
            float a[4];
#pragma unroll
            for (int i = 0; i < 4; ++i) a[i] = (4 * q + i < T) ? w[G_::OFF + i] : 0.f;
            s0 += (a[0] + a[1]) + (a[2] + a[3]);
#pragma unroll
            for (int d = 0; d < K1; ++d) {
                float acc = G0[d];
#pragma unroll
                for (int i = 0; i < 4; ++i) acc = fmaf(a[i], w[G_::OFF + i + d], acc);
                G0[d] = acc;
            }
        }
        float* orow = out + (size_t)b * NV;
#pragma unroll
        for (int i = 0; i < NEI; ++i) {
            if (ea[i] >= 0) {
                const float* xa = Xb + LP + ea[i];
                float acc = 0.f;
                if (eb[i] >= 0) {
                    const float* xb2 = Xb + LP + eb[i];
                    for (int c = 0; c < C; ++c) acc = fmaf(xa[c * RS], xb2[c * RS], acc);
                } else {
                    for (int c = 0; c < C; ++c) acc += xa[c * RS];
                }
                orow[K1 + 1 + tid + NTB * i] = acc;
            }
        }
        constexpr int NR = (K1 + 1 + 3) & ~3, NQ = NR / 4;
        float rv[NR];
#pragma unroll
        for (int d = 0; d < K1; ++d) rv[d] = G0[d];
        rv[K1] = s0;
#pragma unroll
        for (int i = K1 + 1; i < NR; ++i) rv[i] = 0.f;
        wave_reduce<NR>(rv);
        if ((lane & 15) == 0) {
            const int r0 = (lane >> 4) * NQ;
#pragma unroll
            for (int j = 0; j < NQ; ++j)
                if (j + r0 <= K1) red[wave * (K1 + 1) + j + r0] = rv[j];
        }
        __syncthreads();
        if (tid <= K1) {
            float t = 0.f;
            for (int w = 0; w < NWB; ++w) t += red[w * (K1 + 1) + tid];
            orow[tid] = t;
        }
    }
}

template <int K1, int CC, int TT, int FF, bool FOLD>
__device__ __forceinline__ void pass_b_body(const Geo& g, const float* __restrict__ prm,
                                            const float* coef,
                                            const float* __restrict__ vg,
                                            const uint8_t* __restrict__ mask2,
                                            float* __restrict__ d2g, float* __restrict__ E1g,
                                            float* __restrict__ E2g, float* __restrict__ q3g,
                                            float* __restrict__ r3g, float* __restrict__ part,
                                            FinArgs fa, const FoldCall& fc, float* sm) {
    EEG_DIMS_NT(g, NTB);
    TRACE(g, 1, TR_ENTRY);
    unsigned dk0;
    if (FOLD) {
        const eegnet_fold f = fold_rec(fc);
        char* ws = (char*)f.ws;
        prm = f.params;
        coef = (const float*)(ws + fc.off.coef);
        vg = (const float*)(ws + fc.off.v);
        mask2 = nullptr;
        d2g = (float*)(ws + fc.off.d2); E1g = (float*)(ws + fc.off.E1); E2g = (float*)(ws + fc.off.E2);
        q3g = (float*)(ws + fc.off.q3); r3g = (float*)(ws + fc.off.r3);
        part = (float*)(ws + fc.off.partB);
        fa = fold_fin(fc, f, TK_B, 1, 0, true, false, g.nparam);
        dk0 = fold_drop_key(fc, f, 0);
    } else {
        dk0 = drop_key(g, 0);
    }
    float* D2s = sm;
    float* Qs0 = D2s + F2 * RS2;
    float* Wt = Qs0 + 2 * F2 * RS2;
    const int tid = threadIdx.x, lane = tid & 63;
    const int wave = __builtin_amdgcn_readfirstlane(tid >> 6);
    int b0, b1;
    trial_range(g, b0, b1);
    const int NO = EEG_NO(TT);
    constexpr int MO = EEG_MO(TT);
    const int hr = fir_row(lane), oh = RPW * wave + hr;
    constexpr bool VPF = TT != 0;
    float vpf[MO][8];
    if (VPF && b0 < b1) v_load<MO>(vg, b0, F2, NO, oh, lane, vpf);

    for (int i = tid; i < 3 * F2 * RS2; i += NTB) sm[i] = 0.f;
    for (int i = tid; i < F2MAX * (K2 + F2MAX); i += NTB) {
        float v = 0.f;
        if (i < F2MAX * K2) { if (i < F2 * K2) v = prm[g.o_w2 + i]; }
        else {
            const int j = (i - F2MAX * K2) / F2MAX, c = (i - F2MAX * K2) % F2MAX;
            if (j < F2 && c < F2) v = prm[g.o_W3 + j * F2 + c];
        }
        Wt[i] = v;
    }
    float sr[RPW], sr2[RPW];
#pragma unroll
    for (int r = 0; r < RPW; ++r) { sr[r] = 0.f; sr2[r] = 0.f; }
    float alh, beh, gah, bth;
    {
        const int oo = oh < F2 ? oh : 0;
        alh = coef[CF_AL2 * CSTR + oo]; beh = coef[CF_BE2 * CSTR + oo];
        gah = prm[g.o_g2 + oo]; bth = prm[g.o_b2 + oo];
    }
    __syncthreads();

    TRACE(g, 1, TR_PRO);
    TRACE_DECL();
    drain_prologue_loads();
    for (int b = b0; b < b1; ++b) {
        const int bn = b + 1;
        pace_prio(b - b0, b1 - b0);
        float* Qs = Qs0 + ((b - b0) & 1) * F2 * RS2;
        float vc[MO][8];
        if constexpr (VPF) {
#pragma unroll
            for (int m = 0; m < MO; ++m)
#pragma unroll
                for (int i = 0; i < 8; ++i) vc[m][i] = vpf[m][i];
            if (bn < b1) v_load<MO>(vg, bn, F2, NO, oh, lane, vpf);
        } else {
            v_load<MO>(vg, b, F2, NO, oh, lane, vc);
        }
        TRACE_PH(g, 1, 0, tph_);
        float d2v[MO][2], e1v[MO][2], e2v[MO][2];
        if (oh < F2) {
            float* drow = D2s + oh * RS2 + LP2;
#pragma unroll
            for (int m = 0; m < MO; ++m) {
                const int oc = fir_oct(lane) + 32 * m;
                if (oc >= NO) break;
#pragma unroll
                for (int h = 0; h < 2; ++h) {
                    const int q = 2 * oc + h;
                    float pe = 0.f, e1 = 0.f, e2 = 0.f;
#pragma unroll
                    for (int i = 4 * h; i < 4 * h + 4; ++i) {
                        const float xh = fmaf(alh, vc[m][i], beh);
                        const float z = fmaf(gah, xh, bth);
                        const float dz = elu_d(z);
                        pe += z > 0.f ? z : dz - 1.f;
                        e1 += dz;
                        e2 = fmaf(dz, xh, e2);
                    }
                    const float d2 = q < T1 ? pe * 0.25f * keep_mul(g, mask2, dk0, (unsigned)((b * F2 + oh) * T1 + q)) : 0.f;
                    d2v[m][h] = d2; e1v[m][h] = e1; e2v[m][h] = e2;
                    if (q < T1) drow[q] = d2;
                }
            }
        }
        wave_lds_fence();
        TRACE_PH(g, 1, 1, tph_);
#pragma unroll
        for (int r = 0; r < RPW; ++r) {
            const int o = RPW * wave + r;
            if (o < F2) {
                const float* dr = D2s + o * RS2 + LP2 - 7;
                const float* w2 = Wt + o * K2;
                for (int t = lane; t < T1; t += 64) {
                    float a = 0.f;
#pragma unroll
                    for (int k = 0; k < K2; ++k) a = fmaf(w2[k], dr[t + k], a);
                    Qs[o * RS2 + t] = a;
                    q3g[((size_t)b * F2 + o) * T1 + t] = a;
                }
            }
        }
        TRACE_PH(g, 1, 2, tph_);
        if (oh < F2) {
#pragma unroll
            for (int m = 0; m < MO; ++m) {
                const int oc = fir_oct(lane) + 32 * m;
                if (oc >= NO) break;
#pragma unroll
                for (int h = 0; h < 2; ++h) {
                    const int q = 2 * oc + h;
                    if (q < T1) {
                        const size_t gi = ((size_t)b * F2 + oh) * T1 + q;
                        st_pol<EEGNET_NT_MID>(d2v[m][h], d2g + gi); st_pol<EEGNET_NT_MID>(e1v[m][h], E1g + gi);
                        st_pol<EEGNET_NT_MID>(e2v[m][h], E2g + gi);
                    }
                }
            }
        }
        TRACE_PH(g, 1, 3, tph_);
        barrier_lds();
        TRACE_PH(g, 1, 4, tph_);
        for (int t = lane; t < T1; t += 64) {
            float qv[F2MAX];
#pragma unroll
            for (int i = 0; i < F2MAX; ++i) qv[i] = i < F2 ? Qs[i * RS2 + t] : 0.f;
#pragma unroll
            for (int r = 0; r < RPW; ++r) {
                const int o = RPW * wave + r;
                if (o < F2) {
                    const float* w3 = Wt + F2MAX * K2 + o * F2MAX;
                    float rr = 0.f;
#pragma unroll
                    for (int i = 0; i < F2MAX; ++i) rr = fmaf(w3[i], qv[i], rr);
                    r3g[((size_t)b * F2 + o) * T1 + t] = rr;
                    sr[r] += rr;
                    sr2[r] = fmaf(rr, rr, sr2[r]);
                }
            }
        }
        TRACE_PH(g, 1, 5, tph_);
    }
    TRACE_LOOP(g, 1);
    tail_prio();
    {
        float rv[4] = {sr[0], sr[1], sr2[0], sr2[1]};
        wave_reduce<4>(rv);
        const int k = lane >> 4, o = RPW * wave + (k & 1);
        if ((lane & 15) == 0 && o < F2) {
            float* row = part + (size_t)blockIdx.x * g.nB;
            pub(row + ((k < 2 ? 0 : F2) + o), rv[0]);
        }
    }
    {
        double* dsm = (double*)sm;
        if (grid_reduce(g, part, g.nB, fa, dsm)) { fin2(g, dsm + 2, fa); TRACE(g, 1, TR_FIN); }
    }
}

template <int K1, int CC, int TT, int FF, bool FOLD = false>
__global__ __launch_bounds__(NTB, WPEB) void k_pass_b(Geo g, const float* __restrict__ prm,
                                                      const float* coef,
                                                      const float* __restrict__ vg,
                                                      const uint8_t* __restrict__ mask2,
                                                      float* __restrict__ d2g, float* __restrict__ E1g,
                                                      float* __restrict__ E2g, float* __restrict__ q3g,
                                                      float* __restrict__ r3g, float* __restrict__ part,
                                                      FinArgs fa, FoldCall fc) {
    extern __shared__ __attribute__((aligned(16))) float sm[];
    pass_b_body<K1, CC, TT, FF, FOLD>(g, prm, coef, vg, mask2, d2g, E1g, E2g, q3g, r3g, part, fa, fc, sm);
}

#ifndef EEGNET_LDSX_E
#define EEGNET_LDSX_E 0
#endif
template <int K1, int CC, int TT, int FF, bool FOLD>
__device__ __forceinline__ void pass_e_body(const Geo& g, const float* prm,
                                            const float* coef,
                                            const float* __restrict__ x,
                                            const float* __restrict__ sg, const float* __restrict__ vg,
                                            const float* __restrict__ dp2g,
                                            float* __restrict__ part, FinArgs fa, const FoldCall& fc, float* sm) {
    using G_ = KG<K1>;
    EEG_DIMS_NT(g, NTB);
    const int XP = EEG_XP(TT, g);
    TRACE(g, 4, TR_ENTRY);
    const int64_t* perm = nullptr;
    long long row0 = 0;
    if (FOLD) {
        const eegnet_fold f = fold_rec(fc);
        char* ws = (char*)f.ws;
        prm = f.params;
        coef = (const float*)(ws + fc.off.coef);
        x = f.x;
        perm = f.perm; row0 = fc.row0;
        sg = (const float*)(ws + fc.off.s);
        vg = (const float*)(ws + fc.off.v);
        dp2g = (const float*)(ws + fc.off.dp2);
        part = (float*)(ws + fc.off.partE);
        fa = fold_fin(fc, f, TK_E, 0, 0, false, true, g.nparam);
    }
    constexpr int NTS = FF ? 1 : RPW;
    const int D = FF ? 2 : g.D;
    const int QR = FF ? FF / 2 : g.QR;
    float* const Ss = sm;
    float* const Dys = Ss + F2 * RS;
    float* const Xb = Dys + F2 * RS;
    float* const DP = Xb + C * RS;
    float* red = sm;
    const int tid = threadIdx.x, lane = tid & 63;
    const int wave = __builtin_amdgcn_readfirstlane(tid >> 6);
    int b0, b1;
    trial_range(g, b0, b1);
    const int li = lane & 15, lk = lane >> 4;
    constexpr bool XDMA = TT != 0;
    static_assert(!XDMA || (CC && FF), "LDS-DMA staging is specialised to compile-time C and F2");

    TRACE_PS(g, 0);
    if constexpr (!XDMA) zero_fill<false>(sm, (2 * F2 + C) * RS, F2, RS, LP, T, tid);
    TRACE_PS(g, 1);
    float tap[NTS][K1];
    float* CT = DP + ((F2 * T1 + 3) & ~3);
    const int NO = EEG_NO(TT);
    constexpr int MO = EEG_MO(TT);
    const int hr = fir_row(lane), oh = RPW * wave + hr;
    constexpr bool ONEOC = FF && TT && (EEG_NO(TT) <= 32) && (FF == RPW * NWB);
    constexpr bool EINPL = ONEOC || XDMA;
    float* const Eb = EINPL ? Dys : Ss;
    constexpr bool XDMA_ = TT != 0;
    constexpr bool DPDMA_ = XDMA_ && FF && ((FF * (TT / 4)) % 256 == 0);
    constexpr bool PIPEE = ONEOC && XDMA_ && DPDMA_ && (TT / 4 == 64) && (TT == 256);
    float sdyl = 0.f, sdyvl = 0.f;
    constexpr int NWT = (15 + K1 - 1) / 16 + 1;
    floatx4 cq[RPW][NWT];
#pragma unroll
    for (int r = 0; r < RPW; ++r)
#pragma unroll
        for (int j = 0; j < NWT; ++j) cq[r][j] = (floatx4){0.f, 0.f, 0.f, 0.f};
    const int wpc = NWB / NCT;
    const bool gemm_on = wave < wpc * NCT;
    const int ct = gemm_on ? wave / wpc : 0, part_ = gemm_on ? wave - ct * wpc : 0;
    const int kg0 = (NT16 * part_) / wpc, kg1 = gemm_on ? (NT16 * (part_ + 1)) / wpc : 0;
    floatx4 xacc = {0.f, 0.f, 0.f, 0.f};
    constexpr int MS = TT ? (TT + 63) / 64 : 16;
    float pws[XDMA ? 1 : RPW][XDMA ? 1 : MS];
    auto s_rows_load = [&](int bb) {
        if constexpr (!XDMA) {
#pragma unroll
            for (int r = 0; r < RPW; ++r) {
                const float* src = sg + ((size_t)bb * F2 + min(RPW * wave + r, F2 - 1)) * s_pitch(T);
#pragma unroll
                for (int k = 0; k < MS; ++k) pws[r][k] = src[min(lane + 64 * k, T - 1)];
            }
        }
    };
    auto s_rows_put = [&]() {
        if constexpr (!XDMA) {
#pragma unroll
            for (int r = 0; r < RPW; ++r) {
                const int o = RPW * wave + r;
#pragma unroll
                for (int k = 0; k < MS; ++k)
                    if (o < F2 && lane + 64 * k < T) Ss[o * RS + LP + lane + 64 * k] = pws[r][k];
            }
        }
    };
    float pfx[XDMA ? 1 : PF];
    constexpr bool VPF = XDMA;
    float vpf[MO][8];
    constexpr int NDP = (CC && TT) ? (FF * (TT / 4) + NTB - 1) / NTB : 8;
    const int ndp = F2 * T1;
    float pdp[NDP];
    constexpr bool DPDMA = TT && FF && ((FF * (TT / 4)) % 256 == 0);
    if (b0 < b1) {
        if constexpr (XDMA) s_dma_asm(sg + (size_t)b0 * F2 * s_pitch(T), F2, T, RS, LP, Ss, wave, lane);
        else s_rows_load(b0);
        TRACE_PS(g, 3);
        if constexpr (DPDMA) flat_dma_asm(dp2g + (size_t)b0 * ndp, ndp, DP, wave, lane);
        else {
#pragma unroll
            for (int j = 0; j < NDP; ++j) pdp[j] = dp2g[(size_t)b0 * ndp + min(tid + NTB * j, ndp - 1)];
#pragma unroll
            for (int j = 0; j < NDP; ++j)
                if (tid + NTB * j < ndp) DP[tid + NTB * j] = pdp[j];
            for (int i = tid + NTB * NDP; i < ndp; i += NTB) DP[i] = dp2g[(size_t)b0 * ndp + i];
        }
        if constexpr (VPF) v_load<MO>(vg, b0, F2, NO, oh, lane, vpf);
        TRACE_PS(g, 4);
    }
    if constexpr (XDMA) zero_pads(sm, 2 * F2 + C, RS, LP, T, tid);
    load_taps<K1, NTS>(g, prm, D, F2, wave, tap);
    TRACE_PS(g, 2);
    {
        float cv = 0.f;
#pragma unroll
        for (int k = 0; k < 8 * RPW; ++k) {
            const int o = RPW * wave + (k >> 3), f = k & 7;
            if (o < F2 && f < 7) {
                const float* src = f == 0 ? coef + CF_AL2 * CSTR : f == 1 ? coef + CF_BE2 * CSTR
                                 : f == 2 ? prm + g.o_g2 : f == 3 ? prm + g.o_b2 : f == 4 ? coef + CF_AO * CSTR
                                 : f == 5 ? coef + CF_BO * CSTR : coef + CF_CO * CSTR;
                const float v = ldc(src + o);
                cv = lane == k ? v : cv;
            }
        }
        if (lane < 8 * RPW && RPW * wave + (lane >> 3) < F2) CT[8 * RPW * wave + lane] = cv;
    }
    adam_scalars_publish(g, fa);
    const int step0 = adam_step0(g, fa);
    if constexpr (XDMA) barrier_vm<0>();
    else __syncthreads();
    if constexpr (!XDMA) {
        if (b0 < b1) {
            s_rows_put();
            x_prefetch<PF, NTB>(x + fold_row(perm, row0, b0) * (C * XP), C, T, pfx, tid);
            x_store<PF, NTB>(pfx, C, T, RS, LP, Xb, tid);
        }
        __syncthreads();
    }

    TRACE(g, 4, TR_PRO);
    TRACE_DECL();
    drain_prologue_loads();
    for (int b = b0; b < b1; ++b) {
        const int bn = b + 1;
        pace_prio(b - b0, b1 - b0);
        float vc[MO][8];
        if constexpr (VPF) {
#pragma unroll
            for (int m = 0; m < MO; ++m)
#pragma unroll
                for (int i = 0; i < 8; ++i) vc[m][i] = vpf[m][i];
            if constexpr (PIPEE)
                if (bn < b1) v_load<MO>(vg, bn, F2, NO, oh, lane, vpf);
        } else {
            v_load<MO>(vg, b, F2, NO, oh, lane, vc);
        }
        TRACE_PH(g, 4, 0, tph_);
        if (oh < F2) {
            float* drow = Dys + oh * RS + LP;
            const floatx4 c0 = lds_ld4(CT + 8 * oh), c1 = lds_ld4(CT + 8 * oh + 4);
            const float alh = c0[0], beh = c0[1], gah = c0[2], bth = c0[3];
            const float Aoh = c1[0], Boh = c1[1], Coh = c1[2];
#pragma unroll
            for (int m = 0; m < MO; ++m) {
                const int oc = fir_oct(lane) + 32 * m;
                if (oc >= NO) break;
                float dpq[2];
#pragma unroll
                for (int h = 0; h < 2; ++h)
                    dpq[h] = EEGNET_LDSX_E == 1 ? 0.01f * (oc + h) : (2 * oc + h < T1) ? DP[oh * T1 + 2 * oc + h] * 0.25f : 0.f;
                float dy[8];
#pragma unroll
                for (int i = 0; i < 8; ++i) {
                    const bool in = 8 * oc + i < T;
                    const float v = in ? vc[m][i] : 0.f;
                    const float xh = fmaf(alh, v, beh);
                    const float z = fmaf(gah, xh, bth);
                    const float dz = dpq[i >> 2] * elu_d(z);
                    float d = fmaf(Aoh, dz, fmaf(Coh, xh, Boh));
                    d = in ? d : 0.f;
                    dy[i] = d;
                    sdyl += d;
                    sdyvl = fmaf(d, v, sdyvl);
                }
                if (EEGNET_LDSX_E != 5)
                    lds_st_oct(drow + 8 * oc, oc, (floatx4){dy[0], dy[1], dy[2], dy[3]}, (floatx4){dy[4], dy[5], dy[6], dy[7]});
            }
        }
        TRACE_PH(g, 4, 1, tph_);
        wave_lds_fence();
        if constexpr (PIPEE) {
            if (bn < b1) {
#pragma unroll
                for (int r = 0; r < RPW; ++r) {
                    const int o = RPW * wave + r;
                    if (EEGNET_LDSX_E != 7) dma4(dp2g + (size_t)bn * ndp + o * T1 + lane, DP + o * T1);
                }
            }
        }
        if constexpr (XDMA)
            if (EEGNET_LDSX_E != 7) x_dma_asm(x + fold_row(perm, row0, b) * (C * XP), C, T, XP, RS, LP, Xb, wave, lane);
        TRACE_PH(g, 4, 2, tph_);
        {
            float tl[K1];
            half_taps<K1, NTS>(tap, hr, tl);
            if constexpr (ONEOC) {
                constexpr int NT16C = (TT + 15) / 16, KQC = (NT16C + 3) / 4, NQ = RPW * KQC * NWT;
                const int oc = fir_oct(lane);
                float w[4 * G_::NW8];
                if (EEGNET_LDSX_E == 2) {
#pragma unroll
                    for (int i = 0; i < 4 * G_::NW8; ++i) w[i] = 0.001f * (lane + i);
                } else
                    lds_window<G_::NW8>(Dys + oh * RS + 8 * oc, w);
                float e[8];
#pragma unroll
                for (int i = 0; i < 8; ++i) e[i] = 0.f;
#pragma unroll
                for (int m = 0; m < K1; ++m) {
#pragma unroll
                    for (int i = 0; i < 8; ++i) e[i] = fmaf(tl[K1 - 1 - m], w[G_::OFFD + i + m], e[i]);
#pragma unroll
                    for (int n = (m * NQ) / K1; n < ((m + 1) * NQ) / K1; ++n) {
                        const int r = n / (KQC * NWT), ks = (n / NWT) % KQC, j = n % NWT;
                        const int o = RPW * wave + r, a = 4 * ks + lk;
                        const bool on = a < NT16C;
                        const int ac = on ? a : 0;
                        float av = EEGNET_LDSX_E == 3 ? 0.01f * (li + n) : Dys[o * RS + LP + li + 16 * ac];
                        float bv = EEGNET_LDSX_E == 3 ? 0.02f * (lk + n) : Ss[o * RS + G_::OFF + li + 16 * (ac + j)];
                        av = on ? av : 0.f;
                        bv = on ? bv : 0.f;
                        cq[r][j] = __builtin_amdgcn_mfma_f32_16x16x4f32(av, bv, cq[r][j], 0, 0, 0);
                    }
                }
                float* erow = Dys + oh * RS + LP;
#pragma unroll
                for (int i = 0; i < 8; ++i) e[i] = (8 * oc + i < T) ? e[i] : 0.f;
                wave_lds_fence();
                if (EEGNET_LDSX_E != 6)
                    lds_st_oct(erow + 8 * oc, oc, (floatx4){e[0], e[1], e[2], e[3]}, (floatx4){e[4], e[5], e[6], e[7]});
                if constexpr (PIPEE) {
                    if (bn < b1 && EEGNET_LDSX_E != 7) {
#pragma unroll
                        for (int r = 0; r < RPW; ++r) {
                            const int o = RPW * wave + r;
                            dma16(sg + ((size_t)bn * F2 + o) * s_pitch(T) + 4 * lane, Ss + o * RS + LP);
                        }
                    }
                }
            } else {
                const int KQ = (NT16 + 3) >> 2;
#pragma unroll
                for (int r = 0; r < RPW; ++r) {
                    const int o = RPW * wave + r;
                    if (o < F2) {
                        const float* dyr = Dys + o * RS + LP + li;
                        const float* sr = Ss + o * RS + G_::OFF + li;
                        for (int ks = 0; ks < KQ; ++ks) {
                            const int a = 4 * ks + lk;
                            const bool on = a < NT16;
                            const int ac = on ? a : 0;
                            float av = dyr[16 * ac];
                            av = on ? av : 0.f;
#pragma unroll
                            for (int j = 0; j < NWT; ++j) {
                                float bv = sr[16 * (ac + j)];
                                bv = on ? bv : 0.f;
                                cq[r][j] = __builtin_amdgcn_mfma_f32_16x16x4f32(av, bv, cq[r][j], 0, 0, 0);
                            }
                        }
                    }
                }
                if constexpr (EINPL) {
                    float e[MO][8];
                    if (oh < F2) {
                        const float* dyr = Dys + oh * RS;
                        constexpr bool TAIL1 = TT && (TT % 8 == 1) && (EEG_NO(TT) % 32 == 1);
#pragma unroll
                        for (int m = 0; m < MO; ++m) {
                            const int oc = min(fir_oct(lane) + 32 * m, NO - 1);
                            float w[4 * G_::NW8];
                            lds_window<G_::NW8>(dyr + 8 * oc, w);
#pragma unroll
                            for (int i = 0; i < 8; ++i) e[m][i] = 0.f;
                            if (TAIL1 && m == MO - 1) {
#pragma unroll
                                for (int k = 0; k < K1; ++k) e[m][0] = fmaf(tl[K1 - 1 - k], w[G_::OFFD + k], e[m][0]);
                            } else {
#pragma unroll
                                for (int k = 0; k < K1; ++k)
#pragma unroll
                                    for (int i = 0; i < 8; ++i)
// ... 212 lines not shown
```

Baseline: 18.36 million trials/s.

## Recompute BN2/pool intermediates in backward pass instead of storing d2/E1/E2 planes

Pass B no longer writes the d2, E1 and E2 intermediate planes to global memory. Pass D (dr variant) now reads the raw v tensor and recomputes the BN2 affine, ELU derivative and pooling quantities through a shared helper. This trades three stored and reloaded planes for one 4x-wider v load plus extra ALU work. The unused D1 pass-D kernel variant is deleted, and a static_assert disables the B2 narrow path, which relied on those planes.

```diff
diff --git a/eegnetreplication_amd/csrc/eegnet_common.h b/eegnetreplication_amd/csrc/eegnet_common.h
--- a/eegnetreplication_amd/csrc/eegnet_common.h
+++ b/eegnetreplication_amd/csrc/eegnet_common.h
@@ -325,6 +325,23 @@
     return (h >> 8) >= g.pthr ? g.scale : 0.f;
 }
 
+__device__ __forceinline__ void bn2_pool4(float v0, float v1, float v2, float v3, float al, float be,
+                                          float ga, float bt, float keep, float& d2, float& e1, float& e2) {
+    const float v[4] = {v0, v1, v2, v3};
+    float pe = 0.f;
+    e1 = 0.f; e2 = 0.f;
+#pragma unroll
+    for (int i = 0; i < 4; ++i) {
+        const float xh = fmaf(al, v[i], be);
+        const float z = fmaf(ga, xh, bt);
+        const float dz = elu_d(z);
+        pe += z > 0.f ? z : dz - 1.f;
+        e1 += dz;
+        e2 = fmaf(dz, xh, e2);
+    }
+    d2 = pe * 0.25f * keep;
+}
+
 __device__ __forceinline__ void drain_prologue_loads() { __builtin_amdgcn_s_waitcnt(0); }
 
 template <int U, typename T>
diff --git a/eegnetreplication_amd/csrc/eegnet_host.hip b/eegnetreplication_amd/csrc/eegnet_host.hip
--- a/eegnetreplication_amd/csrc/eegnet_host.hip
+++ b/eegnetreplication_amd/csrc/eegnet_host.hip
@@ -52,11 +52,9 @@
 #ifndef EEGNET_B2
 #define EEGNET_B2 0
 #endif
+static_assert(EEGNET_B2 != 1, "EEGNET_B2=1: k_pass_b no longer stores the d2 / E1 / E2 planes k_wpass_d reads");
 static bool use_b2_narrow(const Geo&) { return EEGNET_B2 == 1; }
 
-#ifndef EEGNET_D1
-#define EEGNET_D1 0
-#endif
 
 #ifndef EEGNET_GRIDS_MULT
 #define EEGNET_GRIDS_MULT 1
@@ -138,8 +136,7 @@
     g->nwC = std::max(1, std::min(spec ? NWAVE : NTHS / 64, (LDS_MAX / 4 - 4 * F2MAX) / pwC));
     g->nwD = std::max(1, std::min(NTHS / 64, (LDS_MAX / 4) / pwD));
     g->ldsC = std::max(g->nwC * pwC + 4 * F2MAX, g->nwC * g->nC);
-    g->ldsD = EEGNET_D1 ? std::max(g->nwD * pwD, g->nwD * g->nD)
-                        : std::max(dr_lds_floats(spec ? 1 : MAXT1Q), dr_tail_floats(spec));
+    g->ldsD = std::max(dr_lds_floats(spec ? 1 : MAXT1Q), dr_tail_floats(spec));
     g->ldsE = std::max((2 * g->F2 + g->C) * g->RS + rup(g->F2 * g->T1, 4) + 8 * g->F2,
                        NWB * 256 * (1 + (15 + g->K1 - 1) / 16 + 1));
     g->ldsI = rows1 + g->F2 * g->RS + 2 * g->F2 * g->RS2 + nf4;
@@ -302,10 +299,6 @@
                           (const void*)k_pass_e<K1, CC, TT, FF>, (const void*)k_pass_a<K1, CC, TT, FF, true>,
                           (const void*)k_pass_b<K1, CC, TT, FF, true>, (const void*)k_pass_c<K1, CC, TT, FF, true>,
                           (const void*)k_pass_e<K1, CC, TT, FF, true>,
-#if EEGNET_D1
-                          (const void*)k_pass_d<K1, CC, TT, FF>, (const void*)k_pass_d<K1, CC, TT, FF, false, false>,
-                          (const void*)k_pass_d<K1, CC, TT, FF, true, false>,
-#endif
                           (const void*)k_pass_dr<K1, CC, TT, FF>, (const void*)k_pass_dr<K1, CC, TT, FF, false, false>,
                           (const void*)k_pass_dr<K1, CC, TT, FF, true, false>})
         hipFuncSetAttribute(f, hipFuncAttributeMaxDynamicSharedMemorySize, lds);
@@ -388,13 +381,13 @@
 static int grid_wpass_b(const Geo& g, bool sp) { return sp ? std::min(2 * g.gridS, g.B * g.NOC) : g.gridS; }
 static int grid_pass_c(const Geo& g) { return g.wide ? g.gridW2 : use_b2_narrow(g) ? g.gridB2 : g.grid; }
 static int grid_pass_d(const Geo& g) {
-    return g.wide ? g.grid : use_b2_narrow(g) ? g.gridB2 : EEGNET_D1 ? g.grid : g.gridS;
+    return g.wide ? g.grid : use_b2_narrow(g) ? g.gridB2 : g.gridS;
 }
 static int streams_pass_c(const Geo& g) {
     return grid_pass_c(g) * ((g.wide || use_b2_narrow(g)) ? 1 : g.nwC);
 }
 static int streams_pass_d(const Geo& g) {
-    return grid_pass_d(g) * ((g.wide || use_b2_narrow(g) || !EEGNET_D1) ? 1 : g.nwD);
+    return grid_pass_d(g);
 }
 
 template <int K1>
@@ -472,12 +465,12 @@
     if (only < 0 || only == 0) { { PROF(KID_A); EEG_DISPATCH(K1, g, LAUNCH_A);
     } LAUNCH_CHECK("k_pass_a"); }
 #define LAUNCH_B(K, CC, TT, FF) if (fc.folds) hipLaunchKernelGGL((k_pass_b<K, CC, TT, FF, true>), dim3(g.gridS, nf), dim3(NTB), g.ldsB * 4, s, \
-                       g, params, (const float*)(ws + L.coef), (const float*)(ws + L.v), m2, (float*)(ws + L.d2), \
-                       (float*)(ws + L.E1), (float*)(ws + L.E2), (float*)(ws + L.q3), (float*)(ws + L.r3), \
+                       g, params, (const float*)(ws + L.coef), (const float*)(ws + L.v), m2, \
+                       (float*)(ws + L.q3), (float*)(ws + L.r3), \
                        (float*)(ws + L.partB), fb, fc); \
     else hipLaunchKernelGGL((k_pass_b<K, CC, TT, FF>), dim3(g.gridS, nf), dim3(NTB), g.ldsB * 4, s, \
-                       g, params, (const float*)(ws + L.coef), (const float*)(ws + L.v), m2, (float*)(ws + L.d2), \
-                       (float*)(ws + L.E1), (float*)(ws + L.E2), (float*)(ws + L.q3), (float*)(ws + L.r3), \
+                       g, params, (const float*)(ws + L.coef), (const float*)(ws + L.v), m2, \
+                       (float*)(ws + L.q3), (float*)(ws + L.r3), \
                        (float*)(ws + L.partB), fb, fc)
     if (only < 0 || only == 1) { { PROF(KID_B); EEG_DISPATCH(K1, g, LAUNCH_B);
     } LAUNCH_CHECK("k_pass_b"); }
@@ -533,41 +526,21 @@
     if (only < 0 || only == 2) { { PROF(KID_C); EEG_DISPATCH(K1, g, LAUNCH_CB);
     } LAUNCH_CHECK("k_pass_c(bwd)"); }
 #define LAUNCH_DR(K, CC, TT, FF) if (fc.folds) hipLaunchKernelGGL((k_pass_dr<K, CC, TT, FF, true, false>), dim3(grid_pass_d(g), nf), dim3(NTB), g.ldsD * 4, s, \
-                       g, params, coef, (const float*)(ws + L.d2), (const float*)(ws + L.E1), \
-                       (const float*)(ws + L.E2), (const float*)(ws + L.q3), (const float*)(ws + L.r3), \
+                       g, params, coef, (const float*)(ws + L.v), (const float*)(ws + L.q3), \
+                       (const float*)(ws + L.r3), \
                        m2, m3, dl, (float*)(ws + L.dp2), \
                        (float*)(ws + L.partD), fd, fc); \
     else if (m2 || m3) hipLaunchKernelGGL((k_pass_dr<K, CC, TT, FF>), dim3(grid_pass_d(g), nf), dim3(NTB), g.ldsD * 4, s, \
-                       g, params, coef, (const float*)(ws + L.d2), (const float*)(ws + L.E1), \
-                       (const float*)(ws + L.E2), (const float*)(ws + L.q3), (const float*)(ws + L.r3), \
+                       g, params, coef, (const float*)(ws + L.v), (const float*)(ws + L.q3), \
+                       (const float*)(ws + L.r3), \
                        m2, m3, dl, (float*)(ws + L.dp2), \
                        (float*)(ws + L.partD), fd, fc); \
     else hipLaunchKernelGGL((k_pass_dr<K, CC, TT, FF, false, false>), dim3(grid_pass_d(g), nf), dim3(NTB), g.ldsD * 4, s, \
-                       g, params, coef, (const float*)(ws + L.d2), (const float*)(ws + L.E1), \
-                       (const float*)(ws + L.E2), (const float*)(ws + L.q3), (const float*)(ws + L.r3), \
+                       g, params, coef, (const float*)(ws + L.v), (const float*)(ws + L.q3), \
+                       (const float*)(ws + L.r3), \
                        m2, m3, dl, (float*)(ws + L.dp2), \
                        (float*)(ws + L.partD), fd, fc)
-#define LAUNCH_D(K, CC, TT, FF) if (fc.folds) hipLaunchKernelGGL((k_pass_d<K, CC, TT, FF, true, false>), dim3(grid_pass_d(g), nf), dim3(64 * g.nwD), g.ldsD * 4, s, \
-                       g, params, coef, (const float*)(ws + L.d2), (const float*)(ws + L.E1), \
-                       (const float*)(ws + L.E2), (const float*)(ws + L.q3), (const float*)(ws + L.r3), \
-                       m2, m3, dl, (float*)(ws + L.dp2), \
-                       (float*)(ws + L.partD), fd, fc); \
-    else if (m2 || m3) hipLaunchKernelGGL((k_pass_d<K, CC, TT, FF>), dim3(grid_pass_d(g), nf), dim3(64 * g.nwD), g.ldsD * 4, s, \
-                       g, params, coef, (const float*)(ws + L.d2), (const float*)(ws + L.E1), \
-                       (const float*)(ws + L.E2), (const float*)(ws + L.q3), (const float*)(ws + L.r3), \
-                       m2, m3, dl, (float*)(ws + L.dp2), \
-                       (float*)(ws + L.partD), fd, fc); \
-    else hipLaunchKernelGGL((k_pass_d<K, CC, TT, FF, false, false>), dim3(grid_pass_d(g), nf), dim3(64 * g.nwD), g.ldsD * 4, s, \
-                       g, params, coef, (const float*)(ws + L.d2), (const float*)(ws + L.E1), \
-                       (const float*)(ws + L.E2), (const float*)(ws + L.q3), (const float*)(ws + L.r3), \
-                       m2, m3, dl, (float*)(ws + L.dp2), \
-                       (float*)(ws + L.partD), fd, fc)
-#if EEGNET_D1
-#define LAUNCH_PASS_D LAUNCH_D
-#else
-#define LAUNCH_PASS_D LAUNCH_DR
-#endif
-    if (only < 0 || only == 3) { { PROF(KID_D); EEG_DISPATCH(K1, g, LAUNCH_PASS_D);
+    if (only < 0 || only == 3) { { PROF(KID_D); EEG_DISPATCH(K1, g, LAUNCH_DR);
     } LAUNCH_CHECK("k_pass_d"); }
     }
 #define LAUNCH_E(K, CC, TT, FF) if (fc.folds) hipLaunchKernelGGL((k_pass_e<K, CC, TT, FF, true>), dim3(g.gridE, nf), dim3(NTB), g.ldsE * 4, s, \
diff --git a/eegnetreplication_amd/csrc/eegnet_passes.hip b/eegnetreplication_amd/csrc/eegnet_passes.hip
--- a/eegnetreplication_amd/csrc/eegnet_passes.hip
+++ b/eegnetreplication_amd/csrc/eegnet_passes.hip
@@ -359,261 +359,14 @@
     pass_c_body<K1, CC, TT, FF, FOLD>(g, prm, coef, r3g, mask3, dlin, labels, logits, dlout, part, mode, fa, fc, sm);
 }
 
-#if EEGNET_D1
-template <int K1, int CC, int TT, int FF, bool FOLD = false, bool MASK = true>
-__global__ __launch_bounds__(NTHS) void k_pass_d(Geo g, const float* __restrict__ prm,
-                                                 const float* coef,
-                                                 const float* __restrict__ d2g,
-                                                 const float* __restrict__ E1g,
-                                                 const float* __restrict__ E2g,
-                                                 const float* __restrict__ q3g,
-                                                 const float* __restrict__ r3g,
-                                                 const uint8_t* __restrict__ mask2,
-                                                 const uint8_t* __restrict__ mask3,
-                                                 const float* __restrict__ dl,
-                                                 float* __restrict__ dp2g, float* __restrict__ part,
-                                                 FinArgs fa, FoldCall fc) {
-    EEG_DIMS(g);
-    TRACE(g, 3, TR_ENTRY);
-    unsigned dk0, dk1;
-    if (FOLD) {
-        const eegnet_fold f = fold_rec(fc);
-        char* ws = (char*)f.ws;
-        prm = f.params;
-        coef = (const float*)(ws + fc.off.coef);
-        d2g = (const float*)(ws + fc.off.d2);
-        E1g = (const float*)(ws + fc.off.E1); E2g = (const float*)(ws + fc.off.E2);
-        q3g = (const float*)(ws + fc.off.q3); r3g = (const float*)(ws + fc.off.r3);
-        mask2 = nullptr; mask3 = nullptr;
-        dl = (const float*)(ws + fc.off.dl);
-        dp2g = (float*)(ws + fc.off.dp2);
-        part = (float*)(ws + fc.off.partD);
-        fa = fold_fin(fc, f, TK_D, 0, 0, false, false, g.nparam);
-        dk0 = fold_drop_key(fc, f, 0);
-        dk1 = fold_drop_key(fc, f, 1);
-    } else {
-        dk0 = drop_key(g, 0);
-        dk1 = drop_key(g, 1);
-    }
-    if constexpr (!MASK) { mask2 = nullptr; mask3 = nullptr; }
-    constexpr int MQ = TT ? (TT / 4 + 63) / 64 : MAXT1Q;
-    constexpr int NFQ = (TT && FF) ? (FF * (TT / 32) + 63) / 64 : MAXNFQ;
-    const int RSW = TT ? row_stride_b2(TT / 4) : g.RSW;
-    const int NFP = rup4(NF);
-    const int nw = blockDim.x >> 6;
-    extern __shared__ __attribute__((aligned(16))) float sm[];
-    const int tid = threadIdx.x, lane = tid & 63;
-    const int li = lane & 15, lk = lane >> 4;
-    const int wave = __builtin_amdgcn_readfirstlane(tid >> 6);
-    float* P0 = sm + wave * (3 * F2 * RSW + NFP);
-    float* P1 = P0 + F2 * RSW;
-    float* P2 = P1 + F2 * RSW;
-    float* Hs = P2 + F2 * RSW;
-
-    for (int i = lane; i < 3 * F2 * RSW; i += 64) P0[i] = 0.f;
-    float wf[NCLS][NFQ];
-#pragma unroll
-    for (int n = 0; n < NCLS; ++n)
-#pragma unroll
-        for (int u = 0; u < NFQ; ++u) {
-            const int i = lane + 64 * u;
-            wf[n][u] = i < NF ? prm[g.o_Wfc + n * NF + i] : 0.f;
-        }
-    floatx4 acc3 = {0.f, 0.f, 0.f, 0.f};
-    const int o2 = lane >> 2, kq = lane & 3;
-    float acc2[4] = {0.f, 0.f, 0.f, 0.f};
-    float sz[2 * F2MAX];
-#pragma unroll
-    for (int j = 0; j < 2 * F2MAX; ++j) sz[j] = 0.f;
-    const int nkg = (T1 + 15) >> 4, ntq = (T1 + 3) >> 2;
-    wave_lds_fence();
-
-    TRACE(g, 3, TR_PRO);
-    TRACE_DECL();
-    drain_prologue_loads();
-    float dlv[NCLS];
-    float d[F2MAX][MQ], q[F2MAX][MQ], r[F2MAX][MQ];
-    auto load_trial = [&](int bb) {
-#pragma unroll
-        for (int n = 0; n < NCLS; ++n) dlv[n] = dl[(size_t)bb * NCLS + n];
-        load_rows<MQ>(d2g, bb, F2, T1, lane, d);
-        load_rows<MQ>(q3g, bb, F2, T1, lane, q);
-        load_rows<MQ>(r3g, bb, F2, T1, lane, r);
-    };
-    const int bstep = gridDim.x * nw;
-    if (blockIdx.x * nw + wave < g.B) load_trial(blockIdx.x * nw + wave);
-    for (int b = blockIdx.x * nw + wave; b < g.B; b += bstep) {
-#pragma unroll
-        for (int o = 0; o < F2MAX; ++o)
-#pragma unroll
-            for (int m = 0; m < MQ; ++m) {
-                const int t = lane + 64 * m;
-                if (o < F2 && t < T1) P0[o * RSW + LPD + t] = d[o][m];
-            }
-#pragma unroll
-        for (int u = 0; u < NFQ; ++u) {
-            const int i = lane + 64 * u;
-            float dd = 0.f;
-#pragma unroll
-            for (int n = 0; n < NCLS; ++n) dd = fmaf(dlv[n], wf[n][u], dd);
-            if (i < NF) Hs[i] = dd * keep_mul(g, mask3, dk1, (unsigned)(b * NF + i));
-        }
-        TRACE_PH(g, 3, 0, tph_);
-#pragma unroll
-        for (int o = 0; o < F2MAX; ++o)
-#pragma unroll
-            for (int m = 0; m < MQ; ++m) {
-                const int t = lane + 64 * m;
-                if (o < F2 && t < T1) P1[o * RSW + LPQ + t] = q[o][m];
-            }
-        wave_lds_fence();
-        TRACE_PH(g, 3, 1, tph_);
-        float dr[F2MAX][MQ];
-        {
-            float xh[F2MAX][MQ];
-            bn3_rows<MQ>(coef, F2, r, xh);
-#pragma unroll
-            for (int j = 0; j < F2MAX; ++j) {
-                if (j < F2) {
-                    const int oz = opaque0();
-                    const float g3 = prm[g.o_g3 + j + oz], b3 = prm[g.o_b3 + j + oz];
-                    const float A3 = coef[CF_A3 * CSTR + j + oz], B3 = coef[CF_B3 * CSTR + j + oz];
-                    const float C3 = coef[CF_C3 * CSTR + j + oz];
-#pragma unroll
-                    for (int m = 0; m < MQ; ++m) {
-                        const int t = lane + 64 * m;
-                        const float dz = t < 8 * T2 ? Hs[j * T2 + (t >> 3)] * 0.125f * elu_d(fmaf(g3, xh[j][m], b3)) : 0.f;
-                        dr[j][m] = t < T1 ? fmaf(A3, dz, fmaf(C3, xh[j][m], B3)) : 0.f;
-                        if (t < T1) P2[j * RSW + LPQ + t] = dr[j][m];
-                    }
-                } else {
-#pragma unroll
-                    for (int m = 0; m < MQ; ++m) dr[j][m] = 0.f;
-                }
-            }
-        }
-        wave_lds_fence();
-        TRACE_PH(g, 3, 2, tph_);
-        float e1v[F2MAX][MQ], e2v[F2MAX][MQ];
-        load_rows<MQ>(E1g, b, F2, T1, lane, e1v);
-        load_rows<MQ>(E2g, b, F2, T1, lane, e2v);
-        if (b + bstep < g.B) load_trial(b + bstep);
-        {
-            const bool on = li < F2;
-            const float* ar = P2 + (on ? li : 0) * RSW + LPQ + 2 * lk;
-            const float* br = P1 + (on ? li : 0) * RSW + LPQ + 2 * lk;
-            for (int kg = 0; kg < nkg; ++kg) {
-                floatx2 a0 = lds_ld2(ar + 16 * kg), a1 = lds_ld2(ar + 16 * kg + 8);
-                floatx2 b0 = lds_ld2(br + 16 * kg), b1 = lds_ld2(br + 16 * kg + 8);
-                if (!on) { a0 = (floatx2){0.f, 0.f}; a1 = a0; b0 = a0; b1 = a0; }
-                acc3 = __builtin_amdgcn_mfma_f32_16x16x4f32(a0[0], b0[0], acc3, 0, 0, 0);
-                acc3 = __builtin_amdgcn_mfma_f32_16x16x4f32(a0[1], b0[1], acc3, 0, 0, 0);
-                acc3 = __builtin_amdgcn_mfma_f32_16x16x4f32(a1[0], b1[0], acc3, 0, 0, 0);
-                acc3 = __builtin_amdgcn_mfma_f32_16x16x4f32(a1[1], b1[1], acc3, 0, 0, 0);
-            }
-        }
-        wave_lds_fence();
-        TRACE_PH(g, 3, 3, tph_);
-        float dq[F2MAX][MQ];
-#pragma unroll
-        for (int i = 0; i < F2MAX; ++i) {
-            if (i < F2) {
-                const int oz = i >= 2 ? opaque0_after(dq[i >= 2 ? i - 2 : 0][0]) : opaque0();
-                const float* w3c = prm + (g.o_W3 + i + oz);
-#pragma unroll
-                for (int m = 0; m < MQ; ++m) {
-                    const int t = lane + 64 * m;
-                    float a = 0.f;
-#pragma unroll
-                    for (int j = 0; j < F2MAX; ++j)
-                        if (j < F2) a = fmaf(w3c[j * F2], dr[j][m], a);
-                    dq[i][m] = a;
-                    if (t < T1) P1[i * RSW + LPQ + t] = a;
-                }
-            } else {
-#pragma unroll
-                for (int m = 0; m < MQ; ++m) dq[i][m] = 0.f;
-            }
-        }
-        wave_lds_fence();
-        TRACE_PH(g, 3, 4, tph_);
-        if (o2 < F2) {
-            const float* dqr = P1 + o2 * RSW + LPQ;
-            const float* d2r = P0 + o2 * RSW + 4 * kq;
-            for (int tq = 0; tq < ntq; ++tq) {
-                const floatx4 a4 = lds_ld4(dqr + 4 * tq);
-                const floatx4 w0 = lds_ld4(d2r + 4 * tq), w1 = lds_ld4(d2r + 4 * tq + 4);
-                const float w[8] = {w0[0], w0[1], w0[2], w0[3], w1[0], w1[1], w1[2], w1[3]};
-#pragma unroll
-                for (int kk = 0; kk < 4; ++kk)
-#pragma unroll
-                    for (int i = 0; i < 4; ++i) acc2[kk] = fmaf(a4[i], w[i + kk], acc2[kk]);
-            }
-        }
-        TRACE_PH(g, 3, 5, tph_);
-        const size_t rb = (size_t)b * F2 * T1;
-#pragma unroll
-        for (int o = 0; o < F2MAX; ++o) {
-            if (o >= F2) continue;
-            float a[MQ];
-            const int oz = o >= 2 ? opaque0_after(sz[o >= 2 ? o - 2 : 0]) : opaque0();
-            conv16_same_t<MQ>(dq[o], prm + (g.o_w2 + o * K2 + oz), a, lane);
-#pragma unroll
-            for (int m = 0; m < MQ; ++m) {
-                const int t = lane + 64 * m;
-                if (t < T1) {
-                    const int gi = o * T1 + t;
-                    const float dp = a[m] * keep_mul(g, mask2, dk0, (unsigned)(rb + gi));
-                    st_pol<EEGNET_NT_MID>(dp, dp2g + rb + gi);
-                    sz[o] = fmaf(dp * 0.25f, e1v[o][m], sz[o]);
-                    sz[F2MAX + o] = fmaf(dp * 0.25f, e2v[o][m], sz[F2MAX + o]);
-                }
-            }
-        }
-        wave_lds_fence();
-        TRACE_PH(g, 3, 6, tph_);
-    }
-    TRACE_LOOP(g, 3);
-    __syncthreads();
-    float* red = sm;
-    float* rw = red + wave * g.nD;
-#pragma unroll
-    for (int r = 0; r < 4; ++r) {
-        const int j = 4 * lk + r;
-        if (j < F2 && li < F2) rw[j * F2 + li] = acc3[r];
-    }
-    if (o2 < F2) {
-#pragma unroll
-        for (int kk = 0; kk < 4; ++kk) rw[F2 * F2 + o2 * K2 + 4 * kq + kk] = acc2[kk];
-    }
-    wave_reduce<2 * F2MAX>(sz);
-    if ((lane & 15) == 0) {
-        const int r0 = (lane >> 4) * (F2MAX / 2);
-#pragma unroll
-        for (int j = 0; j < F2MAX / 2; ++j) {
-            const int idx = j + r0;
-            if (idx < F2MAX) { if (idx < F2) rw[F2 * F2 + 16 * F2 + idx] = sz[j]; }
-            else if (idx - F2MAX < F2) rw[F2 * F2 + 17 * F2 + idx - F2MAX] = sz[j];
-        }
-    }
-    __syncthreads();
-    float* row = part + (size_t)blockIdx.x * g.nD;
-    for (int c = tid; c < g.nD; c += blockDim.x) pub(row + c, wave_rows_sum<NTHS / 64>(red, nw, g.nD, c));
-    double* dsm = (double*)sm;
-    if (grid_reduce(g, part, g.nD, fa, dsm)) { fin4(g, prm, dsm + 2, fa); TRACE(g, 3, TR_FIN); }
-}
-#endif
-
 __host__ __device__ constexpr int dr_stride(int MQ) { return 64 * MQ + 2; }
-__host__ __device__ constexpr int dr_lds_floats(int MQ) { return 4 * F2MAX * dr_stride(MQ) + F2MAX * (F2MAX + K2); }
+__host__ __device__ constexpr int dr_lds_floats(int MQ) { return 4 * F2MAX * dr_stride(MQ) + F2MAX * (F2MAX + K2 + 4); }
 __host__ __device__ constexpr int dr_tail_floats(bool hankel) { return NWB * 256 + 18 * F2MAX + (hankel ? NWB * RPW * 2 * 256 : 0); }
 
 template <int K1, int CC, int TT, int FF, bool FOLD = false, bool MASK = true>
 __global__ __launch_bounds__(NTB, TT ? WPEB : 2) void k_pass_dr(Geo g, const float* __restrict__ prm,
                                                   const float* coef,
-                                                  const float* __restrict__ d2g,
-                                                  const float* __restrict__ E1g,
-                                                  const float* __restrict__ E2g,
+                                                  const float* __restrict__ vg,
                                                   const float* __restrict__ q3g,
                                                   const float* __restrict__ r3g,
                                                   const uint8_t* __restrict__ mask2,
@@ -629,8 +382,7 @@
         char* ws = (char*)f.ws;
         prm = f.params;
         coef = (const float*)(ws + fc.off.coef);
-        d2g = (const float*)(ws + fc.off.d2);
-        E1g = (const float*)(ws + fc.off.E1); E2g = (const float*)(ws + fc.off.E2);
+        vg = (const float*)(ws + fc.off.v);
         q3g = (const float*)(ws + fc.off.q3); r3g = (const float*)(ws + fc.off.r3);
         mask2 = nullptr; mask3 = nullptr;
         dl = (const float*)(ws + fc.off.dl);
@@ -652,6 +404,7 @@
     float* const Q0 = DR0 + 2 * F2MAX * RSD;
     float* const W3t = Q0 + 2 * F2MAX * RSD;
     float* const W2t = W3t + F2MAX * F2MAX;
+    float* const CT2 = W2t + F2MAX * K2;
     const int tid = threadIdx.x, lane = tid & 63;
     const int li = lane & 15, lk = lane >> 4;
     const int wave = __builtin_amdgcn_readfirstlane(tid >> 6);
@@ -660,8 +413,10 @@
     const int nks = TT ? NKS : (T1 + 3) >> 2;
     constexpr bool FULL = TT && FF == F2MAX && TT / 4 == 64 * MQ;
 
-    float sr[2][RPW][MQ], sq[2][RPW][MQ], sd[2][RPW][MQ], se1[2][RPW][MQ], se2[2][RPW][MQ];
+    float sr[2][RPW][MQ], sq[2][RPW][MQ];
+    floatx4 sv[2][RPW][MQ];
     floatx4 sdl[2];
+    const int VP = 8 * EEG_NO(TT);
     auto row_base = [&](int bb, int r) {
         const int o = RPW * wave + r;
         return (size_t)bb * F2 * T1 + (size_t)((FULL || o < F2) ? o * T1 : 0);
@@ -685,18 +440,16 @@
             }
         xdl = ldc(reinterpret_cast<const floatx4*>(dl) + bb);
     };
-    auto load_de = [&](int bb, float (&xd)[RPW][MQ], float (&x1)[RPW][MQ], float (&x2)[RPW][MQ]) {
+    auto load_v = [&](int bb, floatx4 (&xv)[RPW][MQ]) {
 #pragma unroll
         for (int r = 0; r < RPW; ++r)
 #pragma unroll
             for (int m = 0; m < MQ; ++m) {
                 bool ok;
                 const int i = lane_off(r, m, ok);
-                const size_t rb_ = row_base(bb, r);
-                const float vd = (d2g + rb_)[i], v1 = (E1g + rb_)[i], v2 = (E2g + rb_)[i];
-                xd[r][m] = ok ? vd : 0.f;
-                x1[r][m] = ok ? v1 : 0.f;
-                x2[r][m] = ok ? v2 : 0.f;
+                const int o = RPW * wave + r;
+                const size_t vb_ = ((size_t)bb * F2 + ((FULL || o < F2) ? o : 0)) * VP;
+                xv[r][m] = *reinterpret_cast<const floatx4*>(vg + vb_ + 4 * i);
             }
     };
 
@@ -710,6 +463,11 @@
             if (o < F2) v = prm[g.o_w2 + k];
         }
         W3t[i] = v;
+    }
+    if (tid < 4 * F2MAX) {
+        const int o = tid >> 2, f = tid & 3, oo = o < F2 ? o : 0;
+        CT2[tid] = f == 0 ? coef[CF_AL2 * CSTR + oo] : f == 1 ? coef[CF_BE2 * CSTR + oo]
+                 : f == 2 ? prm[g.o_g2 + oo] : prm[g.o_b2 + oo];
     }
     if (F2 < F2MAX)
         for (int i = tid; i < 4 * (F2MAX - F2) * RSD; i += NTB) {
@@ -752,14 +510,14 @@
 #pragma unroll
     for (int k = 0; k < 2; ++k) {
         load_rq(min(b0 + k, blast), sr[k], sq[k], sdl[k]);
-        load_de(min(b0 + k, blast), sd[k], se1[k], se2[k]);
+        load_v(min(b0 + k, blast), sv[k]);
     }
     barrier_lds();
 
     TRACE(g, 3, TR_PRO);
     TRACE_DECL();
     auto trial = [&](const int bt, const bool live, const int buf, float (&xr)[RPW][MQ], float (&xq)[RPW][MQ],
-                     float (&xd)[RPW][MQ], float (&x1)[RPW][MQ], float (&x2)[RPW][MQ], floatx4& xdl) {
+                     floatx4 (&xv)[RPW][MQ], floatx4& xdl) {
         const int b = min(bt, blast), bn = min(bt + 2, blast);
         float* DR = DR0 + buf * F2MAX * RSD;
         float* Qb = Q0 + buf * F2MAX * RSD;
@@ -825,11 +583,23 @@
         for (int r = 0; r < RPW; ++r) {
             const int o = RPW * wave + r;
             if (!FULL && o >= F2) continue;
+            float xd[MQ], x1[MQ], x2[MQ], kp2[MQ];
+            const floatx4 c2 = lds_ld4(CT2 + 4 * o);
+#pragma unroll
+            for (int m = 0; m < MQ; ++m) {
+                const int t = lane + 64 * m;
+                const bool ok = FULL || t < T1;
+                kp2[m] = ok ? keep_mul(g, mask2, dk0, (unsigned)(rb + o * T1 + t)) : 0.f;
+                float d2;
+                bn2_pool4(xv[r][m][0], xv[r][m][1], xv[r][m][2], xv[r][m][3], c2[0], c2[1], c2[2], c2[3], kp2[m],
+                          d2, x1[m], x2[m]);
+                xd[m] = ok ? d2 : 0.f;
+            }
             if constexpr (FULL) {
                 const float dqg = live ? dq[r][0] : 0.f;
                 const int i0 = lane - 7, i1 = lane + 9;
-                const float d0 = __builtin_bit_cast(float, __builtin_amdgcn_ds_bpermute(max(i0, 0) * 4, __builtin_bit_cast(int, xd[r][0])));
-                const float d1 = __builtin_bit_cast(float, __builtin_amdgcn_ds_bpermute(min(i1, 63) * 4, __builtin_bit_cast(int, xd[r][0])));
+                const float d0 = __builtin_bit_cast(float, __builtin_amdgcn_ds_bpermute(max(i0, 0) * 4, __builtin_bit_cast(int, xd[0])));
+                const float d1 = __builtin_bit_cast(float, __builtin_amdgcn_ds_bpermute(min(i1, 63) * 4, __builtin_bit_cast(int, xd[0])));
                 hq[r][0] = __builtin_amdgcn_mfma_f32_16x16x4f32(dqg, i0 >= 0 ? d0 : 0.f, hq[r][0], 0, 0, 0);
                 hq[r][1] = __builtin_amdgcn_mfma_f32_16x16x4f32(dqg, i1 < 64 ? d1 : 0.f, hq[r][1], 0, 0, 0);
             } else {
@@ -837,7 +607,7 @@
 #pragma unroll
                 for (int m = 0; m < MQ; ++m) {
                     dqg[m] = live ? dq[r][m] : 0.f;
-                    s[m] = xd[r][m];
+                    s[m] = xd[m];
                     acc2[r][7] = fmaf(dqg[m], s[m], acc2[r][7]);
                 }
 #pragma unroll
@@ -847,7 +617,7 @@
                     for (int m = 0; m < MQ; ++m) acc2[r][k] = fmaf(dqg[m], s[m], acc2[r][k]);
                 }
 #pragma unroll
-                for (int m = 0; m < MQ; ++m) s[m] = xd[r][m];
+                for (int m = 0; m < MQ; ++m) s[m] = xd[m];
 #pragma unroll
                 for (int k = 6; k >= 0; --k) {
                     shr1<MQ>(s, lane);
@@ -869,21 +639,21 @@
                 const int t = lane + 64 * m;
                 if (FULL || t < T1) {
                     const int gi = o * T1 + t;
-                    const float dp = y[m] * keep_mul(g, mask2, dk0, (unsigned)(rb + gi));
+                    const float dp = y[m] * kp2[m];
                     st_pol<EEGNET_NT_MID>(dp, dp2g + rb + gi);
                     const float dpg = live ? dp * 0.25f : 0.f;
-                    sz1[r] = fmaf(dpg, x1[r][m], sz1[r]);
-                    sz2[r] = fmaf(dpg, x2[r][m], sz2[r]);
+                    sz1[r] = fmaf(dpg, x1[m], sz1[r]);
+                    sz2[r] = fmaf(dpg, x2[m], sz2[r]);
                 }
             }
         }
-        load_de(bn, xd, x1, x2);
+        load_v(bn, xv);
         TRACE_PH(g, 3, 4, tph_);
     };
     for (int b = b0; b < b1; b += 2) {
         pace_prio(b - b0, b1 - b0);
-        trial(b, true, 0, sr[0], sq[0], sd[0], se1[0], se2[0], sdl[0]);
-        trial(b + 1, b + 1 < b1, 1, sr[1], sq[1], sd[1], se1[1], se2[1], sdl[1]);
+        trial(b, true, 0, sr[0], sq[0], sv[0], sdl[0]);
+        trial(b + 1, b + 1 < b1, 1, sr[1], sq[1], sv[1], sdl[1]);
     }
     TRACE_LOOP(g, 3);
     tail_prio();
diff --git a/eegnetreplication_amd/csrc/eegnet_stream.hip b/eegnetreplication_amd/csrc/eegnet_stream.hip
--- a/eegnetreplication_amd/csrc/eegnet_stream.hip
+++ b/eegnetreplication_amd/csrc/eegnet_stream.hip
@@ -655,10 +655,9 @@
                                             const float* coef,
                                             const float* __restrict__ vg,
                                             const uint8_t* __restrict__ mask2,
-                                            float* __restrict__ d2g, float* __restrict__ E1g,
-                                            float* __restrict__ E2g, float* __restrict__ q3g,
-                                            float* __restrict__ r3g, float* __restrict__ part,
-                                            FinArgs fa, const FoldCall& fc, float* sm) {
+                                            float* __restrict__ q3g, float* __restrict__ r3g,
+                                            float* __restrict__ part, FinArgs fa, const FoldCall& fc,
+                                            float* sm) {
     EEG_DIMS_NT(g, NTB);
     TRACE(g, 1, TR_ENTRY);
     unsigned dk0;
@@ -669,7 +668,6 @@
         coef = (const float*)(ws + fc.off.coef);
         vg = (const float*)(ws + fc.off.v);
         mask2 = nullptr;
-        d2g = (float*)(ws + fc.off.d2); E1g = (float*)(ws + fc.off.E1); E2g = (float*)(ws + fc.off.E2);
         q3g = (float*)(ws + fc.off.q3); r3g = (float*)(ws + fc.off.r3);
         part = (float*)(ws + fc.off.partB);
         fa = fold_fin(fc, f, TK_B, 1, 0, true, false, g.nparam);
@@ -730,7 +728,6 @@
             v_load<MO>(vg, b, F2, NO, oh, lane, vc);
         }
         TRACE_PH(g, 1, 0, tph_);
-        float d2v[MO][2], e1v[MO][2], e2v[MO][2];
         if (oh < F2) {
             float* drow = D2s + oh * RS2 + LP2;
 #pragma unroll
@@ -740,19 +737,12 @@
 #pragma unroll
                 for (int h = 0; h < 2; ++h) {
                     const int q = 2 * oc + h;
-                    float pe = 0.f, e1 = 0.f, e2 = 0.f;
-#pragma unroll
-                    for (int i = 4 * h; i < 4 * h + 4; ++i) {
-                        const float xh = fmaf(alh, vc[m][i], beh);
-                        const float z = fmaf(gah, xh, bth);
-                        const float dz = elu_d(z);
-                        pe += z > 0.f ? z : dz - 1.f;
-                        e1 += dz;
-                        e2 = fmaf(dz, xh, e2);
+                    if (q < T1) {
+                        float d2, e1, e2;
+                        bn2_pool4(vc[m][4 * h], vc[m][4 * h + 1], vc[m][4 * h + 2], vc[m][4 * h + 3], alh, beh, gah, bth,
+                                  keep_mul(g, mask2, dk0, (unsigned)((b * F2 + oh) * T1 + q)), d2, e1, e2);
+                        drow[q] = d2;
                     }
-                    const float d2 = q < T1 ? pe * 0.25f * keep_mul(g, mask2, dk0, (unsigned)((b * F2 + oh) * T1 + q)) : 0.f;
-                    d2v[m][h] = d2; e1v[m][h] = e1; e2v[m][h] = e2;
-                    if (q < T1) drow[q] = d2;
                 }
             }
         }
@@ -774,22 +764,6 @@
             }
         }
         TRACE_PH(g, 1, 2, tph_);
-        if (oh < F2) {
-#pragma unroll
-            for (int m = 0; m < MO; ++m) {
-                const int oc = fir_oct(lane) + 32 * m;
-                if (oc >= NO) break;
-#pragma unroll
-                for (int h = 0; h < 2; ++h) {
-                    const int q = 2 * oc + h;
-                    if (q < T1) {
-                        const size_t gi = ((size_t)b * F2 + oh) * T1 + q;
-                        st_pol<EEGNET_NT_MID>(d2v[m][h], d2g + gi); st_pol<EEGNET_NT_MID>(e1v[m][h], E1g + gi);
-                        st_pol<EEGNET_NT_MID>(e2v[m][h], E2g + gi);
-                    }
-                }
-            }
-        }
         TRACE_PH(g, 1, 3, tph_);
         barrier_lds();
         TRACE_PH(g, 1, 4, tph_);
@@ -835,12 +809,10 @@
                                                       const float* coef,
                                                       const float* __restrict__ vg,
                                                       const uint8_t* __restrict__ mask2,
-                                                      float* __restrict__ d2g, float* __restrict__ E1g,
-                                                      float* __restrict__ E2g, float* __restrict__ q3g,
-                                                      float* __restrict__ r3g, float* __restrict__ part,
-                                                      FinArgs fa, FoldCall fc) {
+                                                      float* __restrict__ q3g, float* __restrict__ r3g,
+                                                      float* __restrict__ part, FinArgs fa, FoldCall fc) {
     extern __shared__ __attribute__((aligned(16))) float sm[];
-    pass_b_body<K1, CC, TT, FF, FOLD>(g, prm, coef, vg, mask2, d2g, E1g, E2g, q3g, r3g, part, fa, fc, sm);
+    pass_b_body<K1, CC, TT, FF, FOLD>(g, prm, coef, vg, mask2, q3g, r3g, part, fa, fc, sm);
 }
 
 #ifndef EEGNET_LDSX_E
```

Measured after the change: 18.35 million trials/s, median of 2. Within noise of the previous version (-0.0%).
